# BachiLi/redner

Hardware: AMD Instinct MI355X
Metric: Msamples/s fwd+bwd (higher is better)
Workload: dtype f64; 1 GPU; bunny_box 1024x1024, max_bounces 4, Sobol, 256 spp fwd+bwd per step (vertex gradients, primary+secondary edge sampling), sharded by sample index over 1 GPU(s): 256 spp per GPU; spp=256, spp_per_gpu=256, max_bounces=4, parallelism=sample-sharded x1, world_size=1, pool_cap_mb=32768, samples_per_launch=8, sample_workers=2, schedule=library default: two sample workers, batches as large as the buffer cache holds

## Files before the change

### include/redner_amd.h

```cpp
#ifndef REDNER_AMD_H
#define REDNER_AMD_H

#include <stddef.h>
#include <stdint.h>

#ifdef __cplusplus
extern "C" {
#endif

#define RDR_MAX_MIP_LEVELS 8

enum rdr_camera_type { RDR_CAMERA_PERSPECTIVE = 0, RDR_CAMERA_ORTHOGRAPHIC = 1, RDR_CAMERA_FISHEYE = 2,
                       RDR_CAMERA_PANORAMA = 3 };
enum rdr_sampler_type { RDR_SAMPLER_INDEPENDENT = 0, RDR_SAMPLER_SOBOL = 1 };
enum rdr_channel {
    RDR_CH_RADIANCE = 0, RDR_CH_ALPHA, RDR_CH_DEPTH, RDR_CH_POSITION, RDR_CH_GEOMETRY_NORMAL,
    RDR_CH_SHADING_NORMAL, RDR_CH_UV, RDR_CH_BARYCENTRIC_COORDINATES, RDR_CH_DIFFUSE_REFLECTANCE,
    RDR_CH_SPECULAR_REFLECTANCE, RDR_CH_ROUGHNESS, RDR_CH_GENERIC_TEXTURE, RDR_CH_VERTEX_COLOR,
    RDR_CH_SHAPE_ID, RDR_CH_TRIANGLE_ID, RDR_CH_MATERIAL_ID
};

typedef struct rdr_camera_desc {
    int width, height;
    const float *position, *look, *up;
    const float *cam_to_world, *world_to_cam;
    const float *intrinsic_mat_inv, *intrinsic_mat;
    const float *distortion_params;
    float clip_near;
    int camera_type;
    int viewport_beg[2], viewport_end[2];
} rdr_camera_desc;

typedef struct rdr_dcamera_desc {
    float *position, *look, *up, *cam_to_world, *world_to_cam, *intrinsic_mat_inv, *intrinsic_mat,
          *distortion_params;
} rdr_dcamera_desc;

typedef struct rdr_shape_desc {
    const float *vertices;
    const int32_t *indices;
    const float *uvs;
    const float *normals;
    const int32_t *uv_indices;
    const int32_t *normal_indices;
    const float *colors;
    int num_vertices, num_uv_vertices, num_normal_vertices, num_triangles;
    int material_id, light_id;
} rdr_shape_desc;

typedef struct rdr_dshape_desc { float *vertices, *uvs, *normals, *colors; } rdr_dshape_desc;

typedef struct rdr_texture_desc {
    const float *texels[RDR_MAX_MIP_LEVELS];
    int width[RDR_MAX_MIP_LEVELS], height[RDR_MAX_MIP_LEVELS];
    int channels;
    int num_levels;
    const float *uv_scale;
} rdr_texture_desc;

typedef struct rdr_material_desc {
    rdr_texture_desc diffuse_reflectance, specular_reflectance, roughness, generic_texture, normal_map;
    int compute_specular_lighting, two_sided, use_vertex_color;
} rdr_material_desc;

typedef struct rdr_dtexture_desc {
    float *texels[RDR_MAX_MIP_LEVELS];
    int num_levels;
    float *uv_scale;
} rdr_dtexture_desc;
typedef struct rdr_dmaterial_desc {
    rdr_dtexture_desc diffuse_reflectance, specular_reflectance, roughness, generic_texture, normal_map;
} rdr_dmaterial_desc;

typedef struct rdr_area_light_desc {
    int shape_id;
    float intensity[3];
    int two_sided, directly_visible;
} rdr_area_light_desc;
typedef struct rdr_darea_light_desc { float *intensity; } rdr_darea_light_desc;

typedef struct rdr_envmap_desc {
    rdr_texture_desc values;
    const float *env_to_world, *world_to_env;
    const float *sample_cdf_ys, *sample_cdf_xs;
    float pdf_norm;
    int directly_visible;
} rdr_envmap_desc;
typedef struct rdr_denvmap_desc { rdr_dtexture_desc values; float *world_to_env; } rdr_denvmap_desc;

typedef struct rdr_tuning rdr_tuning;
typedef struct rdr_render_options {
    uint64_t seed;
    int num_samples, max_bounces;
    const int *channels; int num_channels;
    int sampler_type;
    int sample_pixel_center;
    int sample_offset, total_samples;
    const rdr_tuning *tuning;
} rdr_render_options;

enum rdr_tune_flags {
    RDR_TUNE_NO_OVERLAP       = 1 << 0,
    RDR_TUNE_FORCE_GENERAL    = 1 << 1,
    RDR_TUNE_PICKN_WALK       = 1 << 2,
    RDR_TUNE_PICKH_FUSED      = 1 << 3,
    RDR_TUNE_PICKH_LAZY       = 1 << 4,
    RDR_TUNE_NO_HOIST         = 1 << 5,
    RDR_TUNE_REFILL_OFF       = 1 << 6,
    RDR_TUNE_REFILL_ALL       = 1 << 7,
    RDR_TUNE_TRACE_BINARY     = 1 << 8,
    RDR_TUNE_TRACE_NO_LDS_TOP = 1 << 9,
    RDR_TUNE_NO_FUSED_BOUNCE  = 1 << 10,
    RDR_TUNE_PICKH_ONE_LAUNCH = 1 << 11,
    RDR_TUNE_NO_NEE_COMPACT   = 1 << 12,
    RDR_TUNE_LARGE_FORMS      = 1 << 13,
    RDR_TUNE_TRACE_EVERY_CONTINUATION = 1 << 14
};
struct rdr_tuning {
    unsigned flags;
    int batch_samples;
    int64_t batch_lanes;
    int workers;
    int refill_rays_per_lane, refill_idle_lanes, refill_steps;
    int wide_max_rays;
    int gather_budget;
    int gather_heavy_cap_plus1, gather_work_cap_plus1;
    int mem_available_mb;
    int refill_order;
    int pickh_slots_per_lane, pickh_idle_lanes, pickh_steps;
    int stale_event_cap_plus1;
};

void rdr_set_stream(void *hip_stream);
void rdr_set_pool_cap_mb(int64_t megabytes);
int64_t rdr_get_pool_cap_mb(void);
enum rdr_build_flags {
    RDR_BUILD_NO_REFIT        = 1 << 0,
    RDR_BUILD_NO_EDGE_CACHE   = 1 << 1,
    RDR_BUILD_SYNC_EDGES      = 1 << 2,
    RDR_BUILD_EDGE_HOST_BUILD = 1 << 3
};
void rdr_set_build_flags(unsigned flags);

typedef struct rdr_dscene_desc {
    rdr_dcamera_desc camera;
    const rdr_dshape_desc *shapes; int num_shapes;
    const rdr_dmaterial_desc *materials; int num_materials;
    const rdr_darea_light_desc *area_lights; int num_area_lights;
    const rdr_denvmap_desc *envmap;
} rdr_dscene_desc;

typedef struct rdr_scene rdr_scene;

rdr_scene *rdr_scene_create(const rdr_camera_desc *camera,
                            const rdr_shape_desc *shapes, int num_shapes,
                            const rdr_material_desc *materials, int num_materials,
                            const rdr_area_light_desc *area_lights, int num_area_lights,
                            const rdr_envmap_desc *envmap,
                            int use_gpu, int gpu_index,
                            int use_primary_edge_sampling, int use_secondary_edge_sampling);
void rdr_scene_destroy(rdr_scene *scene);
int rdr_scene_max_generic_texture_dimension(const rdr_scene *scene);

int rdr_render(const rdr_scene *scene, const rdr_render_options *options,
               float *rendered_image, const float *d_rendered_image,
               const rdr_dscene_desc *d_scene,
               float *screen_gradient_image, float *debug_image);

int rdr_compute_num_channels(const int *channels, int num_channels, int max_generic_texture_dimension);

enum rdr_deferred_light_type { RDR_DL_AMBIENT = 0, RDR_DL_POINT = 1, RDR_DL_DIRECTIONAL = 2, RDR_DL_SPOT = 3 };
typedef struct rdr_deferred_desc {
    int num_images, height, width;
    int aa_samples, alpha;
    int num_lights;
    const int32_t *light_type;
    const int32_t *image_light_range;
    int gpu_index;
} rdr_deferred_desc;
int rdr_deferred_shade(const rdr_deferred_desc *desc, const float *g_buffer, const float *light_params, float *image);
int rdr_deferred_shade_backward(const rdr_deferred_desc *desc, const float *g_buffer, const float *light_params,
                                const float *d_image, float *d_g_buffer, float *d_light_params);

int rdr_mip_num_levels(int height, int width);
int64_t rdr_mip_backward_scratch(int height, int width, int channels);
int rdr_mip_tiled_stages(int height, int width, int channels);
int rdr_mip_pyramid(int height, int width, int channels, int num_levels, float *const *levels, int gpu_index);
int rdr_mip_pyramid_backward(int height, int width, int channels, int num_levels, const float *const *d_levels, float *d_texels,
                             float *scratch, int64_t scratch_floats, int gpu_index);

typedef enum { rdr_normal_weighting_max = 0, rdr_normal_weighting_cotangent = 1 } rdr_normal_weighting;
typedef struct rdr_mesh_topology rdr_mesh_topology;
rdr_mesh_topology *rdr_mesh_topology_create(const int *indices, int num_triangles, int num_vertices, int use_gpu, int gpu_index);
void rdr_mesh_topology_destroy(rdr_mesh_topology *topology);
int rdr_mesh_topology_read(const rdr_mesh_topology *topology, int *offsets, int *corners);
int rdr_vertex_normal_scratch(const rdr_mesh_topology *topology, int scheme, int64_t *forward_floats, int64_t *backward_floats,
                              int64_t *saved_floats);
int rdr_vertex_normal(const rdr_mesh_topology *topology, int scheme, const float *vertices, float *normals, float *saved,
                      float *scratch, int64_t scratch_floats);
int rdr_vertex_normal_backward(const rdr_mesh_topology *topology, int scheme, const float *vertices, const float *saved,
                               const float *d_normals, float *d_vertices, float *scratch, int64_t scratch_floats);

const char *rdr_last_error(void);

typedef struct rdr_trace_stats {
    double closest_ms, any_ms;
    uint64_t closest_launches, any_launches;
    uint64_t closest_rays, any_rays;
    uint64_t closest_nodes, closest_tris, any_nodes, any_tris;
    uint64_t closest_wide_nodes, any_wide_nodes;
    double closest_union_ms, any_union_ms;
} rdr_trace_stats;
void rdr_trace_stats_enable(int timing, int counting);
void rdr_trace_stats_reset(void);
void rdr_trace_stats_get(rdr_trace_stats *out);

int rdr_scene_trace(const rdr_scene *scene, const float *rays, int32_t *hits, int num_rays, int any_hit);

uint64_t rdr_trim_cache(void);

typedef struct rdr_debug_counters {
    uint64_t device_mallocs, host_count_reads;
    uint64_t last_batch_samples, last_workers;
} rdr_debug_counters;
void rdr_debug_counters_get(rdr_debug_counters *out);

int rdr_debug_bvh_check(const rdr_scene *scene);

int rdr_debug_dump_edges(const rdr_scene *scene, const char *path);

int rdr_debug_trace_plan(int num_nodes, int stack_need, int has_wide, int wide_stack_need, int num_rays, int any_hit, int coherent,
                         int counting, const rdr_tuning *tuning, int32_t *out );
int rdr_debug_scene_trace_plan(const rdr_scene *scene, int num_rays, int any_hit, int coherent, int counting,
                               const rdr_tuning *tuning, int32_t *out );

int rdr_libm_exact(void);

int rdr_debug_libm(int fn, const double *x, const double *y, double *out, int n);

enum rdr_scatter_op {
    RDR_SCATTER_ACCUM = 0, RDR_SCATTER_ACCUM_TEXEL, RDR_SCATTER_ACCUM_PLAIN, RDR_SCATTER_ACCUM_TRIPLE,
    RDR_SCATTER_ACCUM_TEXEL_TRIPLE, RDR_SCATTER_TRIGRAD_WAVE, RDR_SCATTER_POSITIONS_WAVE
};
enum rdr_scatter_target {
    RDR_TARGET_VERTICES = 0, RDR_TARGET_UVS, RDR_TARGET_NORMALS, RDR_TARGET_COLORS, RDR_TARGET_TEXTURE, RDR_TARGET_LIGHTS,
    RDR_TARGET_CAMERA, RDR_TARGET_ENVMAP
};
int rdr_debug_grad_scatter(const rdr_scene *scene, const rdr_dscene_desc *d_scene, uint64_t job_samples, int op, int plain,
                           int num_lanes, const uint8_t *active, const int32_t *target, const int32_t *index,
                           const double *values);

#ifdef __cplusplus
}
#endif
#endif
```

### redner_amd/_capi.py

```python
import ctypes as C
import os

MAX_MIP = 8
_HERE = os.path.dirname(os.path.abspath(__file__))
DEFAULT_LIBRARY = os.path.join(_HERE, 'lib', 'libredner_amd.so')
EXACT_LIBRARY = os.path.join(_HERE, 'lib', 'libredner_amd_exact.so')

c_float_p = C.POINTER(C.c_float)
c_int_p = C.POINTER(C.c_int32)


class CameraDesc(C.Structure):
    _fields_ = [('width', C.c_int), ('height', C.c_int),
                ('position', C.c_void_p), ('look', C.c_void_p), ('up', C.c_void_p),
                ('cam_to_world', C.c_void_p), ('world_to_cam', C.c_void_p),
                ('intrinsic_mat_inv', C.c_void_p), ('intrinsic_mat', C.c_void_p),
                ('distortion_params', C.c_void_p),
                ('clip_near', C.c_float), ('camera_type', C.c_int),
                ('viewport_beg', C.c_int * 2), ('viewport_end', C.c_int * 2)]


class DCameraDesc(C.Structure):
    _fields_ = [(n, C.c_void_p) for n in ('position', 'look', 'up', 'cam_to_world', 'world_to_cam',
                                          'intrinsic_mat_inv', 'intrinsic_mat', 'distortion_params')]


class ShapeDesc(C.Structure):
    _fields_ = [('vertices', C.c_void_p), ('indices', C.c_void_p), ('uvs', C.c_void_p),
                ('normals', C.c_void_p), ('uv_indices', C.c_void_p), ('normal_indices', C.c_void_p),
                ('colors', C.c_void_p),
                ('num_vertices', C.c_int), ('num_uv_vertices', C.c_int), ('num_normal_vertices', C.c_int),
                ('num_triangles', C.c_int), ('material_id', C.c_int), ('light_id', C.c_int)]


class DShapeDesc(C.Structure):
    _fields_ = [(n, C.c_void_p) for n in ('vertices', 'uvs', 'normals', 'colors')]


class TextureDesc(C.Structure):
    _fields_ = [('texels', C.c_void_p * MAX_MIP), ('width', C.c_int * MAX_MIP), ('height', C.c_int * MAX_MIP),
                ('channels', C.c_int), ('num_levels', C.c_int), ('uv_scale', C.c_void_p)]


class MaterialDesc(C.Structure):
    _fields_ = [('diffuse_reflectance', TextureDesc), ('specular_reflectance', TextureDesc),
                ('roughness', TextureDesc), ('generic_texture', TextureDesc), ('normal_map', TextureDesc),
                ('compute_specular_lighting', C.c_int), ('two_sided', C.c_int), ('use_vertex_color', C.c_int)]


class DTextureDesc(C.Structure):
    _fields_ = [('texels', C.c_void_p * MAX_MIP), ('num_levels', C.c_int), ('uv_scale', C.c_void_p)]


class DMaterialDesc(C.Structure):
    _fields_ = [(n, DTextureDesc) for n in ('diffuse_reflectance', 'specular_reflectance', 'roughness',
                                            'generic_texture', 'normal_map')]


class AreaLightDesc(C.Structure):
    _fields_ = [('shape_id', C.c_int), ('intensity', C.c_float * 3), ('two_sided', C.c_int),
                ('directly_visible', C.c_int)]


class DAreaLightDesc(C.Structure):
    _fields_ = [('intensity', C.c_void_p)]


class EnvmapDesc(C.Structure):
    _fields_ = [('values', TextureDesc), ('env_to_world', C.c_void_p), ('world_to_env', C.c_void_p),
                ('sample_cdf_ys', C.c_void_p), ('sample_cdf_xs', C.c_void_p),
                ('pdf_norm', C.c_float), ('directly_visible', C.c_int)]


class DEnvmapDesc(C.Structure):
    _fields_ = [('values', DTextureDesc), ('world_to_env', C.c_void_p)]


class Tuning(C.Structure):
    _fields_ = [('flags', C.c_uint), ('batch_samples', C.c_int), ('batch_lanes', C.c_int64), ('workers', C.c_int),
                ('refill_rays_per_lane', C.c_int), ('refill_idle_lanes', C.c_int), ('refill_steps', C.c_int),
                ('wide_max_rays', C.c_int), ('gather_budget', C.c_int),
                ('gather_heavy_cap_plus1', C.c_int), ('gather_work_cap_plus1', C.c_int), ('mem_available_mb', C.c_int),
                ('refill_order', C.c_int), ('pickh_slots_per_lane', C.c_int), ('pickh_idle_lanes', C.c_int), ('pickh_steps', C.c_int),
                ('stale_event_cap_plus1', C.c_int)]


TUNE_NO_OVERLAP, TUNE_FORCE_GENERAL, TUNE_PICKN_WALK, TUNE_PICKH_FUSED, TUNE_PICKH_LAZY, TUNE_NO_HOIST, TUNE_REFILL_OFF, \
    TUNE_REFILL_ALL, TUNE_TRACE_BINARY, TUNE_TRACE_NO_LDS_TOP, TUNE_NO_FUSED_BOUNCE, TUNE_PICKH_ONE_LAUNCH, TUNE_NO_NEE_COMPACT, \
    TUNE_LARGE_FORMS, TUNE_TRACE_EVERY_CONTINUATION = [1 << k for k in range(15)]
BUILD_NO_REFIT, BUILD_NO_EDGE_CACHE, BUILD_SYNC_EDGES, BUILD_EDGE_HOST_BUILD = [1 << k for k in range(4)]


class RenderOptionsDesc(C.Structure):
    _fields_ = [('seed', C.c_uint64), ('num_samples', C.c_int), ('max_bounces', C.c_int),
                ('channels', C.POINTER(C.c_int)), ('num_channels', C.c_int),
                ('sampler_type', C.c_int), ('sample_pixel_center', C.c_int),
                ('sample_offset', C.c_int), ('total_samples', C.c_int),
                ('tuning', C.POINTER(Tuning))]


class DSceneDesc(C.Structure):
    _fields_ = [('camera', DCameraDesc),
                ('shapes', C.POINTER(DShapeDesc)), ('num_shapes', C.c_int),
                ('materials', C.POINTER(DMaterialDesc)), ('num_materials', C.c_int),
                ('area_lights', C.POINTER(DAreaLightDesc)), ('num_area_lights', C.c_int),
                ('envmap', C.POINTER(DEnvmapDesc))]


class TraceStats(C.Structure):
    _fields_ = [('closest_ms', C.c_double), ('any_ms', C.c_double),
                ('closest_launches', C.c_uint64), ('any_launches', C.c_uint64),
                ('closest_rays', C.c_uint64), ('any_rays', C.c_uint64),
                ('closest_nodes', C.c_uint64), ('closest_tris', C.c_uint64),
                ('any_nodes', C.c_uint64), ('any_tris', C.c_uint64),
                ('closest_wide_nodes', C.c_uint64), ('any_wide_nodes', C.c_uint64),
                ('closest_union_ms', C.c_double), ('any_union_ms', C.c_double)]


class DebugCounters(C.Structure):
    _fields_ = [('device_mallocs', C.c_uint64), ('host_count_reads', C.c_uint64),
                ('last_batch_samples', C.c_uint64), ('last_workers', C.c_uint64)]


class DeferredDesc(C.Structure):
    _fields_ = [('num_images', C.c_int), ('height', C.c_int), ('width', C.c_int),
                ('aa_samples', C.c_int), ('alpha', C.c_int), ('num_lights', C.c_int),
                ('light_type', c_int_p), ('image_light_range', c_int_p), ('gpu_index', C.c_int)]


DL_AMBIENT, DL_POINT, DL_DIRECTIONAL, DL_SPOT = range(4)

EXPORTS = ('rdr_scene_create', 'rdr_scene_destroy', 'rdr_scene_max_generic_texture_dimension',
           'rdr_render', 'rdr_compute_num_channels', 'rdr_last_error',
           'rdr_trace_stats_enable', 'rdr_trace_stats_reset', 'rdr_trace_stats_get', 'rdr_scene_trace',
           'rdr_debug_counters_get', 'rdr_trim_cache', 'rdr_debug_dump_edges', 'rdr_debug_bvh_check',
           'rdr_set_stream', 'rdr_set_pool_cap_mb', 'rdr_get_pool_cap_mb', 'rdr_set_build_flags', 'rdr_debug_libm', 'rdr_libm_exact',
           'rdr_deferred_shade', 'rdr_deferred_shade_backward',
           'rdr_mip_num_levels', 'rdr_mip_backward_scratch', 'rdr_mip_tiled_stages', 'rdr_mip_pyramid',
           'rdr_mip_pyramid_backward',
           'rdr_mesh_topology_create', 'rdr_mesh_topology_destroy', 'rdr_mesh_topology_read', 'rdr_vertex_normal_scratch',
           'rdr_vertex_normal', 'rdr_vertex_normal_backward', 'rdr_debug_trace_plan', 'rdr_debug_scene_trace_plan',
           'rdr_debug_grad_scatter')

SCATTER_ACCUM, SCATTER_ACCUM_TEXEL, SCATTER_ACCUM_PLAIN, SCATTER_ACCUM_TRIPLE, SCATTER_ACCUM_TEXEL_TRIPLE, \
    SCATTER_TRIGRAD_WAVE, SCATTER_POSITIONS_WAVE = range(7)
TARGET_VERTICES, TARGET_UVS, TARGET_NORMALS, TARGET_COLORS, TARGET_TEXTURE, TARGET_LIGHTS, TARGET_CAMERA, TARGET_ENVMAP = range(8)

_lib = None
_lib_path = None


def load(path=None):
    global _lib, _lib_path
    path = path or os.environ.get('REDNER_AMD_LIB') or \
        (EXACT_LIBRARY if os.environ.get('REDNER_AMD_LIBM', '').lower() == 'exact' else DEFAULT_LIBRARY)
    if not os.path.exists(path):
        raise RuntimeError(
            "redner_amd: native library %s not found. Build it with "
            "`python -c 'import __graft_entry__ as g; g.build()'` (hipcc, gfx950). "
            "There is no CPU fallback." % path)
    lib = C.CDLL(path)
    for name in EXPORTS:
        if not hasattr(lib, name):
            raise RuntimeError("redner_amd: %s does not export %s" % (path, name))
    lib.rdr_scene_create.restype = C.c_void_p
    lib.rdr_scene_create.argtypes = [C.POINTER(CameraDesc), C.POINTER(ShapeDesc), C.c_int,
                                     C.POINTER(MaterialDesc), C.c_int, C.POINTER(AreaLightDesc), C.c_int,
                                     C.POINTER(EnvmapDesc), C.c_int, C.c_int, C.c_int, C.c_int]
    lib.rdr_scene_destroy.restype = None
    lib.rdr_scene_destroy.argtypes = [C.c_void_p]
    lib.rdr_scene_max_generic_texture_dimension.restype = C.c_int
    lib.rdr_scene_max_generic_texture_dimension.argtypes = [C.c_void_p]
    lib.rdr_render.restype = C.c_int
    lib.rdr_render.argtypes = [C.c_void_p, C.POINTER(RenderOptionsDesc), C.c_void_p, C.c_void_p,
                               C.POINTER(DSceneDesc), C.c_void_p, C.c_void_p]
    lib.rdr_compute_num_channels.restype = C.c_int
    lib.rdr_compute_num_channels.argtypes = [C.POINTER(C.c_int), C.c_int, C.c_int]
    lib.rdr_last_error.restype = C.c_char_p
    lib.rdr_last_error.argtypes = []
    lib.rdr_trace_stats_enable.restype = None
    lib.rdr_trace_stats_enable.argtypes = [C.c_int, C.c_int]
    lib.rdr_trace_stats_reset.restype = None
    lib.rdr_debug_counters_get.restype = None
    lib.rdr_debug_counters_get.argtypes = [C.POINTER(DebugCounters)]
    lib.rdr_trim_cache.restype = C.c_uint64
    lib.rdr_trim_cache.argtypes = []
    lib.rdr_debug_bvh_check.restype = C.c_int
    lib.rdr_debug_bvh_check.argtypes = [C.c_void_p]
    lib.rdr_set_stream.restype = None
    lib.rdr_set_stream.argtypes = [C.c_void_p]
    lib.rdr_set_pool_cap_mb.restype = None
    lib.rdr_set_pool_cap_mb.argtypes = [C.c_int64]
    lib.rdr_get_pool_cap_mb.restype = C.c_int64
    lib.rdr_get_pool_cap_mb.argtypes = []
    lib.rdr_set_build_flags.restype = None
    lib.rdr_set_build_flags.argtypes = [C.c_uint]
    lib.rdr_trace_stats_get.restype = None
    lib.rdr_trace_stats_get.argtypes = [C.POINTER(TraceStats)]
    lib.rdr_scene_trace.restype = C.c_int
    lib.rdr_scene_trace.argtypes = [C.c_void_p, C.c_void_p, C.c_void_p, C.c_int, C.c_int]
    lib.rdr_libm_exact.restype = C.c_int
    lib.rdr_libm_exact.argtypes = []
    lib.rdr_debug_libm.restype = C.c_int
    lib.rdr_debug_libm.argtypes = [C.c_int, C.c_void_p, C.c_void_p, C.c_void_p, C.c_int]
    lib.rdr_deferred_shade.restype = C.c_int
    lib.rdr_deferred_shade.argtypes = [C.POINTER(DeferredDesc), C.c_void_p, C.c_void_p, C.c_void_p]
    lib.rdr_deferred_shade_backward.restype = C.c_int
    lib.rdr_deferred_shade_backward.argtypes = [C.POINTER(DeferredDesc), C.c_void_p, C.c_void_p, C.c_void_p, C.c_void_p, C.c_void_p]
    lib.rdr_mip_num_levels.restype = C.c_int
    lib.rdr_mip_num_levels.argtypes = [C.c_int, C.c_int]
    lib.rdr_mip_backward_scratch.restype = C.c_int64
    lib.rdr_mip_backward_scratch.argtypes = [C.c_int, C.c_int, C.c_int]
    lib.rdr_mip_tiled_stages.restype = C.c_int
    lib.rdr_mip_tiled_stages.argtypes = [C.c_int, C.c_int, C.c_int]
    lib.rdr_mip_pyramid.restype = C.c_int
    lib.rdr_mip_pyramid.argtypes = [C.c_int, C.c_int, C.c_int, C.c_int, C.POINTER(C.c_void_p), C.c_int]
    lib.rdr_mip_pyramid_backward.restype = C.c_int
    lib.rdr_mip_pyramid_backward.argtypes = [C.c_int, C.c_int, C.c_int, C.c_int, C.POINTER(C.c_void_p), C.c_void_p, C.c_void_p,
                                             C.c_int64, C.c_int]
    lib.rdr_mesh_topology_create.restype = C.c_void_p
    lib.rdr_mesh_topology_create.argtypes = [C.c_void_p, C.c_int, C.c_int, C.c_int, C.c_int]
    lib.rdr_mesh_topology_destroy.restype = None
    lib.rdr_mesh_topology_destroy.argtypes = [C.c_void_p]
    lib.rdr_mesh_topology_read.restype = C.c_int
    lib.rdr_mesh_topology_read.argtypes = [C.c_void_p, C.c_void_p, C.c_void_p]
    lib.rdr_vertex_normal_scratch.restype = C.c_int
    lib.rdr_vertex_normal_scratch.argtypes = [C.c_void_p, C.c_int, C.POINTER(C.c_int64), C.POINTER(C.c_int64), C.POINTER(C.c_int64)]
    lib.rdr_vertex_normal.restype = C.c_int
    lib.rdr_vertex_normal.argtypes = [C.c_void_p, C.c_int, C.c_void_p, C.c_void_p, C.c_void_p, C.c_void_p, C.c_int64]
    lib.rdr_vertex_normal_backward.restype = C.c_int
    lib.rdr_vertex_normal_backward.argtypes = [C.c_void_p, C.c_int, C.c_void_p, C.c_void_p, C.c_void_p, C.c_void_p, C.c_void_p,
                                               C.c_int64]
    lib.rdr_debug_trace_plan.restype = C.c_int
    lib.rdr_debug_trace_plan.argtypes = [C.c_int] * 8 + [C.POINTER(Tuning), C.c_void_p]
    lib.rdr_debug_scene_trace_plan.restype = C.c_int
    lib.rdr_debug_scene_trace_plan.argtypes = [C.c_void_p] + [C.c_int] * 4 + [C.POINTER(Tuning), C.c_void_p]
    lib.rdr_debug_grad_scatter.restype = C.c_int
    lib.rdr_debug_grad_scatter.argtypes = [C.c_void_p, C.POINTER(DSceneDesc), C.c_uint64, C.c_int, C.c_int, C.c_int,
                                           C.c_void_p, C.c_void_p, C.c_void_p, C.c_void_p]
    _lib, _lib_path = lib, path
    return lib


def lib():
    if _lib is None:
        load()
    return _lib


def library_path():
    return _lib_path


def is_product_library():
    return _lib_path in (DEFAULT_LIBRARY, EXACT_LIBRARY)


def last_error():
    return lib().rdr_last_error().decode('utf-8', 'replace')
```

### redner_amd/csrc/capi.cpp

```cpp
#include "../../include/redner_amd.h"
#include "render.h"
#include "tuning.h"
#include "trace_plan.h"
#include "edges.h"
#include "deferred.h"
#include "mipmap.h"
#include "vertex_normal.h"
#include <cstdio>
#include "scene.h"
#include <cstring>
#include <exception>
#include <mutex>
#include <string>
#include <vector>
#include <cstdlib>

namespace {
thread_local std::string g_last_error;
std::recursive_mutex g_device_lock[16];
std::recursive_mutex &device_lock(int gpu_index) { return g_device_lock[(gpu_index < 0 ? 0 : gpu_index) & 15]; }
void set_error(const char *what) { g_last_error = what ? what : "unknown error"; }
thread_local void *g_user_stream = nullptr;
void use_caller_stream() { exec::ctx().stream = (hipStream_t)g_user_stream; }
}

struct LibmProbe {
    int fn; const double *x, *y; double *out;
    RDR_FN void operator()(int i) const {
        const double a = x[i], b = y[i];
        double r;
        switch (fn) {
            case 0: r = gm::sin(a); break;
            case 1: r = gm::cos(a); break;
            case 2: r = gm::atan2(a, b); break;
            case 3: r = gm::atan(a); break;
            case 4: r = gm::acos(a); break;
            case 5: r = gm::log(a); break;
            default: r = gm::pow(a, b); break;
        }
        out[i] = r;
    }
};

extern "C" {

const char *rdr_last_error(void) { return g_last_error.c_str(); }

rdr_scene *rdr_scene_create(const rdr_camera_desc *camera, const rdr_shape_desc *shapes, int num_shapes,
                            const rdr_material_desc *materials, int num_materials,
                            const rdr_area_light_desc *area_lights, int num_area_lights,
                            const rdr_envmap_desc *envmap, int use_gpu, int gpu_index,
                            int use_primary_edge_sampling, int use_secondary_edge_sampling) {
    try {
        g_last_error.clear();
        std::lock_guard<std::recursive_mutex> lk(device_lock(gpu_index));
        use_caller_stream();
        return reinterpret_cast<rdr_scene *>(rdr::create_scene(camera, shapes, num_shapes, materials, num_materials,
                                                               area_lights, num_area_lights, envmap, use_gpu, gpu_index,
                                                               use_primary_edge_sampling, use_secondary_edge_sampling));
    } catch (const std::exception &e) {
        set_error(e.what());
        return nullptr;
    }
}

void rdr_scene_destroy(rdr_scene *scene) {
    if (!scene) return;
    rdr::Scene *s = reinterpret_cast<rdr::Scene *>(scene);
    std::lock_guard<std::recursive_mutex> lk(device_lock(s->gpu_index));
    delete s;
}

int rdr_scene_max_generic_texture_dimension(const rdr_scene *scene) {
    return scene ? reinterpret_cast<const rdr::Scene *>(scene)->max_generic_texture_dimension : 0;
}

int rdr_render(const rdr_scene *scene, const rdr_render_options *options, float *rendered_image,
               const float *d_rendered_image, const rdr_dscene_desc *d_scene, float *screen_gradient_image,
               float *debug_image) {
    try {
        g_last_error.clear();
        if (!scene || !options) throw std::runtime_error("rdr_render: scene and options are required");
        const rdr::Scene &s = *reinterpret_cast<const rdr::Scene *>(scene);
        std::lock_guard<std::recursive_mutex> lk(device_lock(s.gpu_index));
        exec::select_device(1, s.gpu_index);
        use_caller_stream();
        rdr::render(s, *options, rendered_image, d_rendered_image, d_scene, screen_gradient_image, debug_image);
        return 0;
    } catch (const std::exception &e) {
        set_error(e.what());
        return 1;
    }
}

int rdr_deferred_shade(const rdr_deferred_desc *desc, const float *g_buffer, const float *light_params, float *image) {
    try {
        g_last_error.clear();
        if (!desc) throw std::runtime_error("rdr_deferred_shade: a description is required");
        std::lock_guard<std::recursive_mutex> lk(device_lock(desc->gpu_index));
        exec::select_device(desc->gpu_index >= 0, desc->gpu_index);
        use_caller_stream();
        rdr::dfr::shade(*desc, g_buffer, light_params, image);
        return 0;
    } catch (const std::exception &e) {
        set_error(e.what());
        return 1;
    }
}

int rdr_deferred_shade_backward(const rdr_deferred_desc *desc, const float *g_buffer, const float *light_params,
                                const float *d_image, float *d_g_buffer, float *d_light_params) {
    try {
        g_last_error.clear();
        if (!desc) throw std::runtime_error("rdr_deferred_shade_backward: a description is required");
        std::lock_guard<std::recursive_mutex> lk(device_lock(desc->gpu_index));
        exec::select_device(desc->gpu_index >= 0, desc->gpu_index);
        use_caller_stream();
        rdr::dfr::shade_backward(*desc, g_buffer, light_params, d_image, d_g_buffer, d_light_params);
        return 0;
    } catch (const std::exception &e) {
        set_error(e.what());
        return 1;
    }
}

int rdr_mip_num_levels(int height, int width) { return height > 0 && width > 0 ? rdr::mip::num_levels(height, width) : 0; }

int64_t rdr_mip_backward_scratch(int height, int width, int channels) {
    try {
        g_last_error.clear();
        return (int64_t)rdr::mip::scratch_floats(rdr::mip::make_shape(height, width, channels, rdr_mip_num_levels(height, width),
                                                                      "rdr_mip_backward_scratch"));
    } catch (const std::exception &e) {
        set_error(e.what());
        return -1;
    }
}

int rdr_mip_tiled_stages(int height, int width, int channels) {
    try {
        g_last_error.clear();
        return rdr::mip::tiled_stages(rdr::mip::make_shape(height, width, channels, rdr_mip_num_levels(height, width),
                                                           "rdr_mip_tiled_stages"));
    } catch (const std::exception &e) {
        set_error(e.what());
        return -1;
    }
}

static void mip_select(int gpu_index, const char *who) {
#if !defined(RDR_HOSTSIM)
    if (gpu_index < 0) throw std::runtime_error(std::string(who) + ": host memory (negative gpu_index) is for the CPU harness only");
#endif
    exec::select_device(gpu_index >= 0, gpu_index);
    use_caller_stream();
}

int rdr_mip_pyramid(int height, int width, int channels, int num_levels, float *const *levels, int gpu_index) {
    try {
        g_last_error.clear();
        std::lock_guard<std::recursive_mutex> lk(device_lock(gpu_index));
        mip_select(gpu_index, "rdr_mip_pyramid");
        rdr::mip::pyramid(height, width, channels, num_levels, levels);
        return 0;
    } catch (const std::exception &e) {
        set_error(e.what());
        return 1;
    }
}

int rdr_mip_pyramid_backward(int height, int width, int channels, int num_levels, const float *const *d_levels, float *d_texels,
                             float *scratch, int64_t scratch_floats, int gpu_index) {
    try {
        g_last_error.clear();
        std::lock_guard<std::recursive_mutex> lk(device_lock(gpu_index));
        mip_select(gpu_index, "rdr_mip_pyramid_backward");
        rdr::mip::pyramid_backward(height, width, channels, num_levels, d_levels, d_texels, scratch,
                                   scratch_floats > 0 ? (size_t)scratch_floats : 0);
        return 0;
    } catch (const std::exception &e) {
        set_error(e.what());
        return 1;
    }
}

static const rdr::vnrm::Topology &topology_of(const rdr_mesh_topology *topology, const char *who) {
    if (!topology) throw std::runtime_error(std::string(who) + ": a topology is required");
    return *reinterpret_cast<const rdr::vnrm::Topology *>(topology);
}

rdr_mesh_topology *rdr_mesh_topology_create(const int *indices, int num_triangles, int num_vertices, int use_gpu, int gpu_index) {
    try {
        g_last_error.clear();
        const int place = use_gpu ? (gpu_index < 0 ? 0 : gpu_index) : -1;
        std::lock_guard<std::recursive_mutex> lk(device_lock(place));
        mip_select(place, "rdr_mesh_topology_create");
        return reinterpret_cast<rdr_mesh_topology *>(rdr::vnrm::create_topology(indices, num_triangles, num_vertices, place));
    } catch (const std::exception &e) {
        set_error(e.what());
        return nullptr;
    }
}

void rdr_mesh_topology_destroy(rdr_mesh_topology *topology) {
    if (!topology) return;
    rdr::vnrm::Topology *t = reinterpret_cast<rdr::vnrm::Topology *>(topology);
    std::lock_guard<std::recursive_mutex> lk(device_lock(t->gpu_index));
    try { exec::select_device(t->gpu_index >= 0, t->gpu_index); } catch (const std::exception &) {}
    delete t;
}

int rdr_mesh_topology_read(const rdr_mesh_topology *topology, int *offsets, int *corners) {
    try {
        g_last_error.clear();
        const rdr::vnrm::Topology &t = topology_of(topology, "rdr_mesh_topology_read");
        std::lock_guard<std::recursive_mutex> lk(device_lock(t.gpu_index));
        mip_select(t.gpu_index, "rdr_mesh_topology_read");
        rdr::vnrm::read_topology(t, offsets, corners);
        return 0;
    } catch (const std::exception &e) {
        set_error(e.what());
        return 1;
    }
}

int rdr_vertex_normal_scratch(const rdr_mesh_topology *topology, int scheme, int64_t *forward_floats, int64_t *backward_floats,
                              int64_t *saved_floats) {
    try {
        g_last_error.clear();
        const rdr::vnrm::Topology &t = topology_of(topology, "rdr_vertex_normal_scratch");
        const bool cot = rdr::vnrm::cotangent(scheme, "rdr_vertex_normal_scratch");
        if (forward_floats) *forward_floats = (int64_t)rdr::vnrm::forward_scratch_floats(t, cot);
        if (backward_floats) *backward_floats = (int64_t)rdr::vnrm::backward_scratch_floats(t, cot);
        if (saved_floats) *saved_floats = (int64_t)rdr::vnrm::saved_floats(t, cot);
        return 0;
    } catch (const std::exception &e) {
        set_error(e.what());
        return 1;
    }
}

int rdr_vertex_normal(const rdr_mesh_topology *topology, int scheme, const float *vertices, float *normals, float *saved,
                      float *scratch, int64_t scratch_floats) {
    try {
        g_last_error.clear();
        const rdr::vnrm::Topology &t = topology_of(topology, "rdr_vertex_normal");
        std::lock_guard<std::recursive_mutex> lk(device_lock(t.gpu_index));
        mip_select(t.gpu_index, "rdr_vertex_normal");
        rdr::vnrm::forward(t, scheme, vertices, normals, saved, scratch, scratch_floats > 0 ? (size_t)scratch_floats : 0);
        return 0;
    } catch (const std::exception &e) {
        set_error(e.what());
        return 1;
    }
}

int rdr_vertex_normal_backward(const rdr_mesh_topology *topology, int scheme, const float *vertices, const float *saved,
                               const float *d_normals, float *d_vertices, float *scratch, int64_t scratch_floats) {
    try {
        g_last_error.clear();
        const rdr::vnrm::Topology &t = topology_of(topology, "rdr_vertex_normal_backward");
        std::lock_guard<std::recursive_mutex> lk(device_lock(t.gpu_index));
        mip_select(t.gpu_index, "rdr_vertex_normal_backward");
        rdr::vnrm::backward(t, scheme, vertices, saved, d_normals, d_vertices, scratch, scratch_floats > 0 ? (size_t)scratch_floats : 0);
        return 0;
    } catch (const std::exception &e) {
        set_error(e.what());
        return 1;
    }
}

int rdr_compute_num_channels(const int *channels, int num_channels, int max_generic_texture_dimension) {
    return rdr::compute_num_channels(channels, num_channels, max_generic_texture_dimension);
}

void rdr_trace_stats_enable(int timing, int counting) {
    exec::trace_stats().timing = timing != 0;
    exec::trace_stats().counting = counting != 0;
}
void rdr_trace_stats_reset(void) {
    exec::TraceStats &s = exec::trace_stats();
    bool t = s.timing, c = s.counting;
    exec::trace_stats_collect();
    s = exec::TraceStats();
    s.timing = t; s.counting = c;
}
void rdr_trace_stats_get(rdr_trace_stats *out) {
    exec::trace_stats_collect();
    const exec::TraceStats &s = exec::trace_stats();
    out->closest_ms = s.closest_ms; out->any_ms = s.any_ms;
    out->closest_launches = s.closest_launches; out->any_launches = s.any_launches;
    out->closest_rays = s.closest_rays; out->any_rays = s.any_rays;
    out->closest_nodes = s.nodes[0]; out->closest_tris = s.tris[0];
    out->any_nodes = s.nodes[1]; out->any_tris = s.tris[1];
    out->closest_wide_nodes = s.wide_nodes[0]; out->any_wide_nodes = s.wide_nodes[1];
    out->closest_union_ms = s.closest_union_ms; out->any_union_ms = s.any_union_ms;
}

uint64_t rdr_trim_cache(void) {
    std::unique_lock<std::recursive_mutex> all[16];
    for (int d = 0; d < 16; ++d) all[d] = std::unique_lock<std::recursive_mutex>(g_device_lock[d]);
    rdr::drop_edge_cache();
    const uint64_t bytes = exec::pool_cached_bytes();
    exec::pool_trim();
    return bytes;
}

void rdr_set_stream(void *hip_stream) { g_user_stream = hip_stream; }
void rdr_set_pool_cap_mb(int64_t megabytes) { exec::pool_set_cap(megabytes < 0 ? -1 : (long long)megabytes << 20); }
int64_t rdr_get_pool_cap_mb(void) { return (int64_t)(exec::pool_cap_bytes() >> 20); }
void rdr_set_build_flags(unsigned flags) { rdr::build_flags_ref().store(flags); }

void rdr_debug_counters_get(rdr_debug_counters *out) {
    out->device_mallocs = exec::pool_device_mallocs();
    out->host_count_reads = exec::host_count_reads();
    out->last_batch_samples = (uint64_t)rdr::last_schedule()[0].load();
    out->last_workers = (uint64_t)rdr::last_schedule()[1].load();
}

int rdr_debug_dump_edges(const rdr_scene *scene, const char *path) {
    const rdr::Scene &s = *reinterpret_cast<const rdr::Scene *>(scene);
    FILE *f = fopen(path, "w");
    if (!f) return 1;
    {
        std::lock_guard<std::recursive_mutex> lk(device_lock(s.gpu_index));
        exec::select_device(1, s.gpu_index);
        try { s.edge_data(); } catch (const std::exception &e) { set_error(e.what()); fclose(f); return 1; }
    }
    if (!s.edges) { fprintf(f, "edges 0\n"); fclose(f); return 0; }
    if (s.edges->device_trees) {
        std::lock_guard<std::recursive_mutex> lk(device_lock(s.gpu_index));
        try { rdr::download_edge_trees(*s.edges); } catch (const std::exception &e) { set_error(e.what()); fclose(f); return 1; }
    }
    const rdr::EdgeData &ed = *s.edges;
    fprintf(f, "edges %d\n", (int)ed.edges.size());
    for (const rdr::EdgeD &e : ed.edges) fprintf(f, "%d %d %d %d %d\n", e.shape_id, e.v0, e.v1, e.f0, e.f1);
    if (!ed.cs_nodes.empty() || !ed.ncs_nodes.empty()) {
        fprintf(f, "expand %.17g\n", ed.edge_bounds_expand);
        for (int t = 0; t < 2; ++t) {
            const std::vector<rdr::EdgeNode> &nodes = t == 0 ? ed.cs_nodes : ed.ncs_nodes;
            int nl = t == 0 ? ed.cs_leaves : ed.ncs_leaves;
            int nn = (int)nodes.size() - nl;
            fprintf(f, "%s %d %d\n", t == 0 ? "cs" : "ncs", nl == 0 ? 0 : nn, nl);
            for (size_t i = 0; i < nodes.size(); ++i) {
                const rdr::EdgeNode &n = nodes[i];
                fprintf(f, "%d %d %d %d %d %.17g %.17g", (int)i, n.parent, n.child0, n.child1, n.edge_id, n.wlen, n.cost);
                fprintf(f, " %.17g %.17g %.17g %.17g %.17g %.17g", n.p_min.x, n.p_min.y, n.p_min.z, n.p_max.x, n.p_max.y, n.p_max.z);
                if (t == 1) fprintf(f, " %.17g %.17g %.17g %.17g %.17g %.17g", n.d_min.x, n.d_min.y, n.d_min.z, n.d_max.x, n.d_max.y, n.d_max.z);
                fprintf(f, "\n");
            }
        }
    }
    fclose(f);
    return 0;
}

int rdr_debug_bvh_check(const rdr_scene *scene) {
    try {
        const rdr::Scene &s = *reinterpret_cast<const rdr::Scene *>(scene);
        if (!s.bvh_dev || s.bvh_dev->parent) return -1;
        std::lock_guard<std::recursive_mutex> lk(device_lock(s.gpu_index));
        exec::select_device(1, s.gpu_index);
        use_caller_stream();
        std::vector<rt::MeshView> meshes(s.shapes.size());
        for (size_t i = 0; i < s.shapes.size(); ++i) meshes[i] = rt::MeshView{s.h_vertices[i].data(), s.h_indices[i].data(), s.shapes[i].num_triangles};
        const rt::BvhHost h = rt::build_bvh(meshes);
        const rt::BvhDev &d = *s.bvh_dev;
        int bad = 0;
        if ((int)h.nodes.size() != d.num_nodes || (int)h.ids.size() != 2 * d.num_slots || (int)h.wide.size() != d.num_wide ||
            h.depth != d.depth || h.wide_stack_need != d.wide_stack_need)
            return 1000000 + std::abs((int)h.nodes.size() - d.num_nodes);
        std::vector<rt::Node> nodes(d.num_nodes);
        std::vector<int> ids((size_t)2 * d.num_slots);
        std::vector<float> tris((size_t)9 * d.num_slots);
        std::vector<rt::Node4> wide(d.num_wide);
        exec::download(nodes.data(), d.nodes, sizeof(rt::Node) * nodes.size());
        exec::download(ids.data(), d.ids, sizeof(int) * ids.size());
        exec::download(tris.data(), d.tris, sizeof(float) * tris.size());
        exec::download(wide.data(), d.wide, sizeof(rt::Node4) * wide.size());
        for (size_t i = 0; i < nodes.size(); ++i) {
            const rt::Node &a = nodes[i], &b = h.nodes[i];
            bool same = a.a == b.a && a.b == b.b;
            for (int k = 0; k < 3; ++k) same = same && a.lo[k] == b.lo[k] && a.hi[k] == b.hi[k];
            bad += !same;
        }
        for (size_t i = 0; i < ids.size(); ++i) bad += ids[i] != h.ids[i];
        for (size_t i = 0; i < tris.size(); ++i) bad += !(tris[i] == h.tris[i]);
        for (size_t i = 0; i < wide.size(); ++i) {
            const rt::Node4 &a = wide[i], &b = h.wide[i];
            bool same = a.aux[0] == b.aux[0];
            for (int k = 0; k < 4; ++k)
                same = same && a.link[k] == b.link[k] && a.lox[k] == b.lox[k] && a.loy[k] == b.loy[k] && a.loz[k] == b.loz[k] &&
                       a.hix[k] == b.hix[k] && a.hiy[k] == b.hiy[k] && a.hiz[k] == b.hiz[k];
            bad += !same;
        }
        return bad;
    } catch (const std::exception &e) {
        set_error(e.what());
        return -2;
    }
}

int rdr_scene_trace(const rdr_scene *scene, const float *rays, int32_t *hits, int num_rays, int any_hit) {
    try {
        g_last_error.clear();
        const rdr::Scene &s = *reinterpret_cast<const rdr::Scene *>(scene);
        std::lock_guard<std::recursive_mutex> lk(device_lock(s.gpu_index));
        exec::select_device(1, s.gpu_index);
        use_caller_stream();
        exec::trace(s.bvh, reinterpret_cast<const rt::RayRec *>(rays), reinterpret_cast<rt::HitRec *>(hits), num_rays, any_hit != 0);
        exec::sync();
        return 0;
    } catch (const std::exception &e) {
        set_error(e.what());
        return 1;
    }
}

static int write_trace_plan(const exec::TraceFacts &facts, int num_rays, int any_hit, int coherent, int counting,
                            const rdr_tuning *tuning, int32_t *out) {
    try {
        g_last_error.clear();
        if (num_rays <= 0 || !out || facts.num_nodes < 0 || facts.stack_need < 0 || facts.wide_stack_need < 0)
            throw std::runtime_error("rdr_debug_trace_plan: bad arguments");
        const exec::TracePlan p = exec::plan_trace(facts, num_rays, any_hit != 0, coherent != 0, counting != 0, rdr::resolve_tuning(tuning));
        const int32_t v[10] = {(int32_t)p.form, p.stack, p.short_index, p.stage_top, p.sorted, p.counting, p.blocks, p.rays_per_lane, p.idle_min, p.steps};
        std::memcpy(out, v, sizeof(v));
        return 0;
    } catch (const std::exception &e) {
        set_error(e.what());
        return 1;
    }
}
int rdr_debug_trace_plan(int num_nodes, int stack_need, int has_wide, int wide_stack_need, int num_rays, int any_hit, int coherent,
                         int counting, const rdr_tuning *tuning, int32_t *out) {
    return write_trace_plan(exec::TraceFacts{num_nodes, stack_need, wide_stack_need, has_wide != 0}, num_rays, any_hit, coherent, counting, tuning, out);
}
int rdr_debug_scene_trace_plan(const rdr_scene *scene, int num_rays, int any_hit, int coherent, int counting, const rdr_tuning *tuning,
                               int32_t *out) {
    if (!scene) { set_error("rdr_debug_scene_trace_plan: bad arguments"); return 1; }
    return write_trace_plan(exec::trace_facts(reinterpret_cast<const rdr::Scene *>(scene)->bvh), num_rays, any_hit, coherent, counting, tuning, out);
}

int rdr_debug_libm(int fn, const double *x, const double *y, double *out, int n) {
    try {
        g_last_error.clear();
        if (fn < 0 || fn > 6 || n < 0) throw std::runtime_error("rdr_debug_libm: bad arguments");
        std::lock_guard<std::recursive_mutex> lk(device_lock(exec::current_device()));
        exec::select_device(1, exec::current_device());
        use_caller_stream();
        const size_t bytes = sizeof(double) * (size_t)n;
        struct Held {
            double *p[3] = {nullptr, nullptr, nullptr};
            ~Held() { exec::device_sync(); for (double *q : p) exec::dfree(q); }
        } held;
        for (double *&q : held.p) q = (double *)exec::dmalloc(bytes);
        double *dx = held.p[0], *dy = held.p[1], *dout = held.p[2];
        exec::upload(dx, x, bytes);
        if (y) exec::upload(dy, y, bytes); else exec::zero(dy, bytes);
        exec::launch(exec::Count(n), LibmProbe{fn, dx, dy, dout});
        exec::download(out, dout, bytes);
        exec::sync();
        return 0;
    } catch (const std::exception &e) {
        set_error(e.what());
        return 1;
    }
}

int rdr_debug_grad_scatter(const rdr_scene *scene, const rdr_dscene_desc *d_scene, uint64_t job_samples, int op, int plain,
                           int num_lanes, const uint8_t *active, const int32_t *target, const int32_t *index,
                           const double *values) {
    try {
        g_last_error.clear();
        if (!scene || !d_scene) throw std::runtime_error("rdr_debug_grad_scatter: scene and d_scene are required");
        const rdr::Scene &s = *reinterpret_cast<const rdr::Scene *>(scene);
        std::lock_guard<std::recursive_mutex> lk(device_lock(s.gpu_index));
        exec::select_device(1, s.gpu_index);
        use_caller_stream();
        rdr::debug_grad_scatter(s, *d_scene, (size_t)job_samples, op, plain != 0, num_lanes, active, target, index, values);
        return 0;
    } catch (const std::exception &e) {
        set_error(e.what());
        return 1;
    }
}

}
```

### redner_amd/csrc/grad_store.h

```cpp
#pragma once
#include "scene.h"
#include "stages_bwd.h"
#include <algorithm>
#include <exception>
#include <stdexcept>
#include <vector>

namespace rdr {

struct Arena {
    std::vector<void *> blocks;
    template <class T> T *get(size_t count) {
        T *p = (T *)exec::pool_alloc(sizeof(T) * (count ? count : 1));
        blocks.push_back(p);
        return p;
    }
    ~Arena() {
        if (std::uncaught_exceptions() > 0) exec::device_sync();
        for (void *p : blocks) exec::pool_free(p);
    }
};

struct GradStore {
    Arena arena;
    GScene g;
    std::vector<GShape> h_shapes;
    std::vector<GMaterial> h_materials;

    static constexpr size_t kSmallTensor = 16384, kSmallTierMax = 65536;
    struct Tier { double *base = nullptr; size_t stride = 0, cursor = 0; int replicas = 1; };
    Tier tier[2];
    struct Pair { double *acc; float *out; size_t count; int tier; };
    std::vector<Pair> pairs;
    bool counting = true;

    double *place(size_t count, int &t) {
        const size_t padded = (count + 3) & ~(size_t)3;
        t = (count <= kSmallTensor && tier[0].cursor + padded <= kSmallTierMax) ? 0 : 1;
        const size_t at = tier[t].cursor;
        tier[t].cursor += padded;
        return counting ? reinterpret_cast<double *>(8) : tier[t].base + at;
    }
    double *mirror(float *out, size_t count) {
        if (!out || count == 0) return nullptr;
        int t;
        double *acc = place(count, t);
        if (!counting) pairs.push_back(Pair{acc, out, count, t});
        return acc;
    }
    GTex mirror_tex(const TexD &t, const rdr_dtexture_desc &d) {
        GTex g;
        for (int i = 0; i < kMaxMip; ++i) g.texels[i] = nullptr;
        g.uv_scale = nullptr;
        if (t.num_levels == 0 || d.num_levels == 0) return g;
        bool constant = t.width[0] <= 0 && t.height[0] <= 0;
        for (int i = 0; i < t.num_levels && i < d.num_levels; ++i) {
            size_t count = constant ? (size_t)t.channels : (size_t)t.width[i] * t.height[i] * t.channels;
            g.texels[i] = mirror(d.texels[i], count);
        }
        g.uv_scale = mirror(d.uv_scale, 2);
        return g;
    }

    GradStore(const Scene &scene, const rdr_dscene_desc &ds, size_t job_samples) {
        counting = true;
        layout(scene, ds);
        for (Tier &t : tier) t.stride = (t.cursor + 31) & ~(size_t)31;
        tier[0].replicas = tier[0].stride ? exec::choose_replicas(tier[0].stride * sizeof(double), 256 * kSmallTierMax * sizeof(double)) : 1;
        tier[1].replicas = tier[1].stride ? exec::choose_replicas(tier[1].stride * sizeof(double), exec::replica_budget(job_samples)) : 1;
        const size_t small_total = tier[0].stride * tier[0].replicas, total = small_total + tier[1].stride * tier[1].replicas;
        double *block = arena.get<double>(total);
        exec::zero(block, sizeof(double) * total);
        tier[0].base = block; tier[1].base = block + small_total;
        exec::set_replicas(ReplicaLayout{block + tier[0].stride, tier[0].stride, tier[1].stride,
                                         (unsigned)(tier[0].replicas - 1), (unsigned)(tier[1].replicas - 1)});
        counting = false; pairs.clear();
        for (Tier &t : tier) t.cursor = 0;
        layout(scene, ds);
        for (const Pair &p : pairs) {
            const Tier &t = tier[p.tier];
            if (p.acc < t.base || p.acc + p.count > t.base + t.stride)
                throw std::runtime_error("render: gradient accumulator straddles a replica tier (GradStore::layout)");
        }
        accumulators_laid_out(tier[0].base, tier[0].stride);
    }
    void layout(const Scene &scene, const rdr_dscene_desc &ds) {
        if (ds.num_shapes != (int)scene.shapes.size() || ds.num_materials != (int)scene.materials.size() ||
            ds.num_area_lights != (int)scene.lights.size())
            throw std::runtime_error("render: DScene does not match the Scene (shape/material/light counts)");
        h_shapes.resize(scene.shapes.size());
        for (size_t i = 0; i < scene.shapes.size(); ++i) {
            const ShapeD &sh = scene.shapes[i];
            const rdr_dshape_desc &d = ds.shapes[i];
            h_shapes[i].vertices = mirror(d.vertices, (size_t)3 * sh.num_vertices);
            if (!h_shapes[i].vertices) throw std::runtime_error("render: DShape.vertices is required");
            h_shapes[i].uvs = sh.uvs ? mirror(d.uvs, (size_t)2 * (sh.num_uv_vertices > 0 ? sh.num_uv_vertices : sh.num_vertices)) : nullptr;
            h_shapes[i].normals = sh.normals ? mirror(d.normals, (size_t)3 * (sh.num_normal_vertices > 0 ? sh.num_normal_vertices : sh.num_vertices)) : nullptr;
            h_shapes[i].colors = sh.colors ? mirror(d.colors, (size_t)3 * sh.num_vertices) : nullptr;
        }
        h_materials.resize(scene.materials.size());
        for (size_t i = 0; i < scene.materials.size(); ++i) {
            const MaterialD &m = scene.materials[i];
            const rdr_dmaterial_desc &d = ds.materials[i];
            h_materials[i].diffuse = mirror_tex(m.diffuse, d.diffuse_reflectance);
            h_materials[i].specular = mirror_tex(m.specular, d.specular_reflectance);
            h_materials[i].roughness = mirror_tex(m.roughness, d.roughness);
            h_materials[i].generic = mirror_tex(m.generic, d.generic_texture);
            h_materials[i].normal_map = mirror_tex(m.normal_map, d.normal_map);
        }
        if (!counting) {
            g.shapes = arena.get<GShape>(h_shapes.size());
            exec::upload(g.shapes, h_shapes.data(), sizeof(GShape) * h_shapes.size());
            g.materials = arena.get<GMaterial>(h_materials.size());
            exec::upload(g.materials, h_materials.data(), sizeof(GMaterial) * h_materials.size());
        }
        g.light_intensity = nullptr;
        if (!scene.lights.empty()) {
            int light_tier = 0;
            g.light_intensity = place(3 * scene.lights.size(), light_tier);
            if (!counting)
                for (size_t l = 0; l < scene.lights.size(); ++l)
                    if (ds.area_lights[l].intensity) pairs.push_back(Pair{g.light_intensity + 3 * l, ds.area_lights[l].intensity, 3, light_tier});
        }
        const rdr_dcamera_desc &dc = ds.camera;
        g.cam.position = mirror(dc.position, 3); g.cam.look = mirror(dc.look, 3); g.cam.up = mirror(dc.up, 3);
        g.cam.cam_to_world = mirror(dc.cam_to_world, 16); g.cam.world_to_cam = mirror(dc.world_to_cam, 16);
        g.cam.intrinsic_mat_inv = mirror(dc.intrinsic_mat_inv, 9); g.cam.intrinsic_mat = mirror(dc.intrinsic_mat, 9);
        g.cam.distortion = mirror(dc.distortion_params, 8);
        g.envmap = nullptr;
        if (scene.d.envmap && ds.envmap) {
            GEnvmap h_envmap;
            h_envmap.values = mirror_tex(scene.h_envmap.values, ds.envmap->values);
            h_envmap.world_to_env = mirror(ds.envmap->world_to_env, 16);
            if (!counting) {
                g.envmap = arena.get<GEnvmap>(1);
                exec::upload(g.envmap, &h_envmap, sizeof(GEnvmap));
            }
        }
    }
    void flush() {
        for (const Pair &p : pairs)
            if (p.tier == 0) accumulator_before_fold(tier[0].base, p.acc, p.count);
        accumulators_folded();
        std::vector<Pair> by_out(pairs);
        std::sort(by_out.begin(), by_out.end(), [](const Pair &a, const Pair &b) { return a.out < b.out; });
        bool aliased = false;
        for (size_t i = 1; i < by_out.size(); ++i) aliased = aliased || by_out[i - 1].out + by_out[i - 1].count > by_out[i].out;
        for (int t = 0; t < 2; ++t) {
            const Tier &tr = tier[t];
            std::vector<FlushSegment> seg;
            for (const Pair &p : pairs) if (p.tier == t) seg.push_back(FlushSegment{(size_t)(p.acc - tr.base), p.count, p.out});
            if (seg.empty()) continue;
            std::sort(seg.begin(), seg.end(), [](const FlushSegment &a, const FlushSegment &b) { return a.begin < b.begin; });
            if (tr.stride > (size_t)0x7fffffff) throw std::runtime_error("render: gradient block too large");
            FlushSegment *d_seg = arena.get<FlushSegment>(seg.size());
            exec::upload(d_seg, seg.data(), sizeof(FlushSegment) * seg.size());
            if (!aliased) exec::launch((int)tr.stride, FlushGrad{tr.base, tr.stride, tr.replicas, d_seg, (int)seg.size()});
            else for (size_t i = 0; i < seg.size(); ++i)
                exec::launch((int)(seg[i].begin + seg[i].count), FlushGrad{tr.base, tr.stride, tr.replicas, d_seg + i, 1});
        }
        exec::set_replicas(ReplicaLayout{nullptr, 0, 0, 0, 0});
    }
};

}
```

### redner_amd/csrc/hip/exec.h

```cpp
#pragma once
#include <hip/hip_runtime.h>
#include <stdint.h>
#include <stdio.h>
#include <atomic>
#include <condition_variable>
#include <cstdlib>
#include <exception>
#include <functional>
#include <mutex>
#include <stdexcept>
#include <string>
#include <thread>

#define RDR_FN __host__ __device__ inline
#define RDR_INLINE_CALL [[clang::always_inline]]
#define RDR_DEV_FN __device__ inline
#define RDR_STACK_DECL(T, name, N) __shared__ T name##_lds[(N) * 256]; T *name = name##_lds + threadIdx.x
#define RDR_STACK_AT(name, k) name[(k) * 256]
#define RDR_WALK_STACK_MEMBER(T, name, N)
#define RDR_WALK_STACK(st, T, name, N, TAG) (rdr::lds_column<T, N, TAG>())
#define RDR_WALK_AT(stk, k) stk[(k) * 256]

namespace rdr {
template <class T, int N, int TAG>
__device__ inline T *lds_column() {
    __shared__ T tile[N * 256];
    return tile + threadIdx.x;
}
__host__ inline void *lds_column_host_stub() { return nullptr; }

struct ReplicaLayout {
    const double *hot_end;
    unsigned long long hot_stride;
    unsigned long long stride;
    unsigned hot_mask, mask;
};
static __device__ ReplicaLayout g_rep = {nullptr, 0, 0, 0, 0};
__device__ inline double *replica_of(double *p) {
    const unsigned wave = blockIdx.x * 4u + (threadIdx.x >> 6);
    const bool hot = p < g_rep.hot_end;
    return p + (size_t)(wave & (hot ? g_rep.hot_mask : g_rep.mask)) * (hot ? g_rep.hot_stride : g_rep.stride);
}
constexpr int kAccumRounds = 3;

__device__ inline double wave_sum(double x) {
#define RDR_DPP_ADD(ctrl)                                                                                  \
    {                                                                                                      \
        const int lo_ = __builtin_amdgcn_update_dpp(0, __double2loint(x), ctrl, 0xf, 0xf, true);         \
        const int hi_ = __builtin_amdgcn_update_dpp(0, __double2hiint(x), ctrl, 0xf, 0xf, true);         \
        x += __hiloint2double(hi_, lo_);                                                                   \
    }
    RDR_DPP_ADD(0xB1)
    RDR_DPP_ADD(0x4E)
    RDR_DPP_ADD(0x141)
    RDR_DPP_ADD(0x140)
#undef RDR_DPP_ADD
    const int lo = __double2loint(x), hi = __double2hiint(x);
    const double r0 = __hiloint2double(__builtin_amdgcn_readlane(hi, 0), __builtin_amdgcn_readlane(lo, 0));
    const double r1 = __hiloint2double(__builtin_amdgcn_readlane(hi, 16), __builtin_amdgcn_readlane(lo, 16));
    const double r2 = __hiloint2double(__builtin_amdgcn_readlane(hi, 32), __builtin_amdgcn_readlane(lo, 32));
    const double r3 = __hiloint2double(__builtin_amdgcn_readlane(hi, 48), __builtin_amdgcn_readlane(lo, 48));
    return (r0 + r1) + (r2 + r3);
}

typedef __attribute__((address_space(1))) double *GlobalDouble;
__device__ inline void global_add_f64(double *p, double v) { (void)__builtin_amdgcn_global_atomic_fadd_f64((GlobalDouble)p, v); }
__device__ inline void accum_rounds(double *p, double v, int ROUNDS);
__device__ inline void accum(double *p, double v) { accum_rounds(p, v, kAccumRounds); }
static __device__ int g_texel_rounds = 8;
__device__ inline void accum_texel(double *p, double v) { accum_rounds(p, v, g_texel_rounds); }
__device__ inline void accum_rounds(double *p, double v, int ROUNDS) {
    p = replica_of(p);
    const unsigned long long act = __ballot(1);
    const unsigned long long addr = (unsigned long long)p;
    const int lane = threadIdx.x & 63;
    const int vlo = __double2loint(v), vhi = __double2hiint(v);
    unsigned long long rem = act;
    bool mine = true;
    for (int round = 0; round < ROUNDS && rem != 0; ++round) {
        const int l = __ffsll((long long)rem) - 1;
        const unsigned lo = __builtin_amdgcn_readlane((unsigned)addr, l);
        const unsigned hi = __builtin_amdgcn_readlane((unsigned)(addr >> 32), l);
        const bool same = addr == (((unsigned long long)hi << 32) | lo);
        const unsigned long long m = __ballot(same) & rem;
        rem &= ~m;
        if (__popcll(m) < 2) continue;
        double s;
        if (act == ~0ull) {
            s = wave_sum(same ? v : 0.0);
        } else {
            s = 0;
            unsigned long long mm = m;
            while (mm) {
                const int k = __ffsll((long long)mm) - 1;
                mm &= mm - 1;
                s += __hiloint2double(__builtin_amdgcn_readlane(vhi, k), __builtin_amdgcn_readlane(vlo, k));
            }
        }
        if (lane == l) global_add_f64(p, s);
        if (same) mine = false;
    }
    if (mine) global_add_f64(p, v);
}
__device__ inline void accum_triple_rounds(double *p, double x, double y, double z, int ROUNDS) {
    p = replica_of(p);
    const unsigned long long act = __ballot(1);
    const unsigned long long addr = (unsigned long long)p;
    const int lane = threadIdx.x & 63;
    unsigned long long rem = act;
    bool mine = true;
    for (int round = 0; round < ROUNDS && rem != 0; ++round) {
        const int l = __ffsll((long long)rem) - 1;
        const unsigned lo = __builtin_amdgcn_readlane((unsigned)addr, l);
        const unsigned hi = __builtin_amdgcn_readlane((unsigned)(addr >> 32), l);
        const bool same = addr == (((unsigned long long)hi << 32) | lo);
        const unsigned long long m = __ballot(same) & rem;
        rem &= ~m;
        if (__popcll(m) < 2) continue;
        double sx, sy, sz;
        if (act == ~0ull) {
            sx = wave_sum(same ? x : 0.0); sy = wave_sum(same ? y : 0.0); sz = wave_sum(same ? z : 0.0);
        } else {
            sx = sy = sz = 0;
            const int xlo = __double2loint(x), xhi = __double2hiint(x), ylo = __double2loint(y), yhi = __double2hiint(y);
            const int zlo = __double2loint(z), zhi = __double2hiint(z);
            unsigned long long mm = m;
            while (mm) {
                const int k = __ffsll((long long)mm) - 1;
                mm &= mm - 1;
                sx += __hiloint2double(__builtin_amdgcn_readlane(xhi, k), __builtin_amdgcn_readlane(xlo, k));
                sy += __hiloint2double(__builtin_amdgcn_readlane(yhi, k), __builtin_amdgcn_readlane(ylo, k));
                sz += __hiloint2double(__builtin_amdgcn_readlane(zhi, k), __builtin_amdgcn_readlane(zlo, k));
            }
        }
        if (lane == l) { global_add_f64(p, sx); global_add_f64(p + 1, sy); global_add_f64(p + 2, sz); }
        if (same) mine = false;
    }
    if (mine) { global_add_f64(p, x); global_add_f64(p + 1, y); global_add_f64(p + 2, z); }
}
__device__ inline void accum_triple(double *p, double x, double y, double z) { accum_triple_rounds(p, x, y, z, kAccumRounds); }
__device__ inline void accum_texel_triple(double *p, double x, double y, double z) { accum_triple_rounds(p, x, y, z, g_texel_rounds); }
__host__ inline void accum_triple(double *p, double x, double y, double z) { p[0] += x; p[1] += y; p[2] += z; }
__host__ inline void accum_texel_triple(double *p, double x, double y, double z) { p[0] += x; p[1] += y; p[2] += z; }
__host__ inline void accum(double *p, double v) { *p += v; }
__host__ inline void accum_texel(double *p, double v) { *p += v; }
__device__ inline void accum_plain(double *p, double v) {
    p = replica_of(p);
    global_add_f64(p, v);
}
__host__ inline void accum_plain(double *p, double v) { *p += v; }
__device__ inline void atomic_add_f64(double *p, double v) { global_add_f64(p, v); }
__host__ inline void atomic_add_f64(double *p, double v) { *p += v; }
__device__ inline int atomic_fetch_add(int *p, int v) { return atomicAdd(p, v); }
__host__ inline int atomic_fetch_add(int *p, int v) { int o = *p; *p += v; return o; }
}

namespace exec {

inline void check(hipError_t e, const char *what) {
    if (e != hipSuccess) throw std::runtime_error(std::string("HIP error in ") + what + ": " + hipGetErrorString(e));
}

struct Context {
    hipStream_t stream = nullptr;
};
Context &ctx();

inline void *dmalloc(size_t bytes) {
    void *p = nullptr;
    check(hipMalloc(&p, bytes ? bytes : 16), "hipMalloc");
    return p;
}
inline void dfree(void *p) { if (p) (void)hipFree(p); }
void *pool_alloc(size_t bytes);
void pool_free(void *p);
void pool_trim();
size_t pool_cached_bytes();
size_t memory_available();
double memory_held_by_others();
void pool_set_cap(long long bytes);
size_t pool_cap_bytes();
size_t pool_device_mallocs();
inline std::atomic<size_t> &host_count_reads_ref() { static std::atomic<size_t> n{0}; return n; }
inline size_t host_count_reads() { return host_count_reads_ref().load(); }
inline void zero(void *p, size_t bytes) { if (bytes) check(hipMemsetAsync(p, 0, bytes, ctx().stream), "hipMemsetAsync"); }
inline void upload(void *dst, const void *src, size_t bytes) {
    if (bytes) check(hipMemcpyAsync(dst, src, bytes, hipMemcpyHostToDevice, ctx().stream), "upload");
    check(hipStreamSynchronize(ctx().stream), "upload sync");
}
inline void download(void *dst, const void *src, size_t bytes) {
    if (bytes) check(hipMemcpyAsync(dst, src, bytes, hipMemcpyDeviceToHost, ctx().stream), "download");
    check(hipStreamSynchronize(ctx().stream), "download sync");
}
inline void copy_dev(void *dst, const void *src, size_t bytes) {
    if (bytes) check(hipMemcpyAsync(dst, src, bytes, hipMemcpyDeviceToDevice, ctx().stream), "copy_dev");
}
inline void sync() { check(hipStreamSynchronize(ctx().stream), "sync"); }
constexpr bool kDeviceEdgeTrees = true;
constexpr bool kDeviceBvh = true;
__host__ __device__ inline void gather_stats_add(long, long, int, int) {}
inline void device_sync() { (void)hipDeviceSynchronize(); }
void upload_async(void *dst, const void *src, size_t bytes);
void upload_flush();
struct DownloadItem { void *dst; const void *src; size_t bytes; };
void download_batch(const DownloadItem *items, int n);
const void *device_constant(const void *host, size_t bytes);
inline int current_device() { int d = 0; (void)hipGetDevice(&d); return d; }

hipStream_t side_stream(int k);
struct StreamScope {
    hipStream_t saved;
    explicit StreamScope(hipStream_t s) : saved(ctx().stream) { ctx().stream = s; }
    ~StreamScope() { ctx().stream = saved; }
    StreamScope(const StreamScope &) = delete;
};
constexpr int kMaxHelpers = 3;
class SecondThread {
public:
    static SecondThread &get(int k = 0) {
        static std::mutex lock;
        static SecondThread *t[16][kMaxHelpers] = {};
        int dev = 0;
        (void)hipGetDevice(&dev);
        std::lock_guard<std::mutex> lk(lock);
        SecondThread *&p = t[dev & 15][k];
        if (!p) p = new SecondThread();
        return *p;
    }
    void start(std::function<void()> job) {
        int dev = 0;
        check(hipGetDevice(&dev), "hipGetDevice");
        std::unique_lock<std::mutex> lk(m_);
        cv_.wait(lk, [&] { return state_ == 0; });
        job_ = std::move(job); device_ = dev; state_ = 1;
        cv_.notify_all();
    }
    void wait() {
        std::unique_lock<std::mutex> lk(m_);
        cv_.wait(lk, [&] { return state_ == 0; });
        if (failure_) { std::exception_ptr f = failure_; failure_ = nullptr; std::rethrow_exception(f); }
    }
private:
    SecondThread() { std::thread([this] { loop(); }).detach(); }
    void loop() {
        hipStream_t streams[16] = {};
        for (;;) {
            std::function<void()> job; int dev;
            { std::unique_lock<std::mutex> lk(m_); cv_.wait(lk, [&] { return state_ == 1; }); job = std::move(job_); dev = device_; state_ = 2; }
            std::exception_ptr failure;
            try {
                check(hipSetDevice(dev), "hipSetDevice");
                hipStream_t &s = streams[dev & 15];
                if (!s) {
                    static const bool low = std::getenv("RDR_HELPER_LOW") != nullptr;
                    int least = 0, greatest = 0;
                    if (low && hipDeviceGetStreamPriorityRange(&least, &greatest) == hipSuccess && least != greatest)
                        check(hipStreamCreateWithPriority(&s, hipStreamNonBlocking, least), "hipStreamCreateWithPriority");
                    else check(hipStreamCreateWithFlags(&s, hipStreamNonBlocking), "hipStreamCreate");
                }
                ctx().stream = s;
                job();
                check(hipStreamSynchronize(s), "second stream sync");
            } catch (...) { failure = std::current_exception(); }
            { std::unique_lock<std::mutex> lk(m_); failure_ = failure; state_ = 0; }
            cv_.notify_all();
        }
    }
    std::mutex m_; std::condition_variable cv_;
    std::function<void()> job_; int device_ = 0; int state_ = 0;
    std::exception_ptr failure_;
};

struct Fence {
    hipEvent_t e = nullptr;
    Fence() { check(hipEventCreateWithFlags(&e, hipEventDisableTiming), "hipEventCreate"); }
    ~Fence() { if (e) (void)hipEventDestroy(e); }
    Fence(const Fence &) = delete;
    void after(hipStream_t producer) { check(hipEventRecord(e, producer), "hipEventRecord"); }
    void gate(hipStream_t consumer) { check(hipStreamWaitEvent(consumer, e, 0), "hipStreamWaitEvent"); }
};

inline int choose_replicas(size_t replica_bytes, size_t budget) {
    int r = 256;
    while (r > 1 && replica_bytes * (size_t)r > budget) r >>= 1;
    return r;
}
inline size_t replica_budget(size_t job_samples) {
    static const size_t mb = [] { const char *e = std::getenv("RDR_REPLICA_MB"); return e ? (size_t)std::atoi(e) : (size_t)0; }();
    if (mb) return mb << 20;
    const size_t lo = (size_t)256 << 20, hi = (size_t)1 << 30, want = job_samples * 64;
    return want < lo ? lo : (want > hi ? hi : want);
}
inline void set_replicas(const rdr::ReplicaLayout &layout) {
    check(hipMemcpyToSymbolAsync(HIP_SYMBOL(rdr::g_rep), &layout, sizeof(layout), 0, hipMemcpyHostToDevice, ctx().stream), "set_replicas");
    static const int texel_rounds = [] { const char *e = std::getenv("RDR_TEXEL_ROUNDS"); return e ? std::atoi(e) : 0; }();
    if (texel_rounds > 0) check(hipMemcpyToSymbolAsync(HIP_SYMBOL(rdr::g_texel_rounds), &texel_rounds, sizeof(int), 0, hipMemcpyHostToDevice, ctx().stream), "set_replicas");
    check(hipStreamSynchronize(ctx().stream), "set_replicas sync");
}

struct Count {
    const int *dev; int upper;
    Count(int n) : dev(nullptr), upper(n) {}
    Count(const int *d, int u) : dev(d), upper(u) {}
};

template <class F, class = void> struct MinBlocks { static constexpr int value = 1; };
template <class F> struct MinBlocks<F, decltype((void)F::kMinBlocksPerCU)> { static constexpr int value = F::kMinBlocksPerCU; };

template <class F>
__global__ void __launch_bounds__(256, MinBlocks<F>::value) stage_kernel(F f, int n, const int *count) {
    int i = blockIdx.x * 256 + threadIdx.x;
    if (count) { const int c = *count; n = c < n ? c : n; }
    if (i < n) { RDR_INLINE_CALL f(i); }
}

constexpr int kRefillIdle = 16;
constexpr int kWalkSteps = 16;
template <class W, class = void> struct WalkGate { __device__ static bool closed(const W &) { return false; } };
template <class W> struct WalkGate<W, decltype((void)&W::gate_closed)> { __device__ static bool closed(const W &w) { return w.gate_closed(); } };
template <class W>
__global__ void __launch_bounds__(256) persistent_kernel(W w, int n, const int *count, int *next_item) {
    if (WalkGate<W>::closed(w)) return;
    if (count) { const int c = *count; n = c < n ? c : n; }
    typename W::State st;
    bool busy = false;
    const int lane = threadIdx.x & 63;
    for (;;) {
        const unsigned long long idle = __ballot(!busy);
        const int nidle = __popcll(idle);
        if (nidle >= kRefillIdle) {
            const int leader = __ffsll((long long)idle) - 1;
            int base = 0;
            if (lane == leader) base = atomicAdd(next_item, nidle);
            base = __shfl(base, leader);
            if (!busy) {
                const int item = base + __popcll(idle & ((1ull << lane) - 1ull));
                if (item < n) {
                    if (w.begin(item, st)) busy = true;
                    else w.finish(st);
                }
            }
            if (__ballot(busy) == 0ull && base + nidle >= n) break;
        }
#pragma unroll 1
        for (int it = 0; it < kWalkSteps; ++it) {
            if (busy && w.step(st)) { w.finish(st); busy = false; }
        }
    }
}
#ifndef RDR_CHUNKED_MIN_BLOCKS
#define RDR_CHUNKED_MIN_BLOCKS 1
#endif
template <class W>
__global__ void __launch_bounds__(256, RDR_CHUNKED_MIN_BLOCKS) chunked_kernel(W w, int n, const int *count, int items_per_lane, int idle_min, int steps, int *next_chunk) {
    if (count) { const int c = *count; n = c < n ? c : n; }
    const int chunk = 64 * items_per_lane;
    const int lane = threadIdx.x & 63;
    int next = 0, end = 0;
    bool more = true;
    typename W::State st;
    bool busy = false;
    for (;;) {
        const unsigned long long idle = __ballot(!busy);
        const int nidle = __popcll(idle);
        if (nidle >= idle_min || nidle == 64) {
            if (next >= end && more) {
                int base = 0;
                if (lane == 0) base = atomicAdd(next_chunk, chunk);
                base = __builtin_amdgcn_readfirstlane(base);
                if (base >= n) more = false;
                else { next = base; end = base + chunk < n ? base + chunk : n; }
            }
            if (next < end) {
                if (!busy) {
                    const int item = next + __popcll(idle & ((1ull << lane) - 1ull));
                    if (item < end) {
                        if (w.begin(item, st)) busy = true;
                        else w.finish(st);
                    }
                }
                next += nidle;
            }
        }
        if (__ballot(busy) == 0ull) { if (next >= end && !more) break; continue; }
#pragma unroll 1
        for (int it = 0; it < steps; ++it) {
            if (busy && w.step(st)) { w.finish(st); busy = false; }
        }
    }
}
int *persistent_counter();
template <class W>
inline void launch_chunked(Count n, const W &w, int items_per_lane = 4, int idle_min = 16, int steps = 8) {
    if (n.upper <= 0) return;
    const int per_block = 4 * 64 * items_per_lane;
    const int blocks = (int)std::min<long long>(((long long)n.upper + per_block - 1) / per_block, 256 * 6);
    hipLaunchKernelGGL(chunked_kernel<W>, dim3(blocks), dim3(256), 0, ctx().stream, w, n.upper, n.dev, items_per_lane, idle_min, steps, persistent_counter());
    check(hipGetLastError(), "chunked launch");
}
template <class W>
inline void launch_persistent(Count n, const W &w) {
    if (n.upper <= 0) return;
    int blocks = std::min((n.upper + 255) / 256, 256 * 8);
    hipLaunchKernelGGL(persistent_kernel<W>, dim3(blocks), dim3(256), 0, ctx().stream, w, n.upper, n.dev, persistent_counter());
    check(hipGetLastError(), "persistent launch");
}

template <class F>
inline void launch(Count n, const F &f) {
    if (n.upper <= 0) return;
    int blocks = (n.upper + 255) / 256;
    hipLaunchKernelGGL(stage_kernel<F>, dim3(blocks), dim3(256), 0, ctx().stream, f, n.upper, n.dev);
    check(hipGetLastError(), "stage launch");
}

}

#include "../bvh.h"
namespace exec {

constexpr int kCompactItems = 4;
constexpr int kCompactTile = 256 * kCompactItems;

__device__ inline int lane_prefix(unsigned long long ballot) {
    return __builtin_amdgcn_mbcnt_hi((unsigned)(ballot >> 32), __builtin_amdgcn_mbcnt_lo((unsigned)ballot, 0));
}

template <class P>
__global__ void __launch_bounds__(256) compact_count(const int *in, int n, const int *count, P pred, int *block_counts) {
    __shared__ int wave_tot[4];
    if (count) { const int c = *count; n = c < n ? c : n; }
    int base = blockIdx.x * kCompactTile;
    int cnt = 0;
    for (int it = 0; it < kCompactItems; ++it) {
        int i = base + it * 256 + threadIdx.x;
        bool keep = false;
        if (i < n) { int p = in ? in[i] : i; keep = pred(p); }
        unsigned long long b = __ballot(keep);
        cnt += __popcll(b);
    }
    if ((threadIdx.x & 63) == 0) wave_tot[threadIdx.x >> 6] = cnt;
    __syncthreads();
    if (threadIdx.x == 0) block_counts[blockIdx.x] = wave_tot[0] + wave_tot[1] + wave_tot[2] + wave_tot[3];
}

static __global__ void __launch_bounds__(256) compact_scan(int *block_counts, int nblocks, int *total, int ticket, int *total_dev,
                                                           const int *base, int n_in, const int *count_in, int *dyn, int inc) {
    __shared__ int part[256];
    int per = (nblocks + 255) / 256;
    int beg = threadIdx.x * per, end = min(beg + per, nblocks);
    int s = 0;
    for (int i = beg; i < end; ++i) s += block_counts[i];
    part[threadIdx.x] = s;
    __syncthreads();
    if (threadIdx.x == 0) {
        int run = 0;
        for (int i = 0; i < 256; ++i) { int t = part[i]; part[i] = run; run += t; }
        const int all = run + (base ? *base : 0);
        if (total_dev) *total_dev = all;
        if (dyn) {
            if (count_in) { const int c = *count_in; n_in = c < n_in ? c : n_in; }
            if (n_in > 0) *dyn += inc;
        }
        total[0] = all;
        __hip_atomic_store(total + 1, ticket, __ATOMIC_RELEASE, __HIP_MEMORY_SCOPE_SYSTEM);
    }
    __syncthreads();
    int run = part[threadIdx.x];
    for (int i = beg; i < end; ++i) { int t = block_counts[i]; block_counts[i] = run; run += t; }
}

template <class P>
__global__ void __launch_bounds__(256) compact_scatter(const int *in, int n, const int *count, P pred, const int *block_offsets, int *out,
                                                        const int *out_base, int *pos_out) {
    __shared__ int wave_tot[kCompactItems][4];
    if (count) { const int c = *count; n = c < n ? c : n; }
    if (out_base) { out += *out_base; if (pos_out) pos_out += *out_base; }
    int base = blockIdx.x * kCompactTile;
    int wave = threadIdx.x >> 6;
    int val[kCompactItems]; bool keep[kCompactItems]; int rank[kCompactItems];
    for (int it = 0; it < kCompactItems; ++it) {
        int i = base + it * 256 + threadIdx.x;
        keep[it] = false; val[it] = 0;
        if (i < n) { val[it] = in ? in[i] : i; keep[it] = pred(val[it]); }
        unsigned long long b = __ballot(keep[it]);
        rank[it] = lane_prefix(b);
        if ((threadIdx.x & 63) == 0) wave_tot[it][wave] = __popcll(b);
    }
    __syncthreads();
    int off = block_offsets[blockIdx.x];
    for (int it = 0; it < kCompactItems; ++it) {
        int before = 0;
        for (int w = 0; w < wave; ++w) before += wave_tot[it][w];
        if (keep[it]) {
            out[off + before + rank[it]] = val[it];
            if (pos_out) pos_out[off + before + rank[it]] = base + it * 256 + (int)threadIdx.x;
        }
        off += wave_tot[it][0] + wave_tot[it][1] + wave_tot[it][2] + wave_tot[it][3];
    }
}

struct CompactScratch { int *block_counts = nullptr; int *total = nullptr; volatile int *total_host = nullptr; int capacity = 0; int ticket = 0; };
CompactScratch &compact_scratch(int nblocks, int which = 0);

int *new_count();
template <class P>
inline Count compact_dev(const int *in, Count n, int *out, const P &pred, const Count *append_at = nullptr, int *dyn = nullptr, int inc = 0,
                         int *pos_out = nullptr, int scratch = 0) {
    const int base_upper = append_at ? append_at->upper : 0;
    if (n.upper <= 0) return append_at ? *append_at : Count(0);
    int nblocks = (n.upper + kCompactTile - 1) / kCompactTile;
    if (nblocks > 256 * 4096) throw std::runtime_error("compact: input too large");
    CompactScratch &sc = compact_scratch(nblocks, scratch);
    hipStream_t st = ctx().stream;
    int *result = new_count();
    const int *base = append_at ? append_at->dev : nullptr;
    if (append_at && !append_at->dev) throw std::runtime_error("compact: append position must live on the device");
    hipLaunchKernelGGL(compact_count<P>, dim3(nblocks), dim3(256), 0, st, in, n.upper, n.dev, pred, sc.block_counts);
    const int ticket = ++sc.ticket;
    hipLaunchKernelGGL(compact_scan, dim3(1), dim3(256), 0, st, sc.block_counts, nblocks, sc.total, ticket, result, base, n.upper, n.dev, dyn, inc);
    hipLaunchKernelGGL(compact_scatter<P>, dim3(nblocks), dim3(256), 0, st, in, n.upper, n.dev, pred, sc.block_counts, out, base, pos_out);
    check(hipGetLastError(), "compact launch");
    return Count(result, n.upper + base_upper);
}
template <class P>
inline int compact(const int *in, int n, int *out, const P &pred) {
    if (n <= 0) return 0;
    host_count_reads_ref()++;
    CompactScratch &sc = compact_scratch((n + kCompactTile - 1) / kCompactTile);
    (void)compact_dev(in, Count(n), out, pred);
    hipStream_t st = ctx().stream;
    const int ticket = sc.ticket;
    for (long spins = 0; sc.total_host[1] != ticket; ++spins) {
        __builtin_ia32_pause();
        if ((spins & 0xfffff) == 0xfffff && hipStreamQuery(st) != hipErrorNotReady) {
            check(hipStreamSynchronize(st), "compact sync");
            if (sc.total_host[1] != ticket) throw std::runtime_error("compact: count was not published");
        }
    }
    std::atomic_thread_fence(std::memory_order_acquire);
    return sc.total_host[0];
}
static __global__ void scale_count_kernel(const int *src, int upper, int k, int *dst) {
    const int c = *src;
    *dst = k * (c < upper ? c : upper);
}
inline Count scaled_count(Count c, int k) {
    if (!c.dev) return Count(k * c.upper);
    int *dst = new_count();
    hipLaunchKernelGGL(scale_count_kernel, dim3(1), dim3(1), 0, ctx().stream, c.dev, c.upper, k, dst);
    return Count(dst, k * c.upper);
}
inline int read_count(Count c) {
    if (!c.dev) return c.upper;
    host_count_reads_ref()++;
    int v = 0;
    download(&v, c.dev, sizeof(int));
    return v < c.upper ? v : c.upper;
}

struct TraceStats {
    double closest_ms = 0, any_ms = 0;
    double closest_union_ms = 0, any_union_ms = 0;
    uint64_t closest_launches = 0, any_launches = 0, closest_rays = 0, any_rays = 0, nodes[2] = {0, 0}, tris[2] = {0, 0}, wide_nodes[2] = {0, 0};
    bool timing = false, counting = false;
};
TraceStats &trace_stats();
void trace_stats_collect();
void trace(const rt::BvhD &bvh, const rt::RayRec *rays, rt::HitRec *hits, Count n, bool any, bool coherent = false);
inline int sample_workers(int lanes, int samples, bool batches = false) {
    if (batches) return samples >= 2 ? 2 : 1;
    if (lanes >= (1 << 19)) return 1;
    return (lanes <= (1 << 17) && samples >= 8) ? std::min(4, 1 + kMaxHelpers) : 2;
}
void select_device(int use_gpu, int gpu_index);

}

namespace rdr {
inline void accumulators_laid_out(double *, size_t) {}
inline void accumulator_before_fold(double *, double *, size_t) {}
inline void accumulators_folded() {}
__device__ inline void accum_f32(float *p, float v) { atomicAdd(p, v); }
__host__ inline void accum_f32(float *p, float v) { *p += v; }
}
```

### redner_amd/csrc/hip/trace.hip

```cpp
#include "exec.h"
#include "../tuning.h"
#include "../trace_plan.h"
#include <algorithm>
#include <cstring>
#include <map>
#include <type_traits>
#include <unordered_map>
#include <vector>

namespace exec {

Context &ctx() { static thread_local Context c; return c; }

void select_device(int use_gpu, int gpu_index) {
    if (!use_gpu)
        throw std::runtime_error("redner_amd renders on an MI355X (gfx950) GPU only: Scene(use_gpu=False) "
                                 "is not supported and there is no CPU fallback");
    int count = 0;
    hipError_t e = hipGetDeviceCount(&count);
    if (e != hipSuccess || count == 0)
        throw std::runtime_error("redner_amd: no HIP device is visible (hipGetDeviceCount) -- a gfx950 GPU is required");
    if (gpu_index < 0) gpu_index = 0;
    if (gpu_index >= count) throw std::runtime_error("redner_amd: gpu_index out of range");
    check(hipSetDevice(gpu_index), "hipSetDevice");
}

namespace {
struct Pool {
    std::mutex lock;
    std::multimap<size_t, void *> free_blocks[16];
    std::unordered_map<void *, std::pair<size_t, int>> live;
    size_t parked[16] = {};
    size_t from_driver[16] = {};
    size_t device_mallocs = 0;
    long long cap_override = -1;
};
Pool &pool() { static Pool *p = new Pool(); return *p; }

size_t pool_cap(const Pool &pl) {
    if (pl.cap_override >= 0) return (size_t)pl.cap_override;
    static const size_t dflt = [] {
        if (const char *e = std::getenv("RDR_POOL_CAP_MB")) return (size_t)std::max(0, std::atoi(e)) << 20;
        const size_t eight = (size_t)8192 << 20;
        size_t free_b = 0, total_b = 0;
        if (hipMemGetInfo(&free_b, &total_b) != hipSuccess) { (void)hipGetLastError(); return eight; }
        return std::min(total_b / 4, eight);
    }();
    return dflt;
}
}

size_t pool_cap_bytes() { Pool &pl = pool(); std::lock_guard<std::mutex> lk(pl.lock); return pool_cap(pl); }

void pool_set_cap(long long bytes) {
    Pool &pl = pool();
    std::lock_guard<std::mutex> lk(pl.lock);
    pl.cap_override = bytes;
}

static void *pool_alloc_raw(size_t bytes);
static void pool_release(int only_dev);
void *pool_alloc(size_t bytes) {
    void *p = pool_alloc_raw(bytes);
    static const bool poison = std::getenv("RDR_POOL_POISON") != nullptr;
    if (poison) check(hipMemsetAsync(p, 0xFF, std::max<size_t>(bytes, 16), ctx().stream), "pool poison");
    return p;
}
static void *pool_alloc_raw(size_t bytes) {
    const size_t want = (std::max<size_t>(bytes, 16) + 255) & ~(size_t)255;
    int dev = 0;
    (void)hipGetDevice(&dev);
    Pool &pl = pool();
    {
        std::lock_guard<std::mutex> lk(pl.lock);
        auto &fl = pl.free_blocks[dev & 15];
        auto it = fl.lower_bound(want);
        if (it != fl.end() && it->first <= want + want / 4 + 4096) {
            void *p = it->second;
            pl.live[p] = {it->first, dev};
            pl.parked[dev & 15] -= it->first;
            fl.erase(it);
            return p;
        }
    }
    void *p = nullptr;
    hipError_t e = hipMalloc(&p, want);
    if (e != hipSuccess) {
        (void)hipGetLastError();
        pool_release(dev);
        check(hipMalloc(&p, want), "hipMalloc");
    }
    std::lock_guard<std::mutex> lk(pl.lock);
    pl.device_mallocs++;
    pl.from_driver[dev & 15] += want;
    pl.live[p] = {want, dev};
    return p;
}

void pool_free(void *p) {
    if (!p) return;
    Pool &pl = pool();
    std::unique_lock<std::mutex> lk(pl.lock);
    auto it = pl.live.find(p);
    if (it == pl.live.end()) { lk.unlock(); (void)hipFree(p); return; }
    const size_t bytes = it->second.first;
    const int d = it->second.second & 15;
    pl.live.erase(it);
    if (pl.parked[d] + bytes > pool_cap(pl)) {
        pl.from_driver[d] -= bytes;
        lk.unlock();
        (void)hipFree(p);
        return;
    }
    pl.free_blocks[d].emplace(bytes, p);
    pl.parked[d] += bytes;
}

static void pool_release(int only_dev) {
    Pool &pl = pool();
    std::vector<std::pair<int, void *>> gone;
    {
        std::lock_guard<std::mutex> lk(pl.lock);
        for (int d = 0; d < 16; ++d) {
            if (only_dev >= 0 && d != (only_dev & 15)) continue;
            auto &fl = pl.free_blocks[d];
            for (auto &kv : fl) gone.push_back({d, kv.second});
            fl.clear();
            pl.from_driver[d] -= pl.parked[d];
            pl.parked[d] = 0;
        }
    }
    if (gone.empty()) return;
    int dev = 0;
    (void)hipGetDevice(&dev);
    int at = dev;
    for (auto &g : gone) {
        if (g.first != at) { (void)hipSetDevice(g.first); at = g.first; }
        (void)hipFree(g.second);
    }
    if (at != dev) (void)hipSetDevice(dev);
}
void pool_trim() { pool_release(-1); }

size_t pool_cached_bytes() {
    Pool &pl = pool();
    std::lock_guard<std::mutex> lk(pl.lock);
    size_t total = 0;
    for (size_t b : pl.parked) total += b;
    return total;
}

size_t memory_available() {
    size_t free_b = 0, total_b = 0;
    if (hipMemGetInfo(&free_b, &total_b) != hipSuccess) { (void)hipGetLastError(); return ~(size_t)0; }
    int dev = 0;
    (void)hipGetDevice(&dev);
    Pool &pl = pool();
    std::lock_guard<std::mutex> lk(pl.lock);
    return free_b + pl.parked[dev & 15];
}

double memory_held_by_others() {
    size_t free_b = 0, total_b = 0;
    if (hipMemGetInfo(&free_b, &total_b) != hipSuccess || total_b == 0) { (void)hipGetLastError(); return 0.0; }
    int dev = 0;
    (void)hipGetDevice(&dev);
    Pool &pl = pool();
    std::lock_guard<std::mutex> lk(pl.lock);
    const double used = (double)(total_b - free_b), mine = (double)pl.from_driver[dev & 15];
    return used > mine ? (used - mine) / (double)total_b : 0.0;
}

size_t pool_device_mallocs() { Pool &pl = pool(); std::lock_guard<std::mutex> lk(pl.lock); return pl.device_mallocs; }

namespace {
struct Staging { char *base = nullptr; size_t cap = 0, used = 0; };
Staging &staging() { static thread_local Staging s; return s; }
char *staging_reserve(size_t bytes) {
    Staging &st = staging();
    const size_t need = (bytes + 255) & ~(size_t)255;
    if (st.used + need > st.cap) {
        sync();
        st.used = 0;
        if (need > st.cap) {
            if (st.base) (void)hipHostFree(st.base);
            st.cap = std::max<size_t>(need * 2, (size_t)32 << 20);
            check(hipHostMalloc((void **)&st.base, st.cap, hipHostMallocDefault), "hipHostMalloc (staging)");
        }
    }
    char *p = st.base + st.used;
    st.used += need;
    return p;
}
}

void upload_async(void *dst, const void *src, size_t bytes) {
    if (!bytes) return;
    char *stage = staging_reserve(bytes);
    std::memcpy(stage, src, bytes);
    check(hipMemcpyAsync(dst, stage, bytes, hipMemcpyHostToDevice, ctx().stream), "upload_async");
}
void upload_flush() { sync(); staging().used = 0; }

void download_batch(const DownloadItem *items, int n) {
    size_t total = 0;
    for (int i = 0; i < n; ++i) total += (items[i].bytes + 255) & ~(size_t)255;
    if (!total) return;
    upload_flush();
    char *stage = staging_reserve(total);
    size_t at = 0;
    for (int i = 0; i < n; ++i) {
        if (items[i].bytes) check(hipMemcpyAsync(stage + at, items[i].src, items[i].bytes, hipMemcpyDeviceToHost, ctx().stream), "download_batch");
        at += (items[i].bytes + 255) & ~(size_t)255;
    }
    sync();
    at = 0;
    for (int i = 0; i < n; ++i) {
        if (items[i].bytes) std::memcpy(items[i].dst, stage + at, items[i].bytes);
        at += (items[i].bytes + 255) & ~(size_t)255;
    }
    staging().used = 0;
}

const void *device_constant(const void *host, size_t bytes) {
    static std::mutex lock;
    static std::map<std::pair<const void *, int>, void *> table;
    int dev = 0;
    (void)hipGetDevice(&dev);
    std::lock_guard<std::mutex> lk(lock);
    void *&p = table[{host, dev}];
    if (!p) {
        p = dmalloc(bytes);
        check(hipMemcpy(p, host, bytes, hipMemcpyHostToDevice), "device_constant");
    }
    return p;
}

CompactScratch &compact_scratch(int nblocks, int which) {
    static thread_local CompactScratch per_device[16][2];
    int dev = 0;
    (void)hipGetDevice(&dev);
    CompactScratch &s = per_device[dev & 15][which & 1];
    if (s.capacity < nblocks) {
        if (s.block_counts) (void)hipFree(s.block_counts);
        if (!s.total) {
            void *h = nullptr, *d = nullptr;
            check(hipHostMalloc(&h, 64, hipHostMallocMapped), "hipHostMalloc");
            check(hipHostGetDevicePointer(&d, h, 0), "hipHostGetDevicePointer");
            s.total_host = (volatile int *)h;
            s.total = (int *)d;
            s.total_host[0] = 0; s.total_host[1] = 0;
        }
        s.capacity = nblocks + 1024;
        s.block_counts = (int *)dmalloc(sizeof(int) * s.capacity);
    }
    return s;
}

constexpr int kTopNodes = 255;
typedef const __attribute__((address_space(3))) float *LdsFloats;
struct FetchStaged {
    const rt::Node *nodes; LdsFloats top; int ntop;
    __device__ void pair(int i, rt::Node &l, rt::Node &r) const {
        if (i < ntop) {
            LdsFloats p = top + 8 * i;
            l.lo[0] = p[0]; l.lo[1] = p[1]; l.lo[2] = p[2]; l.a = __float_as_int(p[3]);
            l.hi[0] = p[4]; l.hi[1] = p[5]; l.hi[2] = p[6]; l.b = __float_as_int(p[7]);
            r.lo[0] = p[8]; r.lo[1] = p[9]; r.lo[2] = p[10]; r.a = __float_as_int(p[11]);
            r.hi[0] = p[12]; r.hi[1] = p[13]; r.hi[2] = p[14]; r.b = __float_as_int(p[15]);
        } else { l = nodes[i]; r = nodes[i + 1]; }
    }
    __device__ rt::Node operator()(int i) const {
        rt::Node n;
        if (i < ntop) {
            LdsFloats p = top + 8 * i;
            n.lo[0] = p[0]; n.lo[1] = p[1]; n.lo[2] = p[2]; n.a = __float_as_int(p[3]);
            n.hi[0] = p[4]; n.hi[1] = p[5]; n.hi[2] = p[6]; n.b = __float_as_int(p[7]);
        } else n = nodes[i];
        return n;
    }
};
__device__ inline void wave_tally(unsigned long long *p, unsigned long long v) {
    const unsigned long long act = __ballot(1);
    double s;
    if (act == ~0ull) s = rdr::wave_sum((double)v);
    else {
        s = 0;
        const int lo = (int)(unsigned)v, hi = (int)(unsigned)(v >> 32);
        for (unsigned long long m = act; m; m &= m - 1) {
            const int k = __ffsll((long long)m) - 1;
            s += (double)(((unsigned long long)(unsigned)__builtin_amdgcn_readlane(hi, k) << 32) | (unsigned)__builtin_amdgcn_readlane(lo, k));
        }
    }
    if ((int)(threadIdx.x & 63) == __ffsll((long long)act) - 1) atomicAdd(p, (unsigned long long)s);
}

template <bool ANY, bool COUNT, int STACK, class IDX, bool TOP>
__global__ void __launch_bounds__(256) trace_kernel(rt::BvhD bvh, const rt::RayRec *__restrict__ rays,
                                                    rt::HitRec *__restrict__ hits, int n, const int *count,
                                                    unsigned long long *counters) {
    if (count) { const int c = *count; n = c < n ? c : n; }
    if ((int)(blockIdx.x * 256) >= n) return;
    __shared__ IDX stack_tile[STACK * 256];
    IDX *stack = stack_tile + threadIdx.x;
    __shared__ rt::Node top[kTopNodes + 1];
    const int ntop = TOP ? (bvh.num_nodes < kTopNodes ? bvh.num_nodes : kTopNodes) : 0;
    if (TOP) {
        if ((int)threadIdx.x < ntop) top[threadIdx.x] = bvh.nodes[threadIdx.x];
        __syncthreads();
    }
    int i = blockIdx.x * 256 + threadIdx.x;
    if (i >= n) return;
    rt::RayRec r = rays[i];
    rt::Hit h{0.f, -1, -1};
    rt::Counters c{0, 0};
    if (!(r.tmax < 0.f)) {
        float o[3] = {r.ox, r.oy, r.oz}, d[3] = {r.dx, r.dy, r.dz};
        if (COUNT) {
            h = TOP ? rt::traverse_with<ANY, IDX>(bvh, o, d, r.tmin, r.tmax, stack, 256, &c, FetchStaged{bvh.nodes, (LdsFloats)(const float *)top, ntop})
                    : rt::traverse<ANY, IDX>(bvh, o, d, r.tmin, r.tmax, stack, 256, &c);
        } else {
            h = TOP ? rt::traverse_with<ANY, IDX>(bvh, o, d, r.tmin, r.tmax, stack, 256, (rt::Counters *)nullptr, FetchStaged{bvh.nodes, (LdsFloats)(const float *)top, ntop})
                    : rt::traverse<ANY, IDX>(bvh, o, d, r.tmin, r.tmax, stack, 256, nullptr);
        }
    }
    if (COUNT) {
        wave_tally(&counters[ANY ? 3 : 4], 1ull);
        wave_tally(&counters[0], c.nodes);
        wave_tally(&counters[1], c.tris);
    }
    hits[i] = rt::HitRec{h.shape, h.shape >= 0 ? h.prim : -1};
}

template <bool ANY, bool COUNT, int STACK>
__global__ void __launch_bounds__(256) trace_wide_kernel(rt::BvhD bvh, const rt::RayRec *__restrict__ rays, rt::HitRec *__restrict__ hits,
                                                         int n, const int *count, unsigned long long *counters) {
    if (count) { const int c = *count; n = c < n ? c : n; }
    if ((int)(blockIdx.x * 256) >= n) return;
    __shared__ int stack_tile[STACK * 256];
    int *stack = stack_tile + threadIdx.x;
    const int i = blockIdx.x * 256 + threadIdx.x;
    if (i >= n) return;
    const rt::RayRec r = rays[i];
    rt::Hit h{0.f, -1, -1};
    rt::Counters c{0, 0};
    if (!(r.tmax < 0.f)) {
        const float o[3] = {r.ox, r.oy, r.oz}, d[3] = {r.dx, r.dy, r.dz};
        h = rt::traverse_wide<ANY>(bvh, o, d, r.tmin, r.tmax, stack, 256, COUNT ? &c : nullptr);
    }
    if (COUNT) { wave_tally(&counters[ANY ? 3 : 4], 1ull); wave_tally(&counters[ANY ? 5 : 6], c.nodes); wave_tally(&counters[1], c.tris); }
    hits[i] = rt::HitRec{h.shape, h.shape >= 0 ? h.prim : -1};
}

constexpr int kHybridLds = 16, kHybridSpill = rt::kTraverseStack - kHybridLds;
template <bool ANY, class IDX, int LDSN, class Fetch>
__device__ inline bool traverse_some(const rt::BvhD &bvh, const float o[3], const float d[3], const float inv[3], float tnear, float tfar,
                                     IDX *stack, int (&spill)[LDSN > 0 ? kHybridSpill : 1], rt::Hit &best, int &cur, int &sp, int budget, const Fetch &fetch) {
    using namespace rt;
    for (int it = 0; it < budget; ++it) {
        const Node n = fetch(cur);
        if (n.b > 0) {
            for (int k = 0; k < n.b; ++k) {
                const int slot = n.a + k;
                const float *t = bvh.tris + 9 * slot;
                float th;
                if (ray_triangle(o, d, tnear, tfar, t, t + 3, t + 6, &th)) {
                    const int s = bvh.ids[2 * slot], p = bvh.ids[2 * slot + 1];
                    if (ANY) { best = Hit{th, s, p}; return true; }
                    if (closer(th, s, p, best)) best = Hit{th, s, p};
                }
            }
        } else {
            Node l, r;
            fetch.pair(n.a, l, r);
            const float lim = best.shape < 0 ? tfar : best.t * 1.0000004f + 1e-30f;
            float tl, tr;
            const bool hl = ray_box_once(o, inv, tnear, lim, l.lo, l.hi, &tl);
            const bool hr = ray_box_once(o, inv, tnear, lim, r.lo, r.hi, &tr);
            if (hl && hr) {
                int near = n.a, far = n.a + 1;
                if (tr < tl) { near = n.a + 1; far = n.a; }
                if (LDSN == 0 || sp < LDSN) stack[sp * 256] = (IDX)far; else spill[sp - LDSN] = far;
                ++sp;
                cur = near;
                continue;
            } else if (hl) { cur = n.a; continue; }
            else if (hr) { cur = n.a + 1; continue; }
        }
        if (sp == 0) return true;
        --sp;
        cur = (LDSN == 0 || sp < LDSN) ? (int)stack[sp * 256] : spill[sp - LDSN];
    }
    return false;
}

template <bool ANY, int STACK, class IDX, bool SORT>
__global__ void __launch_bounds__(256) __attribute__((amdgpu_waves_per_eu(STACK <= 16 ? 6 : (STACK <= 24 ? 7 : (STACK <= 32 ? 4 : 1)), 8))) trace_refill_kernel(rt::BvhD bvh, const rt::RayRec *__restrict__ rays, rt::HitRec *__restrict__ hits,
                                                           int n, const int *count, int rays_per_lane, int idle_min, int steps, int sort_mode) {
    if (count) { const int c = *count; n = c < n ? c : n; }
    const int chunk = 64 * rays_per_lane;
    if ((long long)blockIdx.x * 4 * chunk >= n) return;
    __shared__ IDX stack_tile[STACK * 256];
    IDX *stack = stack_tile + threadIdx.x;
    constexpr int kTop = (SORT && STACK == 32) ? 191 : kTopNodes;
    __shared__ rt::Node top[kTop + 1];
    __shared__ unsigned char order_tile[SORT ? 4 * 256 : 4];
    const int ntop = bvh.num_nodes < kTop ? bvh.num_nodes : kTop;
    if ((int)threadIdx.x < ntop) top[threadIdx.x] = bvh.nodes[threadIdx.x];
    __syncthreads();
    const FetchStaged fetch{bvh.nodes, (LdsFloats)(const float *)top, ntop};
    const int lane = threadIdx.x & 63, wave = threadIdx.x >> 6;
    const long long first = ((long long)blockIdx.x * 4 + wave) * chunk;
    if (first >= n) return;
    const int end = (int)(first + chunk < n ? first + chunk : n);
    unsigned char *order = order_tile + wave * 256;
    const bool sorted = SORT && sort_mode > 0 && rays_per_lane == 4;
    if (sorted) {
        const unsigned long long below = (1ull << lane) - 1ull;
        unsigned keys = 0;
#pragma unroll
        for (int j = 0; j < 4; ++j) {
            const long long r = first + 64 * j + lane;
            unsigned key = 255u;
            if (r < end) {
                const rt::RayRec ray = rays[r];
                if (ray.tmax < 0.f) key = 254u;
                else {
                    const unsigned oct = (ray.dx < 0.f ? 1u : 0u) | (ray.dy < 0.f ? 2u : 0u) | (ray.dz < 0.f ? 4u : 0u);
                    const unsigned gray = oct ^ (oct >> 1);
                    key = gray;
                    if (sort_mode >= 2) {
                        const float ax = fabsf(ray.dx), ay = fabsf(ray.dy), az = fabsf(ray.dz);
                        const unsigned axis = ax >= ay ? (ax >= az ? 0u : 2u) : (ay >= az ? 1u : 2u);
                        key = gray * 3u + ((gray & 1u) ? 2u - axis : axis);
                    }
                }
            }
            keys |= key << (8 * j);
        }
        const int nbins = sort_mode >= 2 ? 24 : 8;
        int off = 0;
        for (int b = 0; b <= nbins; ++b) {
            const unsigned want = b == nbins ? 254u : (unsigned)b;
#pragma unroll
            for (int j = 0; j < 4; ++j) {
                const bool in = ((keys >> (8 * j)) & 255u) == want;
                const unsigned long long m = __ballot(in);
                if (in) order[off + __popcll(m & below)] = (unsigned char)(64 * j + lane);
                off += __popcll(m);
            }
        }
        __builtin_amdgcn_fence(__ATOMIC_SEQ_CST, "wavefront");
        __builtin_amdgcn_wave_barrier();
    }
    int next = (int)first;
    bool live = false;
    int slot = 0, cur = 0, sp = 0;
    rt::Hit best{0.f, -1, -1};
    float o[3] = {0, 0, 0}, d[3] = {1, 1, 1}, inv[3] = {1, 1, 1}, tmin = 0, tmax = -1;
    constexpr int kLdsN = (STACK == kHybridLds && sizeof(IDX) == 4) ? kHybridLds : 0;
    int spill[kLdsN > 0 ? kHybridSpill : 1];
    for (;;) {
        const unsigned long long idle = __ballot(!live);
        const int nidle = __popcll(idle);
        if (next < end && (nidle >= idle_min || nidle == 64)) {
            if (!live) {
                int r = next + __popcll(idle & ((1ull << lane) - 1ull));
                if (r < end) {
                    if (SORT && sorted) r = (int)first + (int)order[r - (int)first];
                    const rt::RayRec ray = rays[r];
                    slot = r; cur = 0; sp = 0;
                    o[0] = ray.ox; o[1] = ray.oy; o[2] = ray.oz; d[0] = ray.dx; d[1] = ray.dy; d[2] = ray.dz;
                    inv[0] = 1.f / d[0]; inv[1] = 1.f / d[1]; inv[2] = 1.f / d[2];
                    tmin = ray.tmin; tmax = ray.tmax;
                    best = rt::Hit{tmax, -1, -1};
                    bool miss = tmax < 0.f || bvh.num_nodes == 0;
                    if (!miss) { float tn; const rt::Node root = fetch(0); miss = !rt::ray_box(o, inv, tmin, tmax, root.lo, root.hi, &tn); }
                    if (miss) hits[r] = rt::HitRec{-1, -1}; else live = true;
                }
            }
            next += nidle;
        }
        if (__ballot(live) == 0ull) { if (next >= end) break; continue; }
        if (live) {
            if (traverse_some<ANY, IDX, kLdsN>(bvh, o, d, inv, tmin, tmax, stack, spill, best, cur, sp, steps, fetch)) {
                hits[slot] = rt::HitRec{best.shape, best.shape >= 0 ? best.prim : -1};
                live = false;
            }
        }
    }
}

hipStream_t side_stream(int k) {
    static thread_local hipStream_t streams[16][4] = {};
    int dev = 0;
    (void)hipGetDevice(&dev);
    hipStream_t &s = streams[dev & 15][k & 3];
    if (!s) {
        static const bool allowed = std::getenv("RDR_NO_SIDE_PRIORITY") == nullptr;
        int least = 0, greatest = 0;
        if ((k & 2) && allowed && hipDeviceGetStreamPriorityRange(&least, &greatest) == hipSuccess && least != greatest)
            check(hipStreamCreateWithPriority(&s, hipStreamNonBlocking, least), "hipStreamCreateWithPriority");
        else
            check(hipStreamCreateWithFlags(&s, hipStreamNonBlocking), "hipStreamCreate");
    }
    return s;
}

int *new_count() {
    static thread_local int *rings[16] = {};
    static thread_local int slots[16] = {};
    constexpr int kRing = 8192;
    int dev = 0;
    (void)hipGetDevice(&dev);
    int *&ring = rings[dev & 15];
    int &slot = slots[dev & 15];
    if (!ring) ring = (int *)dmalloc(sizeof(int) * kRing);
    int *p = ring + slot;
    slot = (slot + 1) % kRing;
    return p;
}

int *persistent_counter() {
    static thread_local int *rings[16] = {};
    static thread_local int slots[16] = {};
    constexpr int kRing = 4096;
    int dev = 0;
    (void)hipGetDevice(&dev);
    int *&ring = rings[dev & 15];
    int &slot = slots[dev & 15];
    if (!ring) ring = (int *)dmalloc(sizeof(int) * kRing);
    int *p = ring + slot;
    slot = (slot + 1) % kRing;
    check(hipMemsetAsync(p, 0, sizeof(int), ctx().stream), "persistent_counter");
    return p;
}

namespace {
struct Pending { hipEvent_t a, b; bool any; };
std::mutex g_stats_lock;
std::vector<Pending> g_pending;
std::vector<hipEvent_t> g_free_events;
unsigned long long *g_counters = nullptr;

hipEvent_t get_event() {
    if (!g_free_events.empty()) { hipEvent_t e = g_free_events.back(); g_free_events.pop_back(); return e; }
    hipEvent_t e;
    check(hipEventCreate(&e), "hipEventCreate");
    return e;
}
}

TraceStats &trace_stats() { static TraceStats s; return s; }

void trace_stats_collect() {
    TraceStats &st = trace_stats();
    std::lock_guard<std::mutex> lk(g_stats_lock);
    if (!g_pending.empty()) {
        check(hipDeviceSynchronize(), "stats sync");
        std::vector<std::pair<double, double>> iv[2];
        const hipEvent_t ref = g_pending.front().a;
        for (Pending &p : g_pending) {
            float ms = 0, at = 0;
            check(hipEventElapsedTime(&ms, p.a, p.b), "hipEventElapsedTime");
            (p.any ? st.any_ms : st.closest_ms) += ms;
            if (p.a != ref && hipEventElapsedTime(&at, ref, p.a) != hipSuccess) { (void)hipGetLastError(); at = 0.f; }
            iv[p.any ? 1 : 0].push_back({(double)at, (double)at + (double)ms});
        }
        for (int k = 0; k < 2; ++k) {
            std::sort(iv[k].begin(), iv[k].end());
            double busy = 0, lo = 0, hi = -1;
            for (const auto &x : iv[k]) {
                if (hi < lo || x.first > hi) { if (hi >= lo) busy += hi - lo; lo = x.first; hi = x.second; }
                else if (x.second > hi) hi = x.second;
            }
            if (hi >= lo) busy += hi - lo;
            (k ? st.any_union_ms : st.closest_union_ms) += busy;
        }
        for (Pending &p : g_pending) { g_free_events.push_back(p.a); g_free_events.push_back(p.b); }
        g_pending.clear();
    }
    if (g_counters) {
        unsigned long long c[8] = {0, 0, 0, 0, 0, 0, 0, 0};
        download(c, g_counters, sizeof(c));
        st.nodes[0] += c[0]; st.tris[0] += c[1]; st.nodes[1] += c[2]; st.tris[1] += c[3];
        st.wide_nodes[0] += c[6]; st.wide_nodes[1] += c[7];
        st.closest_rays += c[4]; st.any_rays += c[5];
        zero(g_counters, sizeof(c));
        sync();
    }
}

namespace {
unsigned long long *counter_base(bool any) {
    std::lock_guard<std::mutex> lk(g_stats_lock);
    if (!g_counters) {
        g_counters = (unsigned long long *)dmalloc(64);
        check(hipMemset(g_counters, 0, 64), "hipMemset");
    }
    return any ? g_counters + 2 : g_counters;
}

template <bool V> using Bool = std::bool_constant<V>;
template <int V> using Int = std::integral_constant<int, V>;
template <class F> void by_bool(bool b, F f) { if (b) f(Bool<true>{}); else f(Bool<false>{}); }
template <int... TIERS, class F> void by_stack(int stack, F f) {
    if (!((stack == TIERS && (f(Int<TIERS>{}), true)) || ...)) throw std::logic_error("trace: the plan names a stack tier its kernel family does not have");
}
template <class F> void wide_case(const TracePlan &p, bool any, F f) {
    by_bool(any, [&](auto a) { by_bool(p.counting, [&](auto c) { by_stack<12, 16, 20, 24, 32, kWideStackMax>(p.stack, [&](auto st) { f(a, c, st); }); }); });
}
template <class F> void refill_case(const TracePlan &p, bool any, F f) {
    by_bool(any, [&](auto a) { by_bool(p.sorted, [&](auto so) {
        if (p.short_index) by_stack<24>(p.stack, [&](auto st) { f(a, st, Bool<true>{}, so); });
        else by_stack<kHybridLds, 32, rt::kTraverseStack>(p.stack, [&](auto st) { f(a, st, Bool<false>{}, so); });
    }); });
}
template <class F> void plain_case(const TracePlan &p, bool any, F f) {
    by_bool(any, [&](auto a) { by_bool(p.counting, [&](auto c) { by_stack<16, 24, 32, rt::kTraverseStack>(p.stack, [&](auto st) {
        by_bool(p.short_index, [&](auto sh) { by_bool(p.stage_top, [&](auto top) { f(a, c, st, sh, top); }); }); }); }); });
}
template <bool SHORT> using StackIndex = std::conditional_t<SHORT, unsigned short, int>;
}

void trace(const rt::BvhD &bvh, const rt::RayRec *rays, rt::HitRec *hits, Count cnt, bool any, bool coherent) {
    const int n = cnt.upper;
    const int *n_dev = cnt.dev;
    if (n <= 0) return;
    TraceStats &st = trace_stats();
    hipStream_t s = ctx().stream;
    const TracePlan plan = plan_trace(trace_facts(bvh), n, any, coherent, st.counting, rdr::tuning());
    Pending p{};
    if (st.timing) {
        { std::lock_guard<std::mutex> lk(g_stats_lock); p.a = get_event(); p.b = get_event(); }
        p.any = any;
        check(hipEventRecord(p.a, s), "hipEventRecord");
    }
    const dim3 grid(plan.blocks), block(256);
    unsigned long long *ctr = plan.counting ? counter_base(any) : nullptr;
    switch (plan.form) {
    case TraceForm::Wide:
        wide_case(plan, any, [&](auto a, auto c, auto stack) {
            hipLaunchKernelGGL((trace_wide_kernel<a, c, stack>), grid, block, 0, s, bvh, rays, hits, n, n_dev, ctr);
        });
        break;
    case TraceForm::Refill:
        refill_case(plan, any, [&](auto a, auto stack, auto sh, auto sorted) {
            hipLaunchKernelGGL((trace_refill_kernel<a, stack, StackIndex<sh>, sorted>), grid, block, 0, s, bvh, rays, hits, n, n_dev,
                               plan.rays_per_lane, plan.idle_min, plan.steps, plan.sort_mode);
        });
        break;
    case TraceForm::Plain:
        plain_case(plan, any, [&](auto a, auto c, auto stack, auto sh, auto top) {
            hipLaunchKernelGGL((trace_kernel<a, c, stack, StackIndex<sh>, top>), grid, block, 0, s, bvh, rays, hits, n, n_dev, ctr);
        });
        break;
    }
    check(hipGetLastError(), "trace launch");
    if (st.timing) check(hipEventRecord(p.b, s), "hipEventRecord");
    std::lock_guard<std::mutex> lk(g_stats_lock);
    if (st.timing) g_pending.push_back(p);
    (any ? st.any_launches : st.closest_launches)++;
    if (!plan.counting) (any ? st.any_rays : st.closest_rays) += (uint64_t)n;
}

}
```

### redner_amd/csrc/render.cpp

```cpp
#include "render.h"
#include "tuning.h"
#include <atomic>
#include <exception>
#include <cstdio>
#include <cstdlib>
#include "stages_fwd.h"
#include "stages_bwd.h"
#include "stages_edge.h"
#include "grad_store.h"
#include <algorithm>
#include <memory>
#include <stdexcept>
#include <type_traits>
#include <vector>

namespace rdr {

namespace {

inline bool overlap_on() { return !tuning().has(RDR_TUNE_NO_OVERLAP); }


VSlice make_slice(Arena &a, int n, bool with_occl, bool with_rdiff = true) {
    VSlice v;
    v.n = n;
    v.ray = a.get<double>((size_t)6 * n);
    v.rdiff = with_rdiff ? a.get<double>((size_t)12 * n) : nullptr;
    v.shape = a.get<int>(n); v.tri = a.get<int>(n);
    v.thr = a.get<double>((size_t)3 * n);
    v.mrough = a.get<double>(n);
    v.occl = with_occl ? a.get<unsigned char>(n) : nullptr;
    v.erd = nullptr; v.erd_touched = nullptr; v.erd_seg = nullptr; v.erd_S = 0; v.erd_P0 = 0;
    return v;
}

struct Queues {
    rt::RayRec *nee, *bsdf;
    rt::HitRec *h_nee, *h_bsdf;
    int *pos[2];
};

struct BounceChain {
    bool fused = false;
    bool have_rays = false;
    const int *qpos = nullptr;
    exec::Count queue_n{0};
    int flip = 0;
};

struct ChannelLayout { int nd, radiance_dim; ChannelsD ch; };
ChannelLayout layout_of(const rdr_render_options &o, int max_generic) {
    ChannelLayout l;
    l.nd = 0; l.radiance_dim = -1;
    if (o.num_channels > kMaxChannels) throw std::runtime_error("render: too many channels");
    if (max_generic > kMaxGeneric) throw std::runtime_error("render: generic textures wider than 16 channels are not supported");
    l.ch.n = o.num_channels; l.ch.max_generic = max_generic; l.ch.radiance_off = -1;
    l.ch.id = nullptr;
    l.ch.radiance_only = o.num_channels == 1 && o.channels[0] == RDR_CH_RADIANCE;
    int d = 0;
    for (int i = 0; i < o.num_channels; ++i) {
        if (o.channels[i] == RDR_CH_RADIANCE) {
            if (l.radiance_dim != -1) throw std::runtime_error("Duplicated radiance channel");
            l.radiance_dim = i;
            l.ch.radiance_off = d;
        }
        int one = o.channels[i];
        int w = compute_num_channels(&one, 1, max_generic);
        if (w < 0) throw std::runtime_error("render: unknown channel id");
        d += w;
    }
    l.nd = d;
    l.ch.nd = d; l.ch.radiance_dim = l.radiance_dim;
    return l;
}

void debug_dump(const char *tag, int sample, int depth, const void *dev_ptr, size_t bytes) {
    static const char *dir = std::getenv("RDR_DEBUG_DUMP");
    if (!dir || !dev_ptr) return;
    std::vector<char> host(bytes);
    exec::download(host.data(), dev_ptr, bytes);
    char path[1024];
    std::snprintf(path, sizeof(path), "%s/%s_s%d_d%d.bin", dir, tag, sample, depth);
    if (FILE *f = std::fopen(path, "wb")) { std::fwrite(host.data(), 1, bytes, f); std::fclose(f); }
}

uint64_t pcg_stream_seed(const rdr_render_options &o) {
    return (uint64_t)o.seed + (uint64_t)o.sample_offset * 0x9E3779B97F4A7C15ULL;
}

bool scene_is_lean(const Scene &scene, const ChannelsD &ch) {
    const CameraD &c = scene.d.cam;
    return scene.d.envmap == nullptr && c.kind == kCamPerspective && !c.distortion.defined && ch.radiance_only &&
           !scene.has_mipmaps && !scene.has_textures && !scene.has_vertex_colors;
}

constexpr int kGeneral = 0, kLean = 1, kMid = 2;
int scene_kind(const Scene &scene, const ChannelsD &ch) {
    if (tuning().has(RDR_TUNE_FORCE_GENERAL)) return kGeneral;
    if (scene_is_lean(scene, ch)) return kLean;
    const CameraD &c = scene.d.cam;
    if (scene.d.envmap == nullptr && c.kind == kCamPerspective && !c.distortion.defined && ch.radiance_only) return kMid;
    return kGeneral;
}
template <class F, class Go> void with_kind(int kind, const F &f, Go &&go) {
    if (kind == kLean) go(LeanStage<F>{f});
    else if (kind == kMid) go(MidStage<F>{f});
    else go(f);
}
template <class W, class Go> void with_walk_kind(int kind, const W &w, Go &&go) {
    if (kind == kLean) go(LeanWalk<W>{w});
    else if (kind == kMid) go(MidWalk<W>{w});
    else go(w);
}
template <class F> void launch_v(int kind, exec::Count n, const F &f) {
    with_kind(kind, f, [&](const auto &k) { exec::launch(n, k); });
}

inline int side_index(int k, int lanes) { return lanes >= (1 << 19) ? k + 2 : k; }
struct Fork {
    exec::Fence from, done;
    bool marked = false, pending = false;
    void mark() { from.after(exec::ctx().stream); marked = true; }
    void join() { if (pending) done.gate(exec::ctx().stream); pending = false; }
    template <class Work> void run(hipStream_t side, Work &&work) {
        if (!marked) mark();
        marked = false;
        from.gate(side);
        exec::StreamScope on(side);
        work();
        done.after(side);
        pending = true;
    }
};
template <class Work> void beside(Fork &fork, bool aside, int k, int lanes, Work &&work) {
    if (aside) fork.run(exec::side_stream(side_index(k, lanes)), work);
    else work();
}

inline bool fuse_bounces(bool pcg, int kind, int chain_lanes) {
    return !pcg && kind == kLean && chain_lanes <= (1 << 19) && !tuning().has(RDR_TUNE_NO_FUSED_BOUNCE);
}
constexpr int kEmitterTestMax = 8;
struct Bounce {
    SamplerD rng{}; int dim = 0, rng_shift = 0;
    const int *active = nullptr; exec::Count num_active{0};
    int *next_active = nullptr;
    const VSlice *v = nullptr, *vn = nullptr, *vnn = nullptr;
    const Queues *q = nullptr;
    Sink sink{};
    int *dyn = nullptr; int dyn_inc = 0;
    bool shadow_rays_coherent = false, last_bounce = false, next_is_last = false;
    BounceChain *chain = nullptr;
    Fork *shadow_fork = nullptr;
};
exec::Count run_bounce(const Scene &scene, const SceneD &sd, const Bounce &b) {
    const VSlice &v = *b.v, &vn = *b.vn;
    const Queues &q = *b.q;
    BounceChain *chain = b.chain;
    const int lean = scene_kind(scene, b.sink.ch);
    const bool fused = chain && chain->fused;
    const bool drawn = fused && chain->have_rays;
    const exec::Count queue_n = drawn ? chain->queue_n : b.num_active;
    const int *qpos = drawn ? chain->qpos : nullptr;
    const bool emitter_test = lean == kLean && scene.emitter_triangles > 0 && scene.emitter_triangles <= kEmitterTestMax &&
                              !tuning().has(RDR_TUNE_TRACE_EVERY_CONTINUATION);
    if (!drawn) {
        BounceSample bs{sd, b.rng, b.dim, b.rng_shift, b.active, v, vn, q.nee, q.bsdf};
        bs.last_bounce_emitters = b.last_bounce && emitter_test;
        launch_v(lean, b.num_active, bs);
    }
    beside(*b.shadow_fork, overlap_on(), 1, b.num_active.upper, [&] {
        exec::trace(scene.bvh, q.nee, q.h_nee, queue_n, true, b.shadow_rays_coherent);
    });
    exec::trace(scene.bvh, q.bsdf, q.h_bsdf, queue_n, false);
    b.shadow_fork->join();
    const BounceContrib contrib{sd, b.rng, b.dim, b.rng_shift, b.active, v, vn, q.h_nee, q.h_bsdf, b.sink};
    if (!fused) {
        launch_v(lean, b.num_active, contrib);
        return exec::compact_dev(b.active, b.num_active, b.next_active, KeepHit{vn.shape}, nullptr, b.dyn, b.dyn_inc);
    }
    if (b.vnn) {
        BounceSample next{sd, b.rng, b.dim + 7, b.rng_shift, b.active, vn, *b.vnn, q.nee, q.bsdf};
        next.last_bounce_emitters = b.next_is_last && emitter_test;
        launch_v(lean, b.num_active, BounceContribSample{contrib, next, qpos});
    } else if (qpos) {
        launch_v(lean, b.num_active, BounceContribSample{contrib, BounceSample{sd, b.rng, b.dim + 7, b.rng_shift, b.active, vn, vn, nullptr, nullptr}, qpos, 1});
    } else {
        launch_v(lean, b.num_active, contrib);
    }
    int *pos_out = q.pos[chain->flip];
    chain->flip ^= 1;
    const exec::Count next = exec::compact_dev(b.active, b.num_active, b.next_active, KeepHit{vn.shape}, nullptr, b.dyn, b.dyn_inc, pos_out);
    chain->have_rays = b.vnn != nullptr;
    chain->qpos = pos_out;
    chain->queue_n = b.num_active;
    return next;
}

struct BatchView { int S = 1, P0 = 0, rows = 0; bool on = false; };

struct Worker {
    Arena arena;
    std::vector<VSlice> vs;
    int *active = nullptr;
    Queues q;
    std::vector<exec::Count> num_active;
    int *main_dyn = nullptr;
    int *seg = nullptr;
    float *stage = nullptr;
    Fork shadow_fork;
};

struct Backward {
    const Scene &scene; const rdr_render_options &opt;
    Worker &w;
    int stride, B;
    const float *d_image; float *screen_grad; double weight; int nd, radiance_dim;
    BatchView batch;
    SceneD sd;
    GradStore &grads;
    Arena arena;
    AdjState adj;
    int adj_point_doubles = kAdjPointDoubles;

    ChannelsD ch;
    int lean = kGeneral;
    uint64_t *pcg_edge = nullptr;
    int *edge_dyn = nullptr;
    int *hoist_dyn = nullptr;
    double *multipliers = nullptr;

    VSlice ea, eb;
    int chain_n = 0;
    double *erd_chain = nullptr;
    int *deferred = nullptr, *deferred_seg = nullptr, *deferred_count = nullptr, *prim_dyn = nullptr;
    int *elist[3] = {nullptr, nullptr, nullptr};
    HLeaf *h_leaves = nullptr, *h_spill = nullptr;
    int *nee_act = nullptr;
    HDescent *h_descent = nullptr;
    GatherShared gshared{nullptr, nullptr, nullptr, nullptr, 0, 0};
    GatherCand *gather_cands = nullptr;
    int *nee_slots = nullptr;
    double *edge_contrib = nullptr, *edge_tmin = nullptr, *hit_pos = nullptr;
    unsigned char *hp_written = nullptr; int *hp_violations = nullptr;
    HitEvent *hp_events = nullptr; int *hp_event_count = nullptr; int hp_event_cap = 0;
    double *hp_carry = nullptr;
    unsigned char *replay_live = nullptr;
    PrimaryEdgeRec *prim_recs = nullptr;
    SecondaryEdgeRec *sec_recs = nullptr;
    SecPick *sec_picks = nullptr;
    unsigned char *sec_mode = nullptr;
    Sink esink{}, psink{};

    Fork walk_fork;
    Fork pickh_fork;
    Fork adjoint_fork;
    const bool overlap = overlap_on();
    const bool has_lights = sd.num_lights > 0;
    const int dim0 = opt.sample_pixel_center ? 0 : 2;
    bool edges_on() const { return prim_recs != nullptr; }
    bool secondary_on() const { return edges_on() && scene.use_secondary_edges; }

    int sample_id = 0;
    int lanes = 0;
    int cur_S = 1;
    SamplerD rng{}, rng_edge{};
    int edim = 0;
    bool hoisted = false;
    SecEdgeArgs early_sa{};

    Backward(const Scene &scene_, const rdr_render_options &opt_, GradStore &grads_, Worker &w_, int P, int B_,
             const float *d_image_, float *screen_grad_, double weight_, int nd_, int radiance_dim_, const ChannelsD &ch_,
             const BatchView &batch_)
        : scene(scene_), opt(opt_), w(w_), stride(P), B(B_), d_image(d_image_), screen_grad(screen_grad_), weight(weight_),
          nd(nd_), radiance_dim(radiance_dim_), batch(batch_), sd(scene_.d), grads(grads_), ch(ch_) {
        if (batch.on) sd.cam.batch_rows = batch.rows;
        lean = scene_kind(scene, ch);
        adj.n = P; adj.plain = 0;
        adj.thr = arena.get<double>((size_t)3 * P);
        adj.ray_dir = arena.get<double>((size_t)3 * P);
        adj_point_doubles = lean == kLean ? kAdjPointDoublesLean : kAdjPointDoubles;
        adj.point = arena.get<double>((size_t)adj_point_doubles * P);
        adj.carries = scene.d.envmap == nullptr ? arena.get<unsigned char>((size_t)P) : nullptr;
        nee_act = arena.get<int>((size_t)P);
        const bool use_edges = scene.edges && scene.edges->d.num_edges > 0 &&
                              (scene.use_primary_edges || scene.use_secondary_edges);
        if (use_edges) {
            edge_dyn = arena.get<int>(kMaxBatch);
            hoist_dyn = arena.get<int>(kMaxBatch);
            const int L = 2 * P;
            ea = make_slice(arena, L, false, lean != kLean);
            eb = make_slice(arena, L, false, lean != kLean);
            if (scene.has_mipmaps) {
                ea.erd = eb.erd = arena.get<double>((size_t)12 * L);
                exec::zero(ea.erd, sizeof(double) * 12 * L);
                if (batch.on) {
                    chain_n = 2 * batch.P0;
                    ea.erd_touched = eb.erd_touched = arena.get<unsigned char>(L);
                    erd_chain = arena.get<double>((size_t)12 * chain_n);
                    exec::zero(erd_chain, sizeof(double) * 12 * chain_n);
                    deferred = arena.get<int>(L);
                    deferred_seg = arena.get<int>(kMaxBatch + 1);
                    deferred_count = arena.get<int>(kMaxBatch);
                    prim_dyn = arena.get<int>(kMaxBatch);
                }
            }
            for (int k = 0; k < 3; ++k) elist[k] = arena.get<int>(L);
            nee_slots = arena.get<int>(P);
            gather_cands = arena.get<GatherCand>((size_t)kGatherCands * P);
            gshared.book = arena.get<GatherBook>(1);
            gshared.heavy_cap = (int)std::min<long long>(std::max<long long>((long long)P / 256, kGatherHeavyCap), kGatherHeavyMax);
            gshared.work_cap = (int)std::min<long long>(std::max<long long>((long long)P / 32, kGatherWorkCap), kGatherWorkMax);
            gshared.heavy_slot = arena.get<int>(gshared.heavy_cap);
            gshared.work = arena.get<GatherWork>(gshared.work_cap);
            gshared.cands_big = arena.get<GatherCand>((size_t)kGatherCandsBig * gshared.heavy_cap);
            if (tuning().gather_heavy_cap >= 0) gshared.heavy_cap = std::min(tuning().gather_heavy_cap, gshared.heavy_cap);
            if (tuning().gather_work_cap >= 0) gshared.work_cap = std::min(tuning().gather_work_cap, gshared.work_cap);
            h_leaves = arena.get<HLeaf>((size_t)kHSamples * P);
            h_spill = arena.get<HLeaf>((size_t)(kHSamples - kHStackLds) * P);
            h_descent = arena.get<HDescent>((size_t)P);
            edge_contrib = arena.get<double>(L);
            edge_tmin = arena.get<double>(L);
            hit_pos = arena.get<double>((size_t)3 * L);
            exec::zero(hit_pos, sizeof(double) * 3 * L);
            if (batch.on && scene.d.envmap != nullptr) {
                hp_written = arena.get<unsigned char>(L);
                hp_violations = arena.get<int>(1);
                exec::zero(hp_violations, sizeof(int));
                hp_event_cap = L;
                hp_events = arena.get<HitEvent>((size_t)hp_event_cap);
                if (tuning().stale_event_cap >= 0) hp_event_cap = std::min(tuning().stale_event_cap, hp_event_cap);
                hp_event_count = arena.get<int>(1);
                exec::zero(hp_event_count, sizeof(int));
                hp_carry = arena.get<double>((size_t)3 * 2 * batch.P0);
                exec::zero(hp_carry, sizeof(double) * 3 * 2 * batch.P0);
                replay_live = arena.get<unsigned char>(P);
            }
            prim_recs = arena.get<PrimaryEdgeRec>(P);
            sec_recs = arena.get<SecondaryEdgeRec>(P);
            sec_picks = arena.get<SecPick>(P);
            sec_mode = arena.get<unsigned char>(P);
            if (!ch.radiance_only) multipliers = arena.get<double>((size_t)L * nd);
            if (opt.sampler_type == RDR_SAMPLER_INDEPENDENT) {
                pcg_edge = arena.get<uint64_t>(P);
                exec::launch(P, PcgInit{pcg_edge, pcg_stream_seed(opt) + 131071U});
            }
        }
        esink = Sink{nullptr, edge_contrib, nd, radiance_dim, weight, ch, nullptr};
        psink = Sink{nullptr, edge_contrib, nd, radiance_dim, weight, ch, multipliers};
    }

    bool chain_mode() const { return erd_chain != nullptr; }
    void erd_view(const int *seg) { ea.erd_seg = eb.erd_seg = seg; ea.erd_S = eb.erd_S = cur_S; ea.erd_P0 = eb.erd_P0 = batch.P0; }
    HitPosView hit_view(const int *seg, int depth = 0) const {
        return HitPosView{hit_pos, ea.n, hp_written ? seg : nullptr, cur_S, batch.P0, hp_written, hp_violations,
                          hp_events, hp_event_count, hp_event_cap, depth};
    }
    const int *seg_of(int d) const { return batch.on ? w.seg + (size_t)d * (kMaxBatch + 1) : nullptr; }
    const int *active_of(int d) const { return w.active + (size_t)d * stride; }

    void edge_rng_consumed(exec::Count n, int count, const int *gate = nullptr) {
        if (pcg_edge) exec::launch(n, PcgAdvance{pcg_edge, count, nullptr, gate});
    }
    SamplerD edge_rng_at(int edim_at, const int *dyn = nullptr, const int *seg = nullptr) const {
        SamplerD r = rng_edge; r.pcg_base = edim_at; r.dyn = dyn ? dyn : edge_dyn;
        if (batch.on) { r.batch = cur_S; r.seg = seg; r.batch_lanes = seg ? 0 : batch.P0; }
        return r;
    }
    void secondary_pass_consumed(exec::Count n, int d) {
        if (batch.on) exec::launch(cur_S, BumpDynSeg{edge_dyn, seg_of(d), 4});
        else exec::launch(1, BumpDyn{edge_dyn, n.dev, 4});
        edge_rng_consumed(n, 4);
    }
    void clear_adjoint_records() {
        exec::zero(adj.thr, sizeof(double) * 3 * stride);
        exec::zero(adj.ray_dir, sizeof(double) * 3 * stride);
        exec::zero(adj.point, sizeof(double) * adj_point_doubles * stride);
    }

    bool large_forms() const { return tuning().has(RDR_TUNE_LARGE_FORMS) || lanes >= (1 << 19); }
    bool nee_compact() const { return !tuning().has(RDR_TUNE_NO_NEE_COMPACT) && large_forms(); }

    void pick_lists(const SecEdgeArgs &sa, exec::Count nA, bool with_descent, exec::Count &nH, exec::Count &nN) {
        launch_v(lean, nA, SecEdgeSetup{sa, sec_mode, sec_recs, sec_picks, ea, edge_tmin, with_descent ? h_descent : nullptr});
        nH = exec::compact_dev((const int *)nullptr, nA, elist[0], KeepMode{sec_mode, 1});
        const exec::Count nN2 = exec::compact_dev((const int *)nullptr, nA, nee_slots, KeepMode{sec_mode, 2});
        nN = exec::compact_dev((const int *)nullptr, nA, nee_slots, KeepMode{sec_mode, 3}, &nN2);
    }
    void launch_pick_n(int need, exec::Count nN, const SecEdgeArgs &sa) {
        const bool walk_all = tuning().has(RDR_TUNE_PICKN_WALK);
        const bool gather = !walk_all && sa.es.gather.num_nodes > 0;
        if (gather) {
            const int gneed = sa.es.gather.stack_need;
            exec::zero(gshared.book, sizeof(GatherBook));
            auto passes = [&](auto tag) {
                constexpr int NS = decltype(tag)::value;
                const int budget = tuning().gather_budget;
                launch_v(lean, nN, SecEdgeGatherN<NS>{sa, nee_slots, sec_picks, gather_cands, gshared, budget});
                launch_v(lean, gshared.work_cap, SecEdgeGatherSub<NS>{sa, nee_slots, gshared});
                launch_v(lean, gshared.heavy_cap, SecEdgeGatherReplay{sa, nee_slots, sec_picks, gshared});
            };
            if (gneed <= 24) passes(std::integral_constant<int, 24>{});
            else if (gneed <= 40) passes(std::integral_constant<int, 40>{});
            else passes(std::integral_constant<int, 64>{});
        }
        const int only_overflow = gather ? 1 : 0;
        const int *walk_needed = gather ? &gshared.book->walk_needed : nullptr;
        auto go = [&](auto walk) {
            walk.walk_needed = walk_needed;
            with_walk_kind(lean, walk, [&](const auto &k) { exec::launch_persistent(nN, k); });
        };
        if (need <= 24) go(SecEdgePickNWalk<24>{sa, nee_slots, sec_picks, only_overflow});
        else if (need <= 32) go(SecEdgePickNWalk<32>{sa, nee_slots, sec_picks, only_overflow});
        else if (need <= 48) go(SecEdgePickNWalk<48>{sa, nee_slots, sec_picks, only_overflow});
        else go(SecEdgePickNWalk<64>{sa, nee_slots, sec_picks, only_overflow});
    }
    void pick_hierarchical(const SecEdgeArgs &sa, exec::Count nH, bool fused, bool one_launch) {
        const bool lazy = tuning().has(RDR_TUNE_PICKH_LAZY);
        const int pickh_k = tuning().pickh_k, pickh_idle = tuning().pickh_idle, pickh_steps = tuning().pickh_steps;
        if (fused) launch_v(lean, nH, SecEdgePickH{sa, elist[0], sec_picks});
        else if (one_launch && lazy) launch_v(lean, nH, SecEdgePickH2<false>{sa, elist[0], sec_picks, h_leaves, h_spill, nH.upper});
        else if (one_launch) launch_v(lean, nH, SecEdgePickH2<true>{sa, elist[0], sec_picks, h_leaves, h_spill, nH.upper});
        else {
            auto descend = [&](auto walk) {
                with_walk_kind(lean, walk, [&](const auto &k) { exec::launch_chunked(nH, k, pickh_k, pickh_idle, pickh_steps); });
            };
            if (lazy) descend(SecEdgePickHDescend<false>{sa.es, elist[0], h_leaves, h_spill, h_descent, nH.upper});
            else descend(SecEdgePickHDescend<true>{sa.es, elist[0], h_leaves, h_spill, h_descent, nH.upper});
            static const bool leaves_walk = std::getenv("RDR_PICKH_LEAVES_WALK") != nullptr;
            if (leaves_walk)
                with_walk_kind(lean, SecEdgePickHLeavesWalk{sa.sc, sa.es, elist[0], sec_picks, h_leaves, h_descent, nH.upper},
                               [&](const auto &k) { exec::launch_chunked(nH, k, pickh_k, pickh_idle, 2); });
            else
                launch_v(lean, nH, SecEdgePickHLeaves{sa, elist[0], sec_picks, h_leaves, h_descent, nH.upper});
        }
    }
    SecEdgeArgs start_picks(int d, int edim_d, const int *dyn, bool early, bool side) {
        const bool fused = tuning().has(RDR_TUNE_PICKH_FUSED);
        const bool one_launch = tuning().has(RDR_TUNE_PICKH_ONE_LAUNCH) || !large_forms();
        const exec::Count nA = w.num_active[d];
        const EdgeSceneD &es = scene.edges->d;
        const SecEdgeArgs sa{sd, es, rng, dim0 + 7 * d, edge_rng_at(edim_d, dyn, seg_of(d)), edim_d, active_of(d), w.vs[d]};
        const int need = es.max_stack;
        exec::Count nH(0), nN(0);
        if (early) {
            beside(walk_fork, true, 1, lanes, [&] {
                pick_lists(sa, nA, !(fused || one_launch), nH, nN);
                pickh_fork.mark();
                launch_pick_n(need, nN, sa);
            });
            beside(pickh_fork, true, 0, lanes, [&] { pick_hierarchical(sa, nH, fused, one_launch); });
        } else {
            pick_lists(sa, nA, !(fused || one_launch), nH, nN);
            beside(walk_fork, side, 1, lanes, [&] { launch_pick_n(need, nN, sa); });
            pick_hierarchical(sa, nH, fused, one_launch);
        }
        return sa;
    }
    void join_picks() { walk_fork.join(); pickh_fork.join(); }

    void hoist_first_vertex_picks() {
        const bool hoist_allowed = !tuning().has(RDR_TUNE_NO_HOIST);
        if (!(hoist_allowed && secondary_on() && overlap && scene.diffuse_only && pcg_edge == nullptr && has_lights && B >= 2 &&
              w.num_active[0].upper > 0)) return;
        int host_part = 0, k = 0;
        bool first = true;
        if (batch.on) {
            CountLiveDepthsSeg cl{hoist_dyn, {}, 0, 4, 0};
            auto flush_tables = [&] { cl.n = k; cl.add = first ? 0 : 1; exec::launch(cur_S, cl); first = false; k = 0; };
            for (int d = B - 1; d >= 1; --d) {
                if (w.num_active[d].upper <= 0) continue;
                cl.seg[k++] = seg_of(d);
                if (k == kDepthGates) flush_tables();
            }
            if (k > 0 || first) flush_tables();
        } else {
            CountLiveDepths cl{hoist_dyn, {}, 0, 4, 0};
            auto flush_gates = [&] { cl.n = k; cl.add = first ? 0 : 1; exec::launch(1, cl); first = false; k = 0; };
            for (int d = B - 1; d >= 1; --d) {
                if (w.num_active[d].upper <= 0) continue;
                if (!w.num_active[d].dev) { host_part += 4; continue; }
                cl.gate[k++] = w.num_active[d].dev;
                if (k == kDepthGates) flush_gates();
            }
            if (k > 0 || first) flush_gates();
            if (host_part) exec::launch(1, BumpDyn{hoist_dyn, nullptr, host_part});
        }
        early_sa = start_picks(0, 0, hoist_dyn, true, true);
        hoisted = true;
    }

    void adj_nee(const AdjBounceArgs &ba, exec::Count nA, int d) {
        if (!nee_compact() || !w.vs[d].occl) { launch_v(lean, nA, AdjBounceNee{ba}); return; }
        AdjBounceArgs lit = ba;
        const exec::Count nLit = exec::compact_dev(ba.active, nA, nee_act, KeepNeeLive{w.vs[d].occl}, nullptr, nullptr, 0, nullptr, 1);
        lit.active = nee_act;
        launch_v(lean, nLit, AdjBounceNee{lit});
    }
    void adj_scatter(const AdjBounceArgs &ba, exec::Count nA, int d) {
        AdjBounceArgs part = ba;
        exec::Count n = nA;
        if (!nee_compact()) {
            if (sd.envmap == nullptr) { part.active = active_of(d + 1); n = w.num_active[d + 1]; }
        } else if (adj.carries) {
            n = exec::compact_dev(active_of(d + 1), w.num_active[d + 1], nee_act,
                                  KeepCarryingContinuation{adj.carries, w.vs[d + 1].shape, sd.shapes}, nullptr, nullptr, 0, nullptr, 1);
            part.active = nee_act;
        } else if (d == B - 1) {
            n = exec::compact_dev(ba.active, nA, nee_act, KeepLitContinuation{w.vs[d + 1].shape, sd.shapes, sd.envmap != nullptr},
                                  nullptr, nullptr, 0, nullptr, 1);
            part.active = nee_act;
        }
        launch_v(lean, n, AdjBounceScatter{part});
    }

    void trace_edge_paths(exec::Count n_act, exec::Count n_slots, int first_depth, bool need_lights, const int *seg = nullptr, int *dyn = nullptr) {
        if (!dyn) dyn = edge_dyn;
        if (need_lights && !has_lights) return;
        int cur = 1;
        BounceChain chain;
        chain.fused = fuse_bounces(pcg_edge != nullptr, lean, n_act.upper);
        for (int depth = first_depth, k = 0; depth < B && n_act.upper > 0; ++depth, ++k) {
            const VSlice &m = (k % 2 == 0) ? ea : eb;
            const VSlice &nx = (k % 2 == 0) ? eb : ea;
            int nxt = (cur == 1) ? 2 : 1;
            Bounce b;
            b.rng = edge_rng_at(edim, dyn, seg); b.dim = edim; b.rng_shift = 1;
            b.active = elist[cur]; b.num_active = n_act; b.next_active = elist[nxt];
            b.v = &m; b.vn = &nx; b.vnn = depth + 1 < B ? &m : nullptr;
            b.q = &w.q; b.sink = esink;
            b.dyn = batch.on ? nullptr : dyn; b.dyn_inc = 7;
            b.last_bounce = depth == B - 1; b.next_is_last = depth + 2 == B;
            b.chain = &chain; b.shadow_fork = &w.shadow_fork;
            const exec::Count next = run_bounce(scene, sd, b);
            if (batch.on) exec::launch(cur_S, BumpDynList{dyn, elist[cur], n_act.dev, n_act.upper, seg, 2 * batch.P0, 7});
            edge_rng_consumed(n_slots, 7, n_act.dev);
            n_act = next;
            cur = nxt;
        }
    }

    void begin_sample(int sample_id_, const SamplerD &main_rng, int n_lanes, int S_now) {
        sample_id = sample_id_; lanes = n_lanes; cur_S = S_now;
        rng = main_rng;
        rng_edge = SamplerD{scene.sobol_table, opt.seed + 131071U, sample_id, pcg_edge, 0};
        edim = 0;
        hoisted = false;
        if (edge_dyn) exec::zero(edge_dyn, sizeof(int) * kMaxBatch);
        if (chain_mode()) exec::zero(ea.erd_touched, (size_t)ea.n);
        if (hp_written) exec::zero(hp_written, (size_t)ea.n);
        clear_adjoint_records();
        if (adj.carries) exec::zero(adj.carries, (size_t)stride);
    }

    void sweep_depth(int d) {
        const exec::Count nA = w.num_active[d];
        if (nA.upper <= 0) return;
        const AdjBounceArgs ba{sd, grads.g, rng, dim0 + 7 * d, active_of(d), w.vs[d], w.vs[d + 1], d_image, nd, radiance_dim, weight, adj};
        bool with_edges = secondary_on();
        if (with_edges && d > 0 && scene.diffuse_only) {
            with_edges = false;
            secondary_pass_consumed(nA, d);
        }
        const bool early_here = hoisted && d == 0;
        const bool side = overlap && with_edges && !early_here;
        beside(adjoint_fork, side, 0, lanes, [&] {
            adj_scatter(ba, nA, d);
            adj_nee(ba, nA, d);
        });
        if (with_edges) secondary_edge_pass(d, nA, early_here, side);
    }
    void secondary_edge_pass(int d, exec::Count nA, bool early_here, bool side) {
        const exec::Count edge_lanes = exec::scaled_count(nA, 2);
        if (chain_mode()) erd_view(seg_of(d));
        const SecEdgeArgs sa = early_here ? early_sa : start_picks(d, edim, nullptr, false, side);
        join_picks();
        debug_dump("sec_mode", sample_id, d, sec_mode, (size_t)nA.upper);
        debug_dump("sec_picks", sample_id, d, sec_picks, sizeof(SecPick) * (size_t)nA.upper);
        launch_v(lean, nA, SecEdgeFinish{sa, sec_mode, sec_picks, d_image, nd, radiance_dim, sec_recs, ea, edge_tmin});
        debug_dump("sec_recs", sample_id, d, sec_recs, sizeof(SecondaryEdgeRec) * (size_t)nA.upper);
        secondary_pass_consumed(nA, d);
        const exec::Count n0 = exec::compact_dev((const int *)nullptr, edge_lanes, elist[0], KeepNonZeroDir{ea.ray, ea.n});
        exec::launch(n0, QueueRays{elist[0], ea, edge_tmin, w.q.bsdf});
        exec::trace(scene.bvh, w.q.bsdf, w.q.h_bsdf, n0, false);
        exec::launch(n0, RecordHits{elist[0], ea, w.q.h_bsdf});
        if (ea.erd) exec::launch(n0, MirrorSurfDiff{sd, elist[0], ea});
        launch_v(lean, nA, SecondaryEdgeWeights{sd, sec_recs, ea, hit_view(seg_of(d))});
        exec::zero(edge_contrib, sizeof(double) * edge_lanes.upper);
        launch_v(lean, n0, ShadeRecorded{sd, elist[0], ea, esink});
        const exec::Count n1 = exec::compact_dev(elist[0], n0, elist[1], KeepHit{ea.shape});
        trace_edge_paths(n1, nA, d + 1, false, seg_of(d));
        adjoint_fork.join();
        exec::launch(nA, SecondaryEdgeDerivatives{sd, grads.g, active_of(d), sec_recs, hit_view(seg_of(d), d), edge_contrib, adj});
    }

    void camera_vertex_adjoint() {
        const bool aside = overlap && screen_grad == nullptr && edges_on() && scene.use_primary_edges;
        beside(adjoint_fork, aside, 0, lanes, [&] {
            launch_v(lean, lanes, AdjPrimary{sd, grads.g, rng, opt.sample_pixel_center, w.vs[0], d_image, nd, radiance_dim, weight, adj, screen_grad, ch});
        });
    }
    void primary_sub_paths(int *list, exec::Count n, const double *chain, int *dyn) {
        if (ea.erd) exec::launch(n, LoadLaneDiff{list, ea, chain, chain_n, 2 * batch.P0});
        exec::launch(n, QueueRays{list, ea, nullptr, w.q.bsdf});
        exec::trace(scene.bvh, w.q.bsdf, w.q.h_bsdf, n, false);
        launch_v(lean, n, ShadePrimary{sd, list, ea, w.q.h_bsdf, psink});
        if (ea.erd) exec::launch(n, MirrorSurfDiff{sd, list, ea});
        const exec::Count n1 = exec::compact_dev(list, n, elist[1], KeepHit{ea.shape});
        trace_edge_paths(n1, lanes, 0, true, nullptr, dyn);
    }
    void primary_edge_pass() {
        const EdgeSceneD &es = scene.edges->d;
        const int edge_lanes = 2 * lanes;
        exec::zero(edge_contrib, sizeof(double) * edge_lanes);
        erd_view(nullptr);
        SamplePrimaryEdges spe{sd, es, edge_rng_at(edim), edim, d_image, nd, radiance_dim, prim_recs, ea, multipliers};
        if (chain_mode()) spe.batch_P0 = batch.P0;
        launch_v(lean, lanes, spe);
        edim += 2;
        edge_rng_consumed(lanes, 2);
        const exec::Count n0 = exec::compact_dev((const int *)nullptr, edge_lanes, elist[0], KeepNonZeroDir{ea.ray, ea.n});
        if (!chain_mode()) {
            primary_sub_paths(elist[0], n0, nullptr, nullptr);
        } else {
            exec::copy_dev(prim_dyn, edge_dyn, sizeof(int) * kMaxBatch);
            const exec::Count nA = exec::compact_dev(elist[0], n0, elist[2], KeepTouched{ea.erd_touched, 1});
            const exec::Count nD = exec::compact_dev(elist[0], n0, deferred, KeepTouched{ea.erd_touched, 0});
            exec::launch(cur_S + 1, SegOffsets{deferred, nD.dev, nD.upper, 2 * batch.P0, cur_S, deferred_seg});
            static const bool tell_chain = std::getenv("RDR_DEBUG_BATCH") != nullptr;
            if (tell_chain) std::fprintf(stderr, "[render] chain mode: %d of %d primary-edge lanes need the previous sample's scratch (sequential part)\n",
                                         exec::read_count(nD), exec::read_count(n0));
            primary_sub_paths(elist[2], nA, nullptr, nullptr);
            for (int k = 0; k < cur_S; ++k) {
                exec::launch(2 * batch.P0, ExtractSegment{deferred, deferred_seg, k, elist[0], deferred_count + k});
                primary_sub_paths(elist[0], exec::Count(deferred_count + k, 2 * batch.P0), erd_chain, prim_dyn);
                exec::launch(chain_n, ChainAdvance{erd_chain, chain_n, ea.erd, ea.n, ea.erd_touched, k});
            }
        }
        launch_v(lean, lanes, PrimaryEdgeDerivatives{sd, grads.g, prim_recs, edge_contrib, screen_grad});
    }

    void replay_stale_hits() {
        clear_adjoint_records();
        exec::zero(replay_live, (size_t)stride);
        const exec::Count n_events(hp_event_count, hp_event_cap);
        for (int d = B - 1; d >= 0; --d) {
            if (w.num_active[d].upper <= 0) continue;
            const AdjBounceArgs ba{sd, grads.g, rng, dim0 + 7 * d, active_of(d), w.vs[d], w.vs[d + 1], d_image, nd, radiance_dim, 0.0, adj};
            launch_v(lean, w.num_active[d], AdjBounceScatterLive{AdjBounceScatter{ba}, replay_live});
            exec::launch(n_events, InjectHitEvents{sd, grads.g, hp_events, d, hit_pos, ea.n, hp_written, hp_carry, 2 * batch.P0, adj, replay_live});
        }
        launch_v(lean, lanes, AdjPrimaryLive{AdjPrimary{sd, grads.g, rng, opt.sample_pixel_center, w.vs[0], d_image, nd, radiance_dim, 0.0,
                                                        adj, screen_grad, ch}, replay_live});
        exec::launch(2 * batch.P0, HitPosCarryAdvance{hp_carry, 2 * batch.P0, cur_S, hit_pos, ea.n, hp_written});
        exec::zero(hp_event_count, sizeof(int));
    }

    void run_sample(int sample_id_, const SamplerD &main_rng, int n_lanes, int S_now) {
        begin_sample(sample_id_, main_rng, n_lanes, S_now);
        hoist_first_vertex_picks();
        for (int d = B - 1; d >= 0 && has_lights; --d) sweep_depth(d);
        camera_vertex_adjoint();
        if (edges_on() && scene.use_primary_edges) primary_edge_pass();
        adjoint_fork.join();
        if (hp_events) replay_stale_hits();
    }
};

struct RestartUnbatched {};
std::atomic<uint64_t> g_unbatchable{0};
uint64_t scene_shape_key(const Scene &scene) {
    uint64_t h = 1469598103934665603ULL;
    auto mix = [&](uint64_t v) { h = (h ^ v) * 1099511628211ULL; };
    mix(scene.shapes.size());
    for (const ShapeD &sh : scene.shapes) { mix((uint64_t)sh.num_vertices); mix((uint64_t)sh.num_triangles); }
    mix(scene.materials.size()); mix(scene.lights.size());
    mix((uint64_t)scene.h_envmap.values.width[0]); mix((uint64_t)scene.h_envmap.values.height[0]);
    return h | 1;
}
BatchView choose_batch(const rdr_render_options &opt, const Tuning &tune, int P, int rows, int lean, int nd,
                       bool samples_independent, bool forward_batches, bool gradient) {
    const int B = opt.max_bounces;
    BatchView batch;
    batch.P0 = P; batch.rows = rows;
    if (!samples_independent && !forward_batches) return batch;
    const int batch_cap = std::min(kMaxBatch, tune.batch_samples);
    const long long total = (long long)opt.num_samples * P;
    int want = opt.num_samples;
    if (total > (1 << 17) && samples_independent) want = (opt.num_samples + 1) / 2;
    long long lane_cap = tune.batch_lanes;
    if (lane_cap == 0) {
        lane_cap = 1LL << 24;
        if (total > (1LL << 22) && exec::memory_held_by_others() > 0.10) lane_cap = 1LL << 22;
    }
    batch.S = std::max(1, std::min(std::min(batch_cap, want), (int)std::max(1LL, lane_cap / P)));
    auto bytes_needed = [&](int S_try) {
        const double lanes = (double)S_try * P;
        const int wk = !samples_independent ? 1 : (tune.workers > 0 ? tune.workers : 2);
        double per_lane = (lean == kLean ? 260.0 * (B + 1) + 660.0 : 400.0 * (B + 1) + 1200.0) * wk;
        if (forward_batches) per_lane += 4.0 * nd * (B + 1);
        if (gradient) per_lane += 4.0 * nd;
        return per_lane * lanes;
    };
    if (tune.batch_lanes == 0 && tune.mem_available_mb < 0) {
        const double cap = (double)exec::pool_cap_bytes();
        while (batch.S > 1 && bytes_needed(batch.S) > cap) --batch.S;
    }
    if (tune.mem_available_mb >= 0 || bytes_needed(batch.S) > 1073741824.0) {
        const double room = 0.8 * (tune.mem_available_mb >= 0 ? tune.mem_available_mb * 1048576.0 : (double)exec::memory_available());
        while (batch.S > 1 && bytes_needed(batch.S) > room) batch.S = (batch.S + 1) / 2;
    }
    batch.on = batch.S > 1;
    return batch;
}

const int *upload_assign_flags(Arena &arena, const rdr_render_options &opt, int max_generic, int nd) {
    std::vector<int> flags((size_t)nd, 0);
    int at = 0;
    bool any_id = false;
    for (int k = 0; k < opt.num_channels; ++k) {
        int one = opt.channels[k];
        const int w = compute_num_channels(&one, 1, max_generic);
        if (one >= RDR_CH_SHAPE_ID) { for (int j = 0; j < w; ++j) flags[at + j] = 1; any_id = true; }
        at += w;
    }
    if (!any_id) return nullptr;
    int *d_flags = arena.get<int>(flags.size());
    exec::upload(d_flags, flags.data(), sizeof(int) * flags.size());
    return d_flags;
}

void render_once(const Scene &scene, const rdr_render_options &opt, float *image, const float *d_image,
                 const rdr_dscene_desc *d_scene, float *screen_gradient_image, const Tuning &tune, bool envmap_batches) {
    if (opt.sampler_type != RDR_SAMPLER_SOBOL && opt.sampler_type != RDR_SAMPLER_INDEPENDENT)
        throw std::runtime_error("render: unknown sampler type");
    if (d_image && !d_scene) throw std::runtime_error("render: d_rendered_image given without d_scene");
    const CameraD &cam = scene.d.cam;
    const int P = (cam.vp_x1 - cam.vp_x0) * (cam.vp_y1 - cam.vp_y0);
    if (P <= 0) return;
    const int B = opt.max_bounces;
    if (B < 0) throw std::runtime_error("render: max_bounces must be >= 0");
    ChannelLayout lay = layout_of(opt, scene.max_generic_texture_dimension);
    if (lay.radiance_dim < 0 && B > 0)
        throw std::runtime_error("render: max_bounces > 0 needs the radiance channel (the reference writes path "
                                 "contributions at the radiance offset, src/path_contribution.cpp:127-129)");
    const int total_spp = opt.total_samples > 0 ? opt.total_samples : opt.num_samples;
    const double weight = 1.0 / total_spp;
    const bool has_lights = scene.d.num_lights > 0;
    if (2 + 7 * B > kSamplerDims) throw std::runtime_error("render: max_bounces exceeds the Sobol' table");

    PhaseTimer timer(d_image ? "render (backward)" : "render (forward)");
    Arena arena;
    {
        int *ids = arena.get<int>(kMaxChannels);
        exec::upload(ids, opt.channels, sizeof(int) * opt.num_channels);
        lay.ch.id = ids;
    }
    std::unique_ptr<GradStore> grads;
    if (d_image) grads.reset(new GradStore(scene, *d_scene, (size_t)P * (size_t)opt.num_samples));

    uint64_t *pcg_main = nullptr;
    if (opt.sampler_type == RDR_SAMPLER_INDEPENDENT) {
        pcg_main = arena.get<uint64_t>(P);
        exec::launch(P, PcgInit{pcg_main, pcg_stream_seed(opt)});
    }
    const int lean = scene_kind(scene, lay.ch);

    const bool sobol_plain = screen_gradient_image == nullptr && opt.sampler_type == RDR_SAMPLER_SOBOL && !timer.on;
    const bool no_edge_passes = !scene.use_primary_edges && !scene.use_secondary_edges;
    const bool chain = (scene.has_mipmaps || scene.d.envmap != nullptr) && !no_edge_passes;
    const bool batchable = sobol_plain && (lean == kLean || no_edge_passes || scene.d.envmap == nullptr || envmap_batches);
    const bool samples_independent = batchable && d_image != nullptr && image == nullptr;
    const bool forward_batches = sobol_plain && d_image == nullptr && image != nullptr;
    const BatchView batch = choose_batch(opt, tune, P, cam.vp_y1 - cam.vp_y0, lean, lay.nd, samples_independent, forward_batches, d_image != nullptr);
    const int S = batch.S;
    const int PL = S * P;
    static const bool tell = std::getenv("RDR_DEBUG_BATCH") != nullptr;
    if (tell) std::fprintf(stderr, "[render] %s: %d samples of %d lanes in batches of %d\n", d_image ? "backward" : "forward", opt.num_samples, P, S);
    const int num_batches = (opt.num_samples + S - 1) / S;
    const float *d_image_lanes = d_image;
    if (batch.on && d_image) {
        float *rep = arena.get<float>((size_t)PL * lay.nd);
        for (int k = 0; k < S; ++k)
            exec::copy_dev(rep + (size_t)k * P * lay.nd, d_image, sizeof(float) * (size_t)P * lay.nd);
        d_image_lanes = rep;
    }
    const int *assign_flags = batch.on && forward_batches && !lay.ch.radiance_only ? upload_assign_flags(arena, opt, scene.max_generic_texture_dimension, lay.nd) : nullptr;
    int workers = 1;
    if (samples_independent) workers = std::max(1, std::min(tune.workers > 0 ? tune.workers : exec::sample_workers(PL, num_batches, batch.on), num_batches));
    if (chain) workers = 1;
    if (d_image != nullptr) { last_schedule()[0].store(S); last_schedule()[1].store(workers); }

    struct SampleWorker : Worker { std::unique_ptr<Backward> bwd; };
    auto make_worker = [&](SampleWorker &w) {
        w.vs.resize(B + 1);
        for (int d = 0; d <= B; ++d) w.vs[d] = make_slice(w.arena, PL, d < B && d_image_lanes != nullptr, lean != kLean);
        w.active = w.arena.get<int>((size_t)(B + 1) * PL);
        w.q.nee = w.arena.get<rt::RayRec>((size_t)2 * PL); w.q.bsdf = w.arena.get<rt::RayRec>((size_t)2 * PL);
        w.q.h_nee = w.arena.get<rt::HitRec>((size_t)2 * PL); w.q.h_bsdf = w.arena.get<rt::HitRec>((size_t)2 * PL);
        w.q.pos[0] = w.arena.get<int>((size_t)2 * PL); w.q.pos[1] = w.arena.get<int>((size_t)2 * PL);
        w.num_active.assign(B + 2, exec::Count(0));
        if (pcg_main) w.main_dyn = w.arena.get<int>(1);
        if (batch.on) w.seg = w.arena.get<int>((size_t)(B + 1) * (kMaxBatch + 1));
        if (batch.on && forward_batches) w.stage = w.arena.get<float>((size_t)(B + 1) * PL * lay.nd);
    };
    auto run_samples = [&](SampleWorker &w, int first, int stride) {
        std::vector<VSlice> &vs = w.vs;
        int *active = w.active;
        const Queues &q = w.q;
        std::vector<exec::Count> &num_active = w.num_active;
        SceneD sd = scene.d;
        if (batch.on) sd.cam.batch_rows = batch.rows;
        for (int b = first; b < num_batches; b += stride) {
            const int s = b * S;
            const int S_now = std::min(S, opt.num_samples - s);
            const int lanes = S_now * P;
            const int sample_id = opt.sample_offset + s;
            SamplerD rng{scene.sobol_table, opt.seed, sample_id, pcg_main, 0};
            if (batch.on) { rng.batch = S_now; rng.batch_lanes = P; }
            Sink sink{image, nullptr, lay.nd, lay.radiance_dim, weight, lay.ch, nullptr};
            const size_t plane = (size_t)PL * lay.nd;
            auto sink_of = [&](int launch) { Sink k = sink; if (w.stage) k.image = w.stage + (size_t)launch * plane; return k; };
            if (w.stage) exec::zero(w.stage, sizeof(float) * plane * (B + 1));
            auto segments = [&](int d) {
                if (batch.on) exec::launch(S_now + 1, SegOffsets{active + (size_t)d * PL, num_active[d].dev, num_active[d].upper, P, S_now,
                                                                 w.seg + (size_t)d * (kMaxBatch + 1)});
            };

            launch_v(lean, lanes, GenPrimary{sd, rng, opt.sample_pixel_center, vs[0], q.bsdf});
            exec::trace(scene.bvh, q.bsdf, q.h_bsdf, lanes, false, true);
            launch_v(lean, lanes, ShadePrimary{sd, nullptr, vs[0], q.h_bsdf, sink_of(0)});
            std::fill(num_active.begin(), num_active.end(), exec::Count(0));
            num_active[0] = exec::compact_dev((const int *)nullptr, lanes, active, KeepHit{vs[0].shape});
            if (d_image) segments(0);
            if (w.main_dyn) exec::zero(w.main_dyn, sizeof(int));

            int dim = opt.sample_pixel_center ? 0 : 2;
            const int dim_first = dim;
            BounceChain chain;
            chain.fused = fuse_bounces(pcg_main != nullptr, lean, 2 * lanes);
            for (int d = 0; d < B && num_active[d].upper > 0 && has_lights; ++d) {
                Bounce bounce;
                bounce.rng = rng; bounce.dim = dim;
                bounce.active = active + (size_t)d * PL; bounce.num_active = num_active[d]; bounce.next_active = active + (size_t)(d + 1) * PL;
                bounce.v = &vs[d]; bounce.vn = &vs[d + 1]; bounce.vnn = d + 1 < B ? &vs[d + 2] : nullptr;
                bounce.q = &q; bounce.sink = sink_of(d + 1);
                bounce.dyn = w.main_dyn; bounce.dyn_inc = 7;
                bounce.shadow_rays_coherent = d == 0;
                bounce.last_bounce = d == B - 1; bounce.next_is_last = d + 2 == B;
                bounce.chain = &chain; bounce.shadow_fork = &w.shadow_fork;
                num_active[d + 1] = run_bounce(scene, sd, bounce);
                if (num_active[d + 1].dev && d_image) segments(d + 1);
                dim += 7;
            }
            if (w.stage) exec::launch(P * lay.nd, ResolveBatchImage{image, w.stage, P, lay.nd, S_now, B + 1, plane, assign_flags, vs[0].shape});

            if (d_image && !w.bwd) {
                scene.edge_data();
                w.bwd.reset(new Backward(scene, opt, *grads, w, PL, B, d_image_lanes, screen_gradient_image, weight, lay.nd, lay.radiance_dim, lay.ch, batch));
            }
            if (w.bwd) w.bwd->run_sample(sample_id, rng, lanes, S_now);
            if (w.bwd && w.bwd->hp_violations && (b == first || b + stride >= num_batches)) {
                int bad = 0;
                exec::download(&bad, w.bwd->hp_violations, sizeof(int));
                if (bad > 0) throw RestartUnbatched();
            }
            if (pcg_main) exec::launch(P, PcgAdvance{pcg_main, dim_first, w.main_dyn, nullptr});
        }
    };

    SampleWorker w0;
    make_worker(w0);
    if (timer.on) exec::sync();
    timer.lap("buffers, accumulators");
    if (workers == 1) {
        run_samples(w0, 0, 1);
    } else {
        exec::sync();
        for (int k = 1; k < workers; ++k)
            exec::SecondThread::get(k - 1).start([&, k] {
                TuningScope helper_scope(tune);
                SampleWorker w;
                make_worker(w);
                run_samples(w, k, workers);
                exec::sync();
            });
        std::exception_ptr failure;
        try { run_samples(w0, 0, workers); } catch (...) { failure = std::current_exception(); }
        for (int k = 1; k < workers; ++k) {
            try { exec::SecondThread::get(k - 1).wait(); } catch (...) { if (!failure) failure = std::current_exception(); }
        }
        if (failure) std::rethrow_exception(failure);
    }
    if (timer.on) exec::sync();
    timer.lap("samples");
    if (grads) grads->flush();
    exec::sync();
    timer.lap("gradient flush");
}

}

void render(const Scene &scene, const rdr_render_options &opt, float *image, const float *d_image,
            const rdr_dscene_desc *d_scene, float *screen_gradient_image, float * ) {
    const Tuning tune = resolve_tuning(opt.tuning);
    TuningScope tuning_scope(tune);
    const bool envmap_edges = scene.d.envmap != nullptr && d_image != nullptr && (scene.use_primary_edges || scene.use_secondary_edges);
    const uint64_t key = envmap_edges ? scene_shape_key(scene) : 0;
    bool optimistic = envmap_edges && g_unbatchable.load(std::memory_order_relaxed) != key;
    try {
        render_once(scene, opt, image, d_image, d_scene, screen_gradient_image, tune, optimistic);
    } catch (const RestartUnbatched &) {
        exec::device_sync();
        g_unbatchable.store(key, std::memory_order_relaxed);
        render_once(scene, opt, image, d_image, d_scene, screen_gradient_image, tune, false);
    }
}

namespace {
struct ScatterProbe {
    int op; bool plain;
    const unsigned char *active;
    double *const *dst;
    const int *shape, *tri;
    const double *val; int width;
    const ShapeD *shapes; const GShape *gshapes;
    RDR_FN void operator()(int i) const {
        if (!active[i]) return;
        const double *v = val + (size_t)width * i;
        switch (op) {
            case RDR_SCATTER_ACCUM: accum(dst[i], v[0]); break;
            case RDR_SCATTER_ACCUM_TEXEL: accum_texel(dst[i], v[0]); break;
            case RDR_SCATTER_ACCUM_PLAIN: accum_plain(dst[i], v[0]); break;
            case RDR_SCATTER_ACCUM_TRIPLE: accum_triple(dst[i], v[0], v[1], v[2]); break;
            case RDR_SCATTER_ACCUM_TEXEL_TRIPLE: accum_texel_triple(dst[i], v[0], v[1], v[2]); break;
            case RDR_SCATTER_TRIGRAD_WAVE: {
                TriGrad g;
#pragma unroll
                for (int k = 0; k < 3; ++k) {
                    g.p[k] = v3(v[3 * k], v[3 * k + 1], v[3 * k + 2]);
                    g.n[k] = v3(v[9 + 3 * k], v[10 + 3 * k], v[11 + 3 * k]);
                    g.uv[k] = v2(v[18 + 2 * k], v[19 + 2 * k]);
                    g.c[k] = v3(v[24 + 3 * k], v[25 + 3 * k], v[26 + 3 * k]);
                }
                scatter_trigrad_wave(shapes, gshapes, shape[i], tri[i], g, plain);
                break;
            }
            default: {
                const V3 pb[3] = {v3(v[0], v[1], v[2]), v3(v[3], v[4], v[5]), v3(v[6], v[7], v[8])};
                scatter_positions_wave(shapes, gshapes, shape[i], tri[i], pb);
                break;
            }
        }
    }
};
}

void debug_grad_scatter(const Scene &scene, const rdr_dscene_desc &ds, size_t job_samples, int op, bool plain, int num_lanes,
                        const uint8_t *active, const int32_t *target, const int32_t *index, const double *values) {
    const auto bad = [](const std::string &what) { throw std::runtime_error("rdr_debug_grad_scatter: " + what); };
    if (op < RDR_SCATTER_ACCUM || op > RDR_SCATTER_POSITIONS_WAVE) bad("unknown op");
    const bool tri_op = op >= RDR_SCATTER_TRIGRAD_WAVE;
    const int width = op == RDR_SCATTER_TRIGRAD_WAVE ? 33 : op == RDR_SCATTER_POSITIONS_WAVE ? 9 : op >= RDR_SCATTER_ACCUM_TRIPLE ? 3 : 1;
    if (num_lanes < 0 || num_lanes > (1 << 24)) bad("num_lanes out of range");
    if (num_lanes > 0 && (!active || !target || !values || (!tri_op && !index))) bad("a per-lane array is missing");

    GradStore grads(scene, ds, job_samples);
    const size_t n = (size_t)num_lanes;
    std::vector<double *> h_dst(n, nullptr);
    std::vector<int> h_shape(n, -1), h_tri(n, 0);
    if (tri_op) {
        for (size_t i = 0; i < n; ++i) {
            const int s = target[3 * i], t = target[3 * i + 1];
            const std::string lane = " (lane " + std::to_string(i) + ")";
            if (s >= (int)scene.shapes.size()) bad("shape out of range" + lane);
            if (s < 0) continue;
            const ShapeD &sh = scene.shapes[s];
            if (t < 0 || t >= sh.num_triangles) bad("triangle out of range" + lane);
            const int nuv = sh.num_uv_vertices > 0 ? sh.num_uv_vertices : sh.num_vertices;
            const int nn = sh.num_normal_vertices > 0 ? sh.num_normal_vertices : sh.num_vertices;
            for (int k = 0; k < 3; ++k) {
                const int vi = scene.h_indices[s][3 * (size_t)t + k];
                const int ui = sh.uv_indices ? scene.h_uv_indices[s][3 * (size_t)t + k] : vi;
                const int ni = sh.normal_indices ? scene.h_normal_indices[s][3 * (size_t)t + k] : vi;
                if (vi < 0 || vi >= sh.num_vertices || (sh.uvs && (ui < 0 || ui >= nuv)) || (sh.normals && (ni < 0 || ni >= nn)))
                    bad("corner index out of range" + lane);
            }
            h_shape[i] = s; h_tri[i] = t;
        }
    } else {
        GEnvmap h_envmap;
        if (grads.g.envmap) exec::download(&h_envmap, grads.g.envmap, sizeof(GEnvmap));
        const int elems = width;
        for (size_t i = 0; i < n; ++i) {
            const int kind = target[3 * i], a = target[3 * i + 1], b = target[3 * i + 2];
            const std::string lane = " (lane " + std::to_string(i) + ")";
            double *acc = nullptr;
            size_t count = 0;
            bool whole_block = false;
            switch (kind) {
                case RDR_TARGET_VERTICES: case RDR_TARGET_UVS: case RDR_TARGET_NORMALS: case RDR_TARGET_COLORS: {
                    if (a < 0 || a >= (int)grads.h_shapes.size()) bad("shape out of range" + lane);
                    const GShape &gs = grads.h_shapes[a];
                    acc = kind == RDR_TARGET_VERTICES ? gs.vertices : kind == RDR_TARGET_UVS ? gs.uvs : kind == RDR_TARGET_NORMALS ? gs.normals : gs.colors;
                    break;
                }
                case RDR_TARGET_TEXTURE: {
                    if (a < 0 || a >= (int)grads.h_materials.size()) bad("material out of range" + lane);
                    if (b < 0 || b >= 5 * kMaxMip) bad("texture level out of range" + lane);
                    const GMaterial &gm = grads.h_materials[a];
                    const GTex *tex[5] = {&gm.diffuse, &gm.specular, &gm.roughness, &gm.generic, &gm.normal_map};
                    acc = tex[b / kMaxMip]->texels[b % kMaxMip];
                    break;
                }
                case RDR_TARGET_LIGHTS:
                    acc = grads.g.light_intensity; count = 3 * scene.lights.size(); whole_block = true;
                    break;
                case RDR_TARGET_CAMERA: {
                    const GCamera &c = grads.g.cam;
                    double *const field[8] = {c.position, c.look, c.up, c.cam_to_world, c.world_to_cam, c.intrinsic_mat_inv, c.intrinsic_mat, c.distortion};
                    if (a < 0 || a >= 8) bad("camera field out of range" + lane);
                    acc = field[a];
                    break;
                }
                case RDR_TARGET_ENVMAP:
                    if (b < 0 || b >= kMaxMip) bad("texture level out of range" + lane);
                    if (grads.g.envmap) acc = h_envmap.values.texels[b];
                    break;
                default: bad("unknown target" + lane);
            }
            if (!acc) bad("the DScene has no such gradient tensor" + lane);
            if (!whole_block) {
                bool found = false;
                for (const GradStore::Pair &p : grads.pairs) if (p.acc == acc) { count = p.count; found = true; break; }
                if (!found) bad("target is not an accumulator of the store" + lane);
            }
            const long long at = index[i];
            if (at < 0 || (size_t)at + (size_t)elems > count) bad("element out of range" + lane);
            h_dst[i] = acc + at;
        }
    }

    struct Held {
        std::vector<void *> p;
        void *get(size_t bytes) { p.push_back(nullptr); p.back() = exec::dmalloc(bytes); return p.back(); }
        ~Held() { exec::device_sync(); for (void *q : p) exec::dfree(q); }
    } held;
    unsigned char *d_active = (unsigned char *)held.get(n);
    double **d_dst = (double **)held.get(sizeof(double *) * n);
    int *d_shape = (int *)held.get(sizeof(int) * n), *d_tri = (int *)held.get(sizeof(int) * n);
    double *d_val = (double *)held.get(sizeof(double) * n * width);
    exec::upload(d_active, active, n);
    exec::upload(d_dst, h_dst.data(), sizeof(double *) * n);
    exec::upload(d_shape, h_shape.data(), sizeof(int) * n);
    exec::upload(d_tri, h_tri.data(), sizeof(int) * n);
    exec::upload(d_val, values, sizeof(double) * n * width);
    exec::launch(exec::Count(num_lanes), ScatterProbe{op, plain, d_active, d_dst, d_shape, d_tri, d_val, width, scene.d.shapes, grads.g.shapes});
    grads.flush();
    exec::sync();
}

}

extern "C" int rdr_libm_exact(void) {
#ifdef RDR_PLATFORM_LIBM
    return 0;
#else
    return 1;
#endif
}
```

### redner_amd/csrc/tuning.h

```cpp
#pragma once
#include "../../include/redner_amd.h"
#include <atomic>
#include <cstdio>
#include <cstdlib>

namespace rdr {

struct Tuning {
    unsigned flags = 0;
    int batch_samples = 16;
    long long batch_lanes = 0;
    int workers = 0;
    int refill_k = 4, refill_idle = 24, refill_steps = 4;
    int wide_max = 1 << 19;
    int gather_budget = 256;
    int gather_heavy_cap = -1, gather_work_cap = -1;
    double mem_available_mb = -1.0;
    int refill_sort = 1;
    int pickh_k = 1, pickh_idle = 8, pickh_steps = 8;
    int stale_event_cap = -1;
    bool trace_hybrid = true;
    bool has(unsigned f) const { return (flags & f) != 0; }
};

namespace detail {
inline const char *env(const char *name) { return std::getenv(name); }
inline bool env_set(const char *name) { return std::getenv(name) != nullptr; }
struct EnvDefaults {
    unsigned flags = 0;
    int batch_samples = 0; long long batch_lanes = 0; int workers = 0;
    int refill_k = 0, refill_idle = 0, refill_steps = 0, wide_max = 0, gather_budget = 0, heavy_cap = -1, work_cap = -1;
    double mem_mb = -1.0;
    int refill_order = 0, pickh_k = 0, pickh_idle = 0, pickh_steps = 0;
    bool trace_hybrid = true;
    EnvDefaults() {
        if (env_set("RDR_NO_OVERLAP") || env_set("RDR_DEBUG_DUMP")) flags |= RDR_TUNE_NO_OVERLAP;
        if (env_set("RDR_FORCE_GENERAL")) flags |= RDR_TUNE_FORCE_GENERAL;
        if (env_set("RDR_PICKN_WALK")) flags |= RDR_TUNE_PICKN_WALK;
        if (env_set("RDR_PICKH_FUSED")) flags |= RDR_TUNE_PICKH_FUSED;
        if (env_set("RDR_PICKH_LAZY")) flags |= RDR_TUNE_PICKH_LAZY;
        if (env_set("RDR_NO_HOIST")) flags |= RDR_TUNE_NO_HOIST;
        if (env_set("RDR_TRACE_REFILL_ALL")) flags |= RDR_TUNE_REFILL_ALL;
        if (env_set("RDR_TRACE_BINARY")) flags |= RDR_TUNE_TRACE_BINARY;
        if (env_set("RDR_TRACE_NO_LDS_TOP")) flags |= RDR_TUNE_TRACE_NO_LDS_TOP;
        if (env_set("RDR_NO_FUSED_BOUNCE")) flags |= RDR_TUNE_NO_FUSED_BOUNCE;
        if (env_set("RDR_PICKH_ONE_LAUNCH")) flags |= RDR_TUNE_PICKH_ONE_LAUNCH;
        if (env_set("RDR_NO_NEE_COMPACT")) flags |= RDR_TUNE_NO_NEE_COMPACT;
        if (env_set("RDR_LARGE_FRAME_FORMS")) flags |= RDR_TUNE_LARGE_FORMS;
        if (env_set("RDR_TRACE_EVERY_CONTINUATION")) flags |= RDR_TUNE_TRACE_EVERY_CONTINUATION;
        if (const char *e = env("RDR_TRACE_REFILL")) {
            int k = 0, idle = 0, steps = 0;
            const int got = std::sscanf(e, "%d,%d,%d", &k, &idle, &steps);
            if (got >= 1 && k <= 0) flags |= RDR_TUNE_REFILL_OFF;
            if (got >= 1 && k > 0) refill_k = k;
            if (got >= 2 && idle > 0) refill_idle = idle;
            if (got >= 3 && steps > 0) refill_steps = steps;
        }
        if (const char *e = env("RDR_BATCH")) batch_samples = std::atoi(e);
        if (const char *e = env("RDR_BATCH_LANES")) batch_lanes = std::atoll(e);
        if (const char *e = env("RDR_WORKERS")) workers = std::atoi(e);
        if (const char *e = env("RDR_WIDE_MAX")) wide_max = std::atoi(e);
        if (const char *e = env("RDR_GATHER_BUDGET")) gather_budget = std::atoi(e);
        if (const char *e = env("RDR_GATHER_CAPS")) { int h = 0, w = 0; if (std::sscanf(e, "%d,%d", &h, &w) == 2) { heavy_cap = h; work_cap = w; } }
        if (const char *e = env("RDR_MEM_AVAILABLE_MB")) mem_mb = std::atof(e);
        if (const char *e = env("RDR_REFILL_SORT")) refill_order = std::atoi(e) + 1;
        if (const char *e = env("RDR_TRACE_HYBRID")) trace_hybrid = e[0] != '0';
        if (const char *e = env("RDR_PICKH_REFILL")) {
            int k = 0, idle = 0, steps = 0;
            const int got = std::sscanf(e, "%d,%d,%d", &k, &idle, &steps);
            if (got >= 1 && k > 0) pickh_k = k;
            if (got >= 2 && idle > 0) pickh_idle = idle;
            if (got >= 3 && steps > 0) pickh_steps = steps;
        }
    }
};
inline const EnvDefaults &env_defaults() { static const EnvDefaults d; return d; }
inline int clampi(long long v, long long lo, long long hi) { return (int)(v < lo ? lo : (v > hi ? hi : v)); }
}

inline Tuning resolve_tuning(const rdr_tuning *t) {
    const detail::EnvDefaults &e = detail::env_defaults();
    static const rdr_tuning zero{};
    const rdr_tuning &u = t ? *t : zero;
    Tuning r;
    r.flags = u.flags | e.flags;
    auto pick = [](long long field, long long env, long long dflt) { return field != 0 ? field : (env != 0 ? env : dflt); };
    r.batch_samples = detail::clampi(pick(u.batch_samples, e.batch_samples, 16), 1, 16);
    r.batch_lanes = pick(u.batch_lanes, e.batch_lanes, 0);
    if (r.batch_lanes < 0) r.batch_lanes = 1;
    r.workers = detail::clampi(pick(u.workers, e.workers, 0), 0, 4);
    r.refill_k = detail::clampi(pick(u.refill_rays_per_lane, e.refill_k, 4), 1, 64);
    r.refill_idle = detail::clampi(pick(u.refill_idle_lanes, e.refill_idle, 24), 1, 64);
    r.refill_steps = detail::clampi(pick(u.refill_steps, e.refill_steps, 4), 1, 1024);
    r.wide_max = (int)pick(u.wide_max_rays, e.wide_max, 1 << 19);
    r.gather_budget = detail::clampi(pick(u.gather_budget, e.gather_budget, 256), 1, 1 << 20);
    r.gather_heavy_cap = u.gather_heavy_cap_plus1 > 0 ? u.gather_heavy_cap_plus1 - 1 : e.heavy_cap;
    r.gather_work_cap = u.gather_work_cap_plus1 > 0 ? u.gather_work_cap_plus1 - 1 : e.work_cap;
    r.mem_available_mb = u.mem_available_mb > 0 ? (double)u.mem_available_mb : e.mem_mb;
    r.refill_sort = detail::clampi(pick(u.refill_order, e.refill_order, 2), 1, 3) - 1;
    r.pickh_k = detail::clampi(pick(u.pickh_slots_per_lane, e.pickh_k, 1), 1, 64);
    r.pickh_idle = detail::clampi(pick(u.pickh_idle_lanes, e.pickh_idle, 8), 1, 64);
    r.pickh_steps = detail::clampi(pick(u.pickh_steps, e.pickh_steps, 8), 1, 1024);
    r.stale_event_cap = u.stale_event_cap_plus1 > 0 ? u.stale_event_cap_plus1 - 1 : -1;
    r.trace_hybrid = e.trace_hybrid;
    return r;
}

inline std::atomic<int> *last_schedule() { static std::atomic<int> s[2]; return s; }

inline Tuning &tuning() {
    static thread_local Tuning t = resolve_tuning(nullptr);
    return t;
}
struct TuningScope {
    Tuning saved;
    explicit TuningScope(const Tuning &t) : saved(tuning()) { tuning() = t; }
    ~TuningScope() { tuning() = saved; }
    TuningScope(const TuningScope &) = delete;
};

inline std::atomic<unsigned> &build_flags_ref() { static std::atomic<unsigned> f{0}; return f; }
inline unsigned build_flags() {
    static const unsigned from_env = (detail::env_set("RDR_NO_REFIT") ? (unsigned)RDR_BUILD_NO_REFIT : 0u) |
                                     (detail::env_set("RDR_NO_EDGE_CACHE") ? (unsigned)RDR_BUILD_NO_EDGE_CACHE : 0u) |
                                     (detail::env_set("RDR_SYNC_EDGES") ? (unsigned)RDR_BUILD_SYNC_EDGES : 0u) |
                                     (detail::env_set("RDR_EDGE_HOST_BUILD") ? (unsigned)RDR_BUILD_EDGE_HOST_BUILD : 0u);
    return from_env | build_flags_ref().load(std::memory_order_relaxed);
}

}
```

Before: 86.37 Msamples/s.

## Size sample batches from an exact dry-run allocation count against the pool cap

Replaces the per-lane byte heuristic in batch selection with an exact count, made by running the worker and backward buffer allotment in a counting arena, and subtracts already-live pool bytes from the cap. It also preallocates the gradient flush segment arrays at layout time instead of per flush, skips queue position buffers when bounces cannot fuse, and orders image resolves across workers with fences. The aim is to pick batch sizes that fit the memory budget, and so avoid over-allocation or unnecessarily small batches, at the cost of extra host bookkeeping and a per-call pool simulation to report memory use.

```diff
diff --git a/include/redner_amd.h b/include/redner_amd.h
--- a/include/redner_amd.h
+++ b/include/redner_amd.h
@@ -222,6 +222,8 @@
 typedef struct rdr_debug_counters {
     uint64_t device_mallocs, host_count_reads;
     uint64_t last_batch_samples, last_workers;
+    uint64_t last_call_bytes;
+    uint64_t pool_peak_bytes;
 } rdr_debug_counters;
 void rdr_debug_counters_get(rdr_debug_counters *out);
 
diff --git a/redner_amd/_capi.py b/redner_amd/_capi.py
--- a/redner_amd/_capi.py
+++ b/redner_amd/_capi.py
@@ -119,7 +119,8 @@
 
 class DebugCounters(C.Structure):
     _fields_ = [('device_mallocs', C.c_uint64), ('host_count_reads', C.c_uint64),
-                ('last_batch_samples', C.c_uint64), ('last_workers', C.c_uint64)]
+                ('last_batch_samples', C.c_uint64), ('last_workers', C.c_uint64),
+                ('last_call_bytes', C.c_uint64), ('pool_peak_bytes', C.c_uint64)]
 
 
 class DeferredDesc(C.Structure):
diff --git a/redner_amd/csrc/capi.cpp b/redner_amd/csrc/capi.cpp
--- a/redner_amd/csrc/capi.cpp
+++ b/redner_amd/csrc/capi.cpp
@@ -8,6 +8,7 @@
 #include "vertex_normal.h"
 #include <cstdio>
 #include "scene.h"
+#include "pool_stats.h"
 #include <cstring>
 #include <exception>
 #include <mutex>
@@ -316,6 +317,8 @@
     out->host_count_reads = exec::host_count_reads();
     out->last_batch_samples = (uint64_t)rdr::last_schedule()[0].load();
     out->last_workers = (uint64_t)rdr::last_schedule()[1].load();
+    out->last_call_bytes = rdr::last_call_bytes().load();
+    out->pool_peak_bytes = (uint64_t)exec::pool_peak_bytes();
 }
 
 int rdr_debug_dump_edges(const rdr_scene *scene, const char *path) {
diff --git a/redner_amd/csrc/grad_store.h b/redner_amd/csrc/grad_store.h
--- a/redner_amd/csrc/grad_store.h
+++ b/redner_amd/csrc/grad_store.h
@@ -1,6 +1,7 @@
 #pragma once
 #include "scene.h"
 #include "stages_bwd.h"
+#include "pool_stats.h"
 #include <algorithm>
 #include <exception>
 #include <stdexcept>
@@ -10,7 +11,11 @@
 
 struct Arena {
     std::vector<void *> blocks;
+    bool counting = false;
+    size_t counted = 0;
+    std::vector<size_t> wants;
     template <class T> T *get(size_t count) {
+        if (counting) { wants.push_back(exec::pool_block_bytes(sizeof(T) * (count ? count : 1))); counted += wants.back(); return nullptr; }
         T *p = (T *)exec::pool_alloc(sizeof(T) * (count ? count : 1));
         blocks.push_back(p);
         return p;
@@ -32,6 +37,7 @@
     Tier tier[2];
     struct Pair { double *acc; float *out; size_t count; int tier; };
     std::vector<Pair> pairs;
+    FlushSegment *d_seg[2] = {nullptr, nullptr};
     bool counting = true;
 
     double *place(size_t count, int &t) {
@@ -83,6 +89,11 @@
                 throw std::runtime_error("render: gradient accumulator straddles a replica tier (GradStore::layout)");
         }
         accumulators_laid_out(tier[0].base, tier[0].stride);
+        for (int t = 0; t < 2; ++t) {
+            size_t n = 0;
+            for (const Pair &p : pairs) n += p.tier == t;
+            if (n) d_seg[t] = arena.get<FlushSegment>(n);
+        }
     }
     void layout(const Scene &scene, const rdr_dscene_desc &ds) {
         if (ds.num_shapes != (int)scene.shapes.size() || ds.num_materials != (int)scene.materials.size() ||
@@ -153,11 +164,10 @@
             if (seg.empty()) continue;
             std::sort(seg.begin(), seg.end(), [](const FlushSegment &a, const FlushSegment &b) { return a.begin < b.begin; });
             if (tr.stride > (size_t)0x7fffffff) throw std::runtime_error("render: gradient block too large");
-            FlushSegment *d_seg = arena.get<FlushSegment>(seg.size());
-            exec::upload(d_seg, seg.data(), sizeof(FlushSegment) * seg.size());
-            if (!aliased) exec::launch((int)tr.stride, FlushGrad{tr.base, tr.stride, tr.replicas, d_seg, (int)seg.size()});
+            exec::upload(d_seg[t], seg.data(), sizeof(FlushSegment) * seg.size());
+            if (!aliased) exec::launch((int)tr.stride, FlushGrad{tr.base, tr.stride, tr.replicas, d_seg[t], (int)seg.size()});
             else for (size_t i = 0; i < seg.size(); ++i)
-                exec::launch((int)(seg[i].begin + seg[i].count), FlushGrad{tr.base, tr.stride, tr.replicas, d_seg + i, 1});
+                exec::launch((int)(seg[i].begin + seg[i].count), FlushGrad{tr.base, tr.stride, tr.replicas, d_seg[t] + i, 1});
         }
         exec::set_replicas(ReplicaLayout{nullptr, 0, 0, 0, 0});
     }
diff --git a/redner_amd/csrc/hip/exec.h b/redner_amd/csrc/hip/exec.h
--- a/redner_amd/csrc/hip/exec.h
+++ b/redner_amd/csrc/hip/exec.h
@@ -3,6 +3,7 @@
 #include <stdint.h>
 #include <stdio.h>
 #include <atomic>
+#include <vector>
 #include <condition_variable>
 #include <cstdlib>
 #include <exception>
@@ -181,6 +182,10 @@
 void pool_set_cap(long long bytes);
 size_t pool_cap_bytes();
 size_t pool_device_mallocs();
+inline size_t pool_block_bytes(size_t bytes) { return ((bytes > 16 ? bytes : 16) + 255) & ~(size_t)255; }
+size_t pool_live_bytes();
+size_t pool_peak_bytes();
+size_t pool_held_after(const std::vector<size_t> &wants);
 inline std::atomic<size_t> &host_count_reads_ref() { static std::atomic<size_t> n{0}; return n; }
 inline size_t host_count_reads() { return host_count_reads_ref().load(); }
 inline void zero(void *p, size_t bytes) { if (bytes) check(hipMemsetAsync(p, 0, bytes, ctx().stream), "hipMemsetAsync"); }
diff --git a/redner_amd/csrc/hip/trace.hip b/redner_amd/csrc/hip/trace.hip
--- a/redner_amd/csrc/hip/trace.hip
+++ b/redner_amd/csrc/hip/trace.hip
@@ -4,6 +4,7 @@
 #include <algorithm>
 #include <cstring>
 #include <map>
+#include <set>
 #include <type_traits>
 #include <unordered_map>
 #include <vector>
@@ -32,6 +33,7 @@
     std::unordered_map<void *, std::pair<size_t, int>> live;
     size_t parked[16] = {};
     size_t from_driver[16] = {};
+    size_t peak[16] = {};
     size_t device_mallocs = 0;
     long long cap_override = -1;
 };
@@ -66,8 +68,9 @@
     if (poison) check(hipMemsetAsync(p, 0xFF, std::max<size_t>(bytes, 16), ctx().stream), "pool poison");
     return p;
 }
+static inline bool close_fit(size_t block, size_t want) { return block <= want + want / 4 + 4096; }
 static void *pool_alloc_raw(size_t bytes) {
-    const size_t want = (std::max<size_t>(bytes, 16) + 255) & ~(size_t)255;
+    const size_t want = pool_block_bytes(bytes);
     int dev = 0;
     (void)hipGetDevice(&dev);
     Pool &pl = pool();
@@ -75,7 +78,7 @@
         std::lock_guard<std::mutex> lk(pl.lock);
         auto &fl = pl.free_blocks[dev & 15];
         auto it = fl.lower_bound(want);
-        if (it != fl.end() && it->first <= want + want / 4 + 4096) {
+        if (it != fl.end() && close_fit(it->first, want)) {
             void *p = it->second;
             pl.live[p] = {it->first, dev};
             pl.parked[dev & 15] -= it->first;
@@ -93,6 +96,7 @@
     std::lock_guard<std::mutex> lk(pl.lock);
     pl.device_mallocs++;
     pl.from_driver[dev & 15] += want;
+    pl.peak[dev & 15] = std::max(pl.peak[dev & 15], pl.from_driver[dev & 15]);
     pl.live[p] = {want, dev};
     return p;
 }
@@ -128,6 +132,7 @@
             fl.clear();
             pl.from_driver[d] -= pl.parked[d];
             pl.parked[d] = 0;
+            pl.peak[d] = pl.from_driver[d];
         }
     }
     if (gone.empty()) return;
@@ -172,6 +177,41 @@
 }
 
 size_t pool_device_mallocs() { Pool &pl = pool(); std::lock_guard<std::mutex> lk(pl.lock); return pl.device_mallocs; }
+
+size_t pool_live_bytes() {
+    int dev = 0;
+    (void)hipGetDevice(&dev);
+    Pool &pl = pool();
+    std::lock_guard<std::mutex> lk(pl.lock);
+    return pl.from_driver[dev & 15] - pl.parked[dev & 15];
+}
+
+size_t pool_held_after(const std::vector<size_t> &wants) {
+    int dev = 0;
+    (void)hipGetDevice(&dev);
+    Pool &pl = pool();
+    std::multiset<size_t> parked;
+    size_t held;
+    {
+        std::lock_guard<std::mutex> lk(pl.lock);
+        for (const auto &kv : pl.free_blocks[dev & 15]) parked.insert(kv.first);
+        held = pl.from_driver[dev & 15];
+    }
+    for (size_t want : wants) {
+        auto it = parked.lower_bound(want);
+        if (it != parked.end() && close_fit(*it, want)) parked.erase(it);
+        else held += want;
+    }
+    return held;
+}
+
+size_t pool_peak_bytes() {
+    int dev = 0;
+    (void)hipGetDevice(&dev);
+    Pool &pl = pool();
+    std::lock_guard<std::mutex> lk(pl.lock);
+    return pl.peak[dev & 15];
+}
 
 namespace {
 struct Staging { char *base = nullptr; size_t cap = 0, used = 0; };
diff --git a/redner_amd/csrc/pool_stats.h b/redner_amd/csrc/pool_stats.h
--- /dev/null
+++ b/redner_amd/csrc/pool_stats.h
@@ -0,0 +1,13 @@
+#pragma once
+#include "exec.h"
+#include <cstddef>
+#include <vector>
+
+#ifdef RDR_HOSTSIM
+namespace exec {
+inline size_t pool_block_bytes(size_t bytes) { return ((bytes > 16 ? bytes : 16) + 255) & ~(size_t)255; }
+inline size_t pool_live_bytes() { return 0; }
+inline size_t pool_peak_bytes() { return 0; }
+inline size_t pool_held_after(const std::vector<size_t> &) { return 0; }
+}
+#endif
diff --git a/redner_amd/csrc/render.cpp b/redner_amd/csrc/render.cpp
--- a/redner_amd/csrc/render.cpp
+++ b/redner_amd/csrc/render.cpp
@@ -9,7 +9,9 @@
 #include "stages_edge.h"
 #include "grad_store.h"
 #include <algorithm>
+#include <condition_variable>
 #include <memory>
+#include <mutex>
 #include <stdexcept>
 #include <type_traits>
 #include <vector>
@@ -189,6 +191,7 @@
         launch_v(lean, b.num_active, contrib);
     }
     int *pos_out = q.pos[chain->flip];
+    if (!pos_out) throw std::logic_error("render: a fused bounce without its queue positions (WorkerShape::may_fuse)");
     chain->flip ^= 1;
     const exec::Count next = exec::compact_dev(b.active, b.num_active, b.next_active, KeepHit{vn.shape}, nullptr, b.dyn, b.dyn_inc, pos_out);
     chain->have_rays = b.vnn != nullptr;
@@ -199,32 +202,49 @@
 
 struct BatchView { int S = 1, P0 = 0, rows = 0; bool on = false; };
 
-struct Worker {
-    Arena arena;
+struct WorkerBuffers {
     std::vector<VSlice> vs;
     int *active = nullptr;
-    Queues q;
+    Queues q{};
     std::vector<exec::Count> num_active;
     int *main_dyn = nullptr;
     int *seg = nullptr;
     float *stage = nullptr;
+};
+struct WorkerShape {
+    int B = 0, PL = 0, nd = 0;
+    bool gradient = false;
+    bool rdiff = true;
+    bool may_fuse = false;
+    bool pcg = false, batch_on = false, staging = false;
+};
+void allot(WorkerBuffers &w, Arena &a, const WorkerShape &s) {
+    const int B = s.B, PL = s.PL;
+    w.vs.resize(B + 1);
+    for (int d = 0; d <= B; ++d) w.vs[d] = make_slice(a, PL, d < B && s.gradient, s.rdiff);
+    w.active = a.get<int>((size_t)(B + 1) * PL);
+    w.q.nee = a.get<rt::RayRec>((size_t)2 * PL); w.q.bsdf = a.get<rt::RayRec>((size_t)2 * PL);
+    w.q.h_nee = a.get<rt::HitRec>((size_t)2 * PL); w.q.h_bsdf = a.get<rt::HitRec>((size_t)2 * PL);
+    w.q.pos[0] = w.q.pos[1] = nullptr;
+    if (s.may_fuse) { w.q.pos[0] = a.get<int>((size_t)2 * PL); w.q.pos[1] = a.get<int>((size_t)2 * PL); }
+    w.num_active.assign(B + 2, exec::Count(0));
+    if (s.pcg) w.main_dyn = a.get<int>(1);
+    if (s.batch_on) w.seg = a.get<int>((size_t)(B + 1) * (kMaxBatch + 1));
+    if (s.staging) w.stage = a.get<float>((size_t)(B + 1) * PL * s.nd);
+}
+struct Worker : WorkerBuffers {
+    Arena arena;
     Fork shadow_fork;
 };
 
-struct Backward {
-    const Scene &scene; const rdr_render_options &opt;
-    Worker &w;
-    int stride, B;
-    const float *d_image; float *screen_grad; double weight; int nd, radiance_dim;
-    BatchView batch;
-    SceneD sd;
-    GradStore &grads;
-    Arena arena;
+struct BackwardShape {
+    int P = 0, P0 = 0, nd = 0, lean = kGeneral;
+    bool edges = false;
+    bool mipmaps = false, envmap = false, batch_on = false, radiance_only = true, pcg = false;
+};
+struct BackwardBuffers {
     AdjState adj;
     int adj_point_doubles = kAdjPointDoubles;
-
-    ChannelsD ch;
-    int lean = kGeneral;
     uint64_t *pcg_edge = nullptr;
     int *edge_dyn = nullptr;
     int *hoist_dyn = nullptr;
@@ -250,6 +270,80 @@
     SecondaryEdgeRec *sec_recs = nullptr;
     SecPick *sec_picks = nullptr;
     unsigned char *sec_mode = nullptr;
+
+    void allot(Arena &arena, const BackwardShape &s) {
+        const int P = s.P;
+        adj.n = P; adj.plain = 0;
+        adj.thr = arena.get<double>((size_t)3 * P);
+        adj.ray_dir = arena.get<double>((size_t)3 * P);
+        adj_point_doubles = s.lean == kLean ? kAdjPointDoublesLean : kAdjPointDoubles;
+        adj.point = arena.get<double>((size_t)adj_point_doubles * P);
+        adj.carries = !s.envmap ? arena.get<unsigned char>((size_t)P) : nullptr;
+        nee_act = arena.get<int>((size_t)P);
+        if (!s.edges) return;
+        edge_dyn = arena.get<int>(kMaxBatch);
+        hoist_dyn = arena.get<int>(kMaxBatch);
+        const int L = 2 * P;
+        ea = make_slice(arena, L, false, s.lean != kLean);
+        eb = make_slice(arena, L, false, s.lean != kLean);
+        if (s.mipmaps) {
+            ea.erd = eb.erd = arena.get<double>((size_t)12 * L);
+            if (s.batch_on) {
+                chain_n = 2 * s.P0;
+                ea.erd_touched = eb.erd_touched = arena.get<unsigned char>(L);
+                erd_chain = arena.get<double>((size_t)12 * chain_n);
+                deferred = arena.get<int>(L);
+                deferred_seg = arena.get<int>(kMaxBatch + 1);
+                deferred_count = arena.get<int>(kMaxBatch);
+                prim_dyn = arena.get<int>(kMaxBatch);
+            }
+        }
+        for (int k = 0; k < 3; ++k) elist[k] = arena.get<int>(L);
+        nee_slots = arena.get<int>(P);
+        gather_cands = arena.get<GatherCand>((size_t)kGatherCands * P);
+        gshared.book = arena.get<GatherBook>(1);
+        gshared.heavy_cap = (int)std::min<long long>(std::max<long long>((long long)P / 256, kGatherHeavyCap), kGatherHeavyMax);
+        gshared.work_cap = (int)std::min<long long>(std::max<long long>((long long)P / 32, kGatherWorkCap), kGatherWorkMax);
+        gshared.heavy_slot = arena.get<int>(gshared.heavy_cap);
+        gshared.work = arena.get<GatherWork>(gshared.work_cap);
+        gshared.cands_big = arena.get<GatherCand>((size_t)kGatherCandsBig * gshared.heavy_cap);
+        h_leaves = arena.get<HLeaf>((size_t)kHSamples * P);
+        h_spill = arena.get<HLeaf>((size_t)(kHSamples - kHStackLds) * P);
+        h_descent = arena.get<HDescent>((size_t)P);
+        edge_contrib = arena.get<double>(L);
+        edge_tmin = arena.get<double>(L);
+        hit_pos = arena.get<double>((size_t)3 * L);
+        if (s.batch_on && s.envmap) {
+            hp_written = arena.get<unsigned char>(L);
+            hp_violations = arena.get<int>(1);
+            hp_event_cap = L;
+            hp_events = arena.get<HitEvent>((size_t)hp_event_cap);
+            hp_event_count = arena.get<int>(1);
+            hp_carry = arena.get<double>((size_t)3 * 2 * s.P0);
+            replay_live = arena.get<unsigned char>(P);
+        }
+        static_assert(sizeof(PrimaryEdgeRec) <= sizeof(SecondaryEdgeRec) && alignof(PrimaryEdgeRec) <= alignof(SecondaryEdgeRec), "edge records share one array");
+        sec_recs = arena.get<SecondaryEdgeRec>(P);
+        prim_recs = arena.counting ? nullptr : reinterpret_cast<PrimaryEdgeRec *>(sec_recs);
+        sec_picks = arena.get<SecPick>(P);
+        sec_mode = arena.get<unsigned char>(P);
+        if (!s.radiance_only) multipliers = arena.get<double>((size_t)L * s.nd);
+        if (s.pcg) pcg_edge = arena.get<uint64_t>(P);
+    }
+};
+
+struct Backward : BackwardBuffers {
+    const Scene &scene; const rdr_render_options &opt;
+    Worker &w;
+    int stride, B;
+    const float *d_image; float *screen_grad; double weight; int nd, radiance_dim;
+    BatchView batch;
+    SceneD sd;
+    GradStore &grads;
+    Arena arena;
+
+    ChannelsD ch;
+    int lean = kGeneral;
     Sink esink{}, psink{};
 
     Fork walk_fork;
@@ -271,80 +365,26 @@
 
     Backward(const Scene &scene_, const rdr_render_options &opt_, GradStore &grads_, Worker &w_, int P, int B_,
              const float *d_image_, float *screen_grad_, double weight_, int nd_, int radiance_dim_, const ChannelsD &ch_,
-             const BatchView &batch_)
+             const BatchView &batch_, const BackwardShape &shape)
         : scene(scene_), opt(opt_), w(w_), stride(P), B(B_), d_image(d_image_), screen_grad(screen_grad_), weight(weight_),
           nd(nd_), radiance_dim(radiance_dim_), batch(batch_), sd(scene_.d), grads(grads_), ch(ch_) {
         if (batch.on) sd.cam.batch_rows = batch.rows;
         lean = scene_kind(scene, ch);
-        adj.n = P; adj.plain = 0;
-        adj.thr = arena.get<double>((size_t)3 * P);
-        adj.ray_dir = arena.get<double>((size_t)3 * P);
-        adj_point_doubles = lean == kLean ? kAdjPointDoublesLean : kAdjPointDoubles;
-        adj.point = arena.get<double>((size_t)adj_point_doubles * P);
-        adj.carries = scene.d.envmap == nullptr ? arena.get<unsigned char>((size_t)P) : nullptr;
-        nee_act = arena.get<int>((size_t)P);
-        const bool use_edges = scene.edges && scene.edges->d.num_edges > 0 &&
-                              (scene.use_primary_edges || scene.use_secondary_edges);
-        if (use_edges) {
-            edge_dyn = arena.get<int>(kMaxBatch);
-            hoist_dyn = arena.get<int>(kMaxBatch);
+        allot(arena, shape);
+        if (edges_on()) {
             const int L = 2 * P;
-            ea = make_slice(arena, L, false, lean != kLean);
-            eb = make_slice(arena, L, false, lean != kLean);
-            if (scene.has_mipmaps) {
-                ea.erd = eb.erd = arena.get<double>((size_t)12 * L);
-                exec::zero(ea.erd, sizeof(double) * 12 * L);
-                if (batch.on) {
-                    chain_n = 2 * batch.P0;
-                    ea.erd_touched = eb.erd_touched = arena.get<unsigned char>(L);
-                    erd_chain = arena.get<double>((size_t)12 * chain_n);
-                    exec::zero(erd_chain, sizeof(double) * 12 * chain_n);
-                    deferred = arena.get<int>(L);
-                    deferred_seg = arena.get<int>(kMaxBatch + 1);
-                    deferred_count = arena.get<int>(kMaxBatch);
-                    prim_dyn = arena.get<int>(kMaxBatch);
-                }
-            }
-            for (int k = 0; k < 3; ++k) elist[k] = arena.get<int>(L);
-            nee_slots = arena.get<int>(P);
-            gather_cands = arena.get<GatherCand>((size_t)kGatherCands * P);
-            gshared.book = arena.get<GatherBook>(1);
-            gshared.heavy_cap = (int)std::min<long long>(std::max<long long>((long long)P / 256, kGatherHeavyCap), kGatherHeavyMax);
-            gshared.work_cap = (int)std::min<long long>(std::max<long long>((long long)P / 32, kGatherWorkCap), kGatherWorkMax);
-            gshared.heavy_slot = arena.get<int>(gshared.heavy_cap);
-            gshared.work = arena.get<GatherWork>(gshared.work_cap);
-            gshared.cands_big = arena.get<GatherCand>((size_t)kGatherCandsBig * gshared.heavy_cap);
+            if (ea.erd) exec::zero(ea.erd, sizeof(double) * 12 * L);
+            if (erd_chain) exec::zero(erd_chain, sizeof(double) * 12 * chain_n);
             if (tuning().gather_heavy_cap >= 0) gshared.heavy_cap = std::min(tuning().gather_heavy_cap, gshared.heavy_cap);
             if (tuning().gather_work_cap >= 0) gshared.work_cap = std::min(tuning().gather_work_cap, gshared.work_cap);
-            h_leaves = arena.get<HLeaf>((size_t)kHSamples * P);
-            h_spill = arena.get<HLeaf>((size_t)(kHSamples - kHStackLds) * P);
-            h_descent = arena.get<HDescent>((size_t)P);
-            edge_contrib = arena.get<double>(L);
-            edge_tmin = arena.get<double>(L);
-            hit_pos = arena.get<double>((size_t)3 * L);
             exec::zero(hit_pos, sizeof(double) * 3 * L);
-            if (batch.on && scene.d.envmap != nullptr) {
-                hp_written = arena.get<unsigned char>(L);
-                hp_violations = arena.get<int>(1);
+            if (hp_written) {
                 exec::zero(hp_violations, sizeof(int));
-                hp_event_cap = L;
-                hp_events = arena.get<HitEvent>((size_t)hp_event_cap);
                 if (tuning().stale_event_cap >= 0) hp_event_cap = std::min(tuning().stale_event_cap, hp_event_cap);
-                hp_event_count = arena.get<int>(1);
                 exec::zero(hp_event_count, sizeof(int));
-                hp_carry = arena.get<double>((size_t)3 * 2 * batch.P0);
                 exec::zero(hp_carry, sizeof(double) * 3 * 2 * batch.P0);
-                replay_live = arena.get<unsigned char>(P);
-            }
-            prim_recs = arena.get<PrimaryEdgeRec>(P);
-            sec_recs = arena.get<SecondaryEdgeRec>(P);
-            sec_picks = arena.get<SecPick>(P);
-            sec_mode = arena.get<unsigned char>(P);
-            if (!ch.radiance_only) multipliers = arena.get<double>((size_t)L * nd);
-            if (opt.sampler_type == RDR_SAMPLER_INDEPENDENT) {
-                pcg_edge = arena.get<uint64_t>(P);
-                exec::launch(P, PcgInit{pcg_edge, pcg_stream_seed(opt) + 131071U});
-            }
+            }
+            if (pcg_edge) exec::launch(P, PcgInit{pcg_edge, pcg_stream_seed(opt) + 131071U});
         }
         esink = Sink{nullptr, edge_contrib, nd, radiance_dim, weight, ch, nullptr};
         psink = Sink{nullptr, edge_contrib, nd, radiance_dim, weight, ch, multipliers};
@@ -678,32 +718,66 @@
     mix((uint64_t)scene.h_envmap.values.width[0]); mix((uint64_t)scene.h_envmap.values.height[0]);
     return h | 1;
 }
-BatchView choose_batch(const rdr_render_options &opt, const Tuning &tune, int P, int rows, int lean, int nd,
-                       bool samples_independent, bool forward_batches, bool gradient) {
-    const int B = opt.max_bounces;
+struct CallShape {
+    WorkerShape worker;
+    BackwardShape backward;
+    bool gradient = false, forward_batches = false, samples_independent = false, chain = false;
+    int gradient_workers(const Tuning &tune, int lanes, int batches, bool batch_on) const {
+        return std::max(1, std::min(tune.workers > 0 ? tune.workers : exec::sample_workers(lanes, batches, batch_on), batches));
+    }
+    int workers_for(const Tuning &tune, int lanes, int batches, bool batch_on) const {
+        if (chain) return 1;
+        if (samples_independent) return gradient_workers(tune, lanes, batches, batch_on);
+        if (!(forward_batches && batch_on)) return 1;
+        return std::max(1, std::min(tune.workers > 0 ? tune.workers : std::max(1, forward_default()), batches));
+    }
+    static int forward_default() {
+        static const int dflt = [] { const char *e = std::getenv("RDR_FORWARD_WORKERS"); return e ? std::max(0, std::atoi(e)) : 1; }();
+        return dflt;
+    }
+};
+size_t call_bytes(const CallShape &cs, const Tuning &tune, int num_samples, int P, int S, std::vector<size_t> *wants = nullptr) {
+    const int PL = S * P, batches = (num_samples + S - 1) / S;
+    const bool on = S > 1;
+    const bool own_size = cs.forward_batches && tune.workers <= 0 && CallShape::forward_default() == 0;
+    const int wk = cs.chain || own_size ? 1 : cs.gradient_workers(tune, PL, batches, on);
+    Arena count;
+    count.counting = true;
+    WorkerShape ws = cs.worker;
+    ws.PL = PL; ws.batch_on = on; ws.staging = on; ws.gradient = true;
+    WorkerBuffers wb;
+    allot(wb, count, ws);
+    BackwardShape bs = cs.backward;
+    bs.P = PL; bs.batch_on = on;
+    BackwardBuffers bb;
+    bb.allot(count, bs);
+    size_t bytes = count.counted * (size_t)wk;
+    if (wants) for (int k = 0; k < wk; ++k) wants->insert(wants->end(), count.wants.begin(), count.wants.end());
+    if (on) {
+        bytes += exec::pool_block_bytes(sizeof(float) * (size_t)PL * ws.nd);
+        if (wants) wants->push_back(exec::pool_block_bytes(sizeof(float) * (size_t)PL * ws.nd));
+    }
+    return bytes;
+}
+
+BatchView choose_batch(const rdr_render_options &opt, const Tuning &tune, int P, int rows, const CallShape &cs) {
+    const bool samples_independent = cs.samples_independent, forward_batches = cs.forward_batches;
     BatchView batch;
     batch.P0 = P; batch.rows = rows;
     if (!samples_independent && !forward_batches) return batch;
     const int batch_cap = std::min(kMaxBatch, tune.batch_samples);
     const long long total = (long long)opt.num_samples * P;
     int want = opt.num_samples;
-    if (total > (1 << 17) && samples_independent) want = (opt.num_samples + 1) / 2;
+    if (total > (1 << 17) && (samples_independent || forward_batches)) want = (opt.num_samples + 1) / 2;
     long long lane_cap = tune.batch_lanes;
     if (lane_cap == 0) {
         lane_cap = 1LL << 24;
         if (total > (1LL << 22) && exec::memory_held_by_others() > 0.10) lane_cap = 1LL << 22;
     }
     batch.S = std::max(1, std::min(std::min(batch_cap, want), (int)std::max(1LL, lane_cap / P)));
-    auto bytes_needed = [&](int S_try) {
-        const double lanes = (double)S_try * P;
-        const int wk = !samples_independent ? 1 : (tune.workers > 0 ? tune.workers : 2);
-        double per_lane = (lean == kLean ? 260.0 * (B + 1) + 660.0 : 400.0 * (B + 1) + 1200.0) * wk;
-        if (forward_batches) per_lane += 4.0 * nd * (B + 1);
-        if (gradient) per_lane += 4.0 * nd;
-        return per_lane * lanes;
-    };
+    auto bytes_needed = [&](int S_try) { return (double)call_bytes(cs, tune, opt.num_samples, P, S_try); };
     if (tune.batch_lanes == 0 && tune.mem_available_mb < 0) {
-        const double cap = (double)exec::pool_cap_bytes();
+        const double cap = (double)exec::pool_cap_bytes() - (double)exec::pool_live_bytes();
         while (batch.S > 1 && bytes_needed(batch.S) > cap) --batch.S;
     }
     if (tune.mem_available_mb >= 0 || bytes_needed(batch.S) > 1073741824.0) {
@@ -772,7 +846,22 @@
     const bool batchable = sobol_plain && (lean == kLean || no_edge_passes || scene.d.envmap == nullptr || envmap_batches);
     const bool samples_independent = batchable && d_image != nullptr && image == nullptr;
     const bool forward_batches = sobol_plain && d_image == nullptr && image != nullptr;
-    const BatchView batch = choose_batch(opt, tune, P, cam.vp_y1 - cam.vp_y0, lean, lay.nd, samples_independent, forward_batches, d_image != nullptr);
+    CallShape cs;
+    cs.gradient = d_image != nullptr; cs.forward_batches = forward_batches; cs.samples_independent = samples_independent;
+    cs.chain = chain && d_image != nullptr;
+    cs.worker.B = B; cs.worker.nd = lay.nd; cs.worker.gradient = d_image != nullptr; cs.worker.rdiff = lean != kLean;
+    cs.worker.pcg = pcg_main != nullptr;
+    cs.worker.may_fuse = fuse_bounces(pcg_main != nullptr, lean, 2 * P);
+    cs.backward.P0 = P; cs.backward.nd = lay.nd; cs.backward.lean = lean;
+    cs.backward.edges = scene.use_primary_edges || scene.use_secondary_edges;
+    cs.backward.mipmaps = scene.has_mipmaps; cs.backward.envmap = scene.d.envmap != nullptr;
+    cs.backward.radiance_only = lay.ch.radiance_only; cs.backward.pcg = opt.sampler_type == RDR_SAMPLER_INDEPENDENT;
+    const BatchView batch = choose_batch(opt, tune, P, cam.vp_y1 - cam.vp_y0, cs);
+    if (d_image != nullptr) {
+        std::vector<size_t> wants;
+        call_bytes(cs, tune, opt.num_samples, P, batch.S, &wants);
+        last_call_bytes().store((uint64_t)exec::pool_held_after(wants));
+    }
     const int S = batch.S;
     const int PL = S * P;
     static const bool tell = std::getenv("RDR_DEBUG_BATCH") != nullptr;
@@ -786,24 +875,31 @@
         d_image_lanes = rep;
     }
     const int *assign_flags = batch.on && forward_batches && !lay.ch.radiance_only ? upload_assign_flags(arena, opt, scene.max_generic_texture_dimension, lay.nd) : nullptr;
-    int workers = 1;
-    if (samples_independent) workers = std::max(1, std::min(tune.workers > 0 ? tune.workers : exec::sample_workers(PL, num_batches, batch.on), num_batches));
-    if (chain) workers = 1;
-    if (d_image != nullptr) { last_schedule()[0].store(S); last_schedule()[1].store(workers); }
+    const int workers = cs.workers_for(tune, PL, num_batches, batch.on);
+    if (d_image != nullptr) {
+        last_schedule()[0].store(S); last_schedule()[1].store(workers);
+    }
 
     struct SampleWorker : Worker { std::unique_ptr<Backward> bwd; };
-    auto make_worker = [&](SampleWorker &w) {
-        w.vs.resize(B + 1);
-        for (int d = 0; d <= B; ++d) w.vs[d] = make_slice(w.arena, PL, d < B && d_image_lanes != nullptr, lean != kLean);
-        w.active = w.arena.get<int>((size_t)(B + 1) * PL);
-        w.q.nee = w.arena.get<rt::RayRec>((size_t)2 * PL); w.q.bsdf = w.arena.get<rt::RayRec>((size_t)2 * PL);
-        w.q.h_nee = w.arena.get<rt::HitRec>((size_t)2 * PL); w.q.h_bsdf = w.arena.get<rt::HitRec>((size_t)2 * PL);
-        w.q.pos[0] = w.arena.get<int>((size_t)2 * PL); w.q.pos[1] = w.arena.get<int>((size_t)2 * PL);
-        w.num_active.assign(B + 2, exec::Count(0));
-        if (pcg_main) w.main_dyn = w.arena.get<int>(1);
-        if (batch.on) w.seg = w.arena.get<int>((size_t)(B + 1) * (kMaxBatch + 1));
-        if (batch.on && forward_batches) w.stage = w.arena.get<float>((size_t)(B + 1) * PL * lay.nd);
+    WorkerShape wshape = cs.worker;
+    wshape.PL = PL; wshape.batch_on = batch.on; wshape.staging = batch.on && forward_batches;
+    auto make_worker = [&](SampleWorker &w) { allot(w, w.arena, wshape); };
+    struct ResolveOrder {
+        std::vector<exec::Fence> fence;
+        std::mutex m; std::condition_variable cv;
+        int recorded = 0;
+        bool failed = false;
+        explicit ResolveOrder(int n) : fence((size_t)n) {}
+        void wait_for(int b) {
+            std::unique_lock<std::mutex> lk(m);
+            cv.wait(lk, [&] { return recorded >= b || failed; });
+            if (recorded < b) throw std::runtime_error("render: another sample worker failed");
+        }
+        void done(int b) { { std::lock_guard<std::mutex> lk(m); recorded = b + 1; } cv.notify_all(); }
+        void fail() { { std::lock_guard<std::mutex> lk(m); failed = true; } cv.notify_all(); }
     };
+    std::unique_ptr<ResolveOrder> resolved;
+    if (workers > 1 && batch.on && forward_batches) resolved.reset(new ResolveOrder(num_batches));
     auto run_samples = [&](SampleWorker &w, int first, int stride) {
         std::vector<VSlice> &vs = w.vs;
         int *active = w.active;
@@ -853,11 +949,18 @@
                 if (num_active[d + 1].dev && d_image) segments(d + 1);
                 dim += 7;
             }
-            if (w.stage) exec::launch(P * lay.nd, ResolveBatchImage{image, w.stage, P, lay.nd, S_now, B + 1, plane, assign_flags, vs[0].shape});
+            if (w.stage) {
+                if (resolved && b > 0) { resolved->wait_for(b); resolved->fence[b - 1].gate(exec::ctx().stream); }
+                exec::launch(P * lay.nd, ResolveBatchImage{image, w.stage, P, lay.nd, S_now, B + 1, plane, assign_flags, vs[0].shape});
+                if (resolved) { resolved->fence[b].after(exec::ctx().stream); resolved->done(b); }
+            }
 
             if (d_image && !w.bwd) {
                 scene.edge_data();
-                w.bwd.reset(new Backward(scene, opt, *grads, w, PL, B, d_image_lanes, screen_gradient_image, weight, lay.nd, lay.radiance_dim, lay.ch, batch));
+                BackwardShape bshape = cs.backward;
+                bshape.P = PL; bshape.batch_on = batch.on;
+                bshape.edges = bshape.edges && scene.edges && scene.edges->d.num_edges > 0;
+                w.bwd.reset(new Backward(scene, opt, *grads, w, PL, B, d_image_lanes, screen_gradient_image, weight, lay.nd, lay.radiance_dim, lay.ch, batch, bshape));
             }
             if (w.bwd) w.bwd->run_sample(sample_id, rng, lanes, S_now);
             if (w.bwd && w.bwd->hp_violations && (b == first || b + stride >= num_batches)) {
@@ -880,13 +983,15 @@
         for (int k = 1; k < workers; ++k)
             exec::SecondThread::get(k - 1).start([&, k] {
                 TuningScope helper_scope(tune);
-                SampleWorker w;
-                make_worker(w);
-                run_samples(w, k, workers);
-                exec::sync();
+                try {
+                    SampleWorker w;
+                    make_worker(w);
+                    run_samples(w, k, workers);
+                    exec::sync();
+                } catch (...) { if (resolved) resolved->fail(); throw; }
             });
         std::exception_ptr failure;
-        try { run_samples(w0, 0, workers); } catch (...) { failure = std::current_exception(); }
+        try { run_samples(w0, 0, workers); } catch (...) { failure = std::current_exception(); if (resolved) resolved->fail(); }
         for (int k = 1; k < workers; ++k) {
             try { exec::SecondThread::get(k - 1).wait(); } catch (...) { if (!failure) failure = std::current_exception(); }
         }
diff --git a/redner_amd/csrc/tuning.h b/redner_amd/csrc/tuning.h
--- a/redner_amd/csrc/tuning.h
+++ b/redner_amd/csrc/tuning.h
@@ -107,6 +107,7 @@
 }
 
 inline std::atomic<int> *last_schedule() { static std::atomic<int> s[2]; return s; }
+inline std::atomic<uint64_t> &last_call_bytes() { static std::atomic<uint64_t> b{0}; return b; }
 
 inline Tuning &tuning() {
     static thread_local Tuning t = resolve_tuning(nullptr);
```

Measured after the change: 86.05 Msamples/s. About the same (-0.4%).
